# tirr-c/jxl-oxide

Measured on NVIDIA H100. Metric: Megapixels/s decoded (8K VarDCT d1.0), higher is better.
Workload: dtype f32

## Files before the change

### jxl_oxide_b200/csrc/cuda_backend.cu

```cuda
#include "cuda_backend.h"

#include <algorithm>
#include <chrono>
#include <cmath>
#include <cstdlib>
#include <cstring>
#include <atomic>
#include <thread>

namespace jxlb {

void upload_sec_large(const float* host224);

#define CUDA_CHECK(expr)                                                                              \
  do {                                                                                                \
    cudaError_t err__ = (expr);                                                                       \
    if (err__ != cudaSuccess)                                                                         \
      fail(kErrCuda, std::string("CUDA error: ") + cudaGetErrorString(err__) + " at " #expr);        \
  } while (0)

CudaBackend::CudaBackend(int device, bool own_stream) : device_(device), own_stream_(own_stream) {
  int count = 0;
  cudaError_t e = cudaGetDeviceCount(&count);
  if (e != cudaSuccess || count == 0)
    fail(kErrCuda, "no CUDA device available: the jxl_oxide_b200 hot path has no CPU fallback");
  CUDA_CHECK(cudaSetDevice(device_));
  if (own_stream_) CUDA_CHECK(cudaStreamCreateWithFlags(&stream_, cudaStreamNonBlocking));
  CUDA_CHECK(cudaEventCreateWithFlags(&sync_event_, cudaEventBlockingSync | cudaEventDisableTiming));
  stage_cap_ = size_t(2) << 20;
  CUDA_CHECK(cudaHostAlloc(reinterpret_cast<void**>(&h_stage_), stage_cap_, cudaHostAllocDefault));
  CUDA_CHECK(cudaMalloc(reinterpret_cast<void**>(&d_stage_), stage_cap_));
  result_cap_ = size_t(256) << 10;
  CUDA_CHECK(cudaHostAlloc(reinterpret_cast<void**>(&h_result_), result_cap_, cudaHostAllocMapped));
  {
    void* f = nullptr;
    CUDA_CHECK(cudaHostAlloc(&f, 128, cudaHostAllocMapped));
    h_flag_ = static_cast<volatile uint32_t*>(f);
    h_flag_[0] = 0;
    h_flag_[16] = 0;
  }
  ensure_static_tables();
  cudaMemPoolProps props;
  std::memset(&props, 0, sizeof(props));
  props.allocType = cudaMemAllocationTypePinned;
  props.handleTypes = cudaMemHandleTypeNone;
  props.location.type = cudaMemLocationTypeDevice;
  props.location.id = device_;
  CUDA_CHECK(cudaMemPoolCreate(&pool_, &props));
  uint64_t keep = UINT64_MAX;
  CUDA_CHECK(cudaMemPoolSetAttribute(pool_, cudaMemPoolAttrReleaseThreshold, &keep));
  CUDA_CHECK(cudaDeviceSetCacheConfig(cudaFuncCachePreferShared));
  if (const char* lanes = std::getenv("JXLB_HF_LANES")) {
    const int n = std::atoi(lanes);
    hf_streams_per_cta = n <= 0 ? 0 : (n <= 4 ? 4 : (n <= 8 ? 8 : (n <= 16 ? 16 : (n <= 32 ? 32 : (n <= 64 ? 64 : 128)))));
  }
}

CudaBackend::~CudaBackend() {
  cudaSetDevice(device_);
  if (stream_) cudaStreamSynchronize(stream_);
  for (auto& kv : planes_)
    if (!(arena_base_ && kv.second.ptr >= static_cast<void*>(arena_base_) && kv.second.ptr < static_cast<void*>(arena_base_ + arena_cap_)) &&
        !in_lf_arena(kv.second.ptr))
      cudaFree(kv.second.ptr);
  for (void* p : temps_)
    if (!in_lf_arena(p)) cudaFree(p);
  for (void* p : deferred_free_) cudaFree(p);
  if (d_codestream_ && !in_lf_arena(d_codestream_) && stream_) cudaFreeAsync(d_codestream_, stream_);
  if (d_natural_orders_) cudaFree(d_natural_orders_);
  if (d_dequant_) cudaFree(d_dequant_);
  if (d_dequant_default_) cudaFree(d_dequant_default_);
  if (sync_event_) cudaEventDestroy(sync_event_);
  if (h_stage_) cudaFreeHost(h_stage_);
  if (d_stage_) cudaFree(d_stage_);
  if (h_result_) cudaFreeHost(h_result_);
  if (h_input_) cudaFreeHost(h_input_);
  if (h_flag_) cudaFreeHost(const_cast<uint32_t*>(h_flag_));
  if (stream_ && own_stream_) cudaStreamDestroy(stream_);
  if (lf_arena_) cudaFree(lf_arena_);
  if (pool_) cudaMemPoolDestroy(pool_);
}

cudaStream_t CudaBackend::S() {
  if (!stream_) {
    JXLB_CHECK(bool(on_need_stream), kErrCuda, "decoder has no CUDA stream");
    if (!heavy_announced_ && (profile || host_phases)) ++profile_acc["host:slot_before_heavy"].first;
    on_need_stream();
    JXLB_CHECK(stream_ != nullptr, kErrCuda, "no CUDA stream was leased to the decoder");
    if (pending_cs_bytes_) {
      CUDA_CHECK(cudaMemcpyAsync(d_codestream_, h_input_, pending_cs_bytes_, cudaMemcpyHostToDevice, stream_));
      pending_cs_bytes_ = 0;
    }
    for (void* p : deferred_free_) CUDA_CHECK(cudaFreeAsync(p, stream_));
    deferred_free_.clear();
  }
  return stream_;
}

void CudaBackend::end_lease() {
  if (!stream_ || own_stream_) return;
  release_temps();
  if (d_dequant_) {
    dfree(d_dequant_);
    d_dequant_ = nullptr;
    cached_hfg_ = nullptr;
  }
  if (d_codestream_ && !in_lf_arena(d_codestream_)) {
    CUDA_CHECK(cudaFreeAsync(d_codestream_, stream_));
    d_codestream_ = nullptr;
    codestream_cap_ = 0;
  }
  stream_ = nullptr;
}

void* CudaBackend::lf_arena_alloc(size_t bytes) {
  if (!lf_arena_) {
    CUDA_CHECK(cudaSetDevice(device_));
    CUDA_CHECK(cudaMalloc(reinterpret_cast<void**>(&lf_arena_), kLfArenaBytes));
  }
  const size_t need = (bytes + 255) & ~size_t(255);
  if (lf_arena_off_ + need > kLfArenaBytes) return nullptr;
  void* p = lf_arena_ + lf_arena_off_;
  lf_arena_off_ += need;
  return p;
}

void CudaBackend::begin_heavy_stage(size_t bytes_hint) {
  if (heavy_announced_) return;
  heavy_announced_ = true;
  if (on_heavy_stage) on_heavy_stage(bytes_hint);
}

void CudaBackend::end_arena() {
  if (!arena_base_) return;
  auto inside = [&](const void* p) { return p >= static_cast<void*>(arena_base_) && p < static_cast<void*>(arena_base_ + arena_cap_); };
  std::vector<void*> keep;
  for (void* p : temps_)
    if (!inside(p)) keep.push_back(p);
  temps_.swap(keep);
  if (d_dequant_ && inside(d_dequant_)) {
    d_dequant_ = nullptr;
    cached_hfg_ = nullptr;
  }
  for (auto it = planes_.begin(); it != planes_.end();)
    it = inside(it->second.ptr) ? planes_.erase(it) : std::next(it);
  arena_base_ = nullptr;
  arena_cap_ = arena_off_ = 0;
}

void* CudaBackend::dmalloc(size_t bytes) {
  void* p = nullptr;
  if (mem_limit_ && mem_in_use_ + bytes > mem_limit_)
    fail(kErrOutOfMemory, "allocation budget exceeded: " + std::to_string(mem_in_use_ + bytes) + " > " + std::to_string(mem_limit_) + " bytes");
  if (arena_base_ && bytes >= (256u << 10)) {
    const size_t need = (bytes + 511) & ~size_t(511);
    if (arena_off_ + need <= arena_cap_) {
      p = arena_base_ + arena_off_;
      arena_off_ += need;
      arena_peak_ = std::max(arena_peak_, arena_off_);
      if (mem_limit_) mem_in_use_ += need;
      return p;
    }
    arena_spill_ += need;
  }
  if (!stream_ && lf_service) {
    if (void* q = lf_arena_alloc(std::max<size_t>(bytes, 16))) return q;
  }
  CUDA_CHECK(cudaSetDevice(device_));
  CUDA_CHECK(cudaMallocFromPoolAsync(&p, std::max<size_t>(bytes, 16), pool_, S()));
  if (mem_limit_) {
    mem_in_use_ += bytes;
    alloc_sizes_[p] = bytes;
  }
  return p;
}
void CudaBackend::dfree(void* p) {
  if (!p) return;
  if (in_lf_arena(p)) return;
  if (!stream_ && lf_service) {
    deferred_free_.push_back(p);
    return;
  }
  if (arena_base_ && p >= arena_base_ && p < arena_base_ + arena_cap_) return;
  if (mem_limit_) {
    auto it = alloc_sizes_.find(p);
    if (it != alloc_sizes_.end()) {
      mem_in_use_ -= std::min<uint64_t>(mem_in_use_, it->second);
      alloc_sizes_.erase(it);
    }
  }
  CUDA_CHECK(cudaFreeAsync(p, S()));
}
void* CudaBackend::upload_temp(const void* src, size_t bytes) {
  const size_t off = (stage_off_ + 15) & ~size_t(15);
  if (off + bytes <= stage_cap_) {
    if (bytes) std::memcpy(h_stage_ + off, src, bytes);
    stage_off_ = off + bytes;
    return d_stage_ + off;
  }
  void* p = dmalloc(bytes);
  temps_.push_back(p);
  if (bytes) CUDA_CHECK(cudaMemcpyAsync(p, src, bytes, cudaMemcpyHostToDevice, S()));
  return p;
}
void* CudaBackend::stage_scratch(size_t bytes) {
  if (stream_) flush_uploads();
  const size_t off = (stage_off_ + 15) & ~size_t(15);
  if (off + bytes <= stage_cap_) {
    stage_off_ = off + bytes;
    if (stream_) stage_flushed_ = stage_off_;
    return d_stage_ + off;
  }
  void* p = dmalloc(bytes);
  temps_.push_back(p);
  return p;
}
void CudaBackend::flush_uploads() {
  if (!stream_ && lf_service) return;
  if (stage_off_ > stage_flushed_)
    CUDA_CHECK(cudaMemcpyAsync(d_stage_ + stage_flushed_, h_stage_ + stage_flushed_, stage_off_ - stage_flushed_, cudaMemcpyHostToDevice, S()));
  stage_flushed_ = stage_off_;
}
void* CudaBackend::fetch_result(const void* dsrc, size_t bytes) {
  const size_t off = (result_off_ + 15) & ~size_t(15);
  JXLB_CHECK(off + bytes <= result_cap_, kErrUnsupported, "too many stream jobs in one launch for the result buffer");
  CUDA_CHECK(cudaMemcpyAsync(h_result_ + off, dsrc, bytes, cudaMemcpyDeviceToHost, S()));
  result_off_ = off + bytes;
  return h_result_ + off;
}
void CudaBackend::release_temps() {
  for (void* p : temps_) dfree(p);
  temps_.clear();
}
void CudaBackend::sync() {
  if (!stream_) return;
  flush_uploads();
  const uint32_t seq = ++sync_seq_;
  launch_signal_word(const_cast<uint32_t*>(h_flag_), seq, S());
  ++launches;
  uint32_t spins = 0;
  const auto t_begin = std::chrono::steady_clock::now();
  auto t0 = t_begin;
  while (*h_flag_ != seq) {
    if (++spins < 2000) {
#if defined(__x86_64__)
      __builtin_ia32_pause();
#endif
      continue;
    }
    const auto waited = std::chrono::steady_clock::now() - t_begin;
    const long nap_us = std::min<long>(200, std::max<long>(20, std::chrono::duration_cast<std::chrono::microseconds>(waited).count() / 8));
    std::this_thread::sleep_for(std::chrono::microseconds(nap_us));
    if ((spins & 255) == 0 && std::chrono::steady_clock::now() - t0 > std::chrono::milliseconds(200)) {
      cudaError_t e = cudaStreamQuery(S());
      if (e == cudaSuccess) break;
      if (e != cudaErrorNotReady) fail(kErrCuda, std::string("CUDA error: ") + cudaGetErrorString(e) + " while waiting for the stream");
      t0 = std::chrono::steady_clock::now();
    }
  }
  std::atomic_thread_fence(std::memory_order_acquire);
  stage_off_ = stage_flushed_ = 0;
  result_off_ = 0;
  resolve_profile();
}

namespace {
struct TimeOrigin {
  cudaEvent_t ev = nullptr;
  double host_ms = 0.0;
  unsigned long long dev_ns = 0;
};
double host_now_ms() {
  return std::chrono::duration<double, std::milli>(std::chrono::steady_clock::now().time_since_epoch()).count();
}
TimeOrigin& time_origin() {
  static TimeOrigin o = [] {
    TimeOrigin t;
    cudaEventCreate(&t.ev);
    cudaDeviceSynchronize();
    cudaEventRecord(t.ev, 0);
    cudaEventSynchronize(t.ev);
    unsigned long long* d = nullptr;
    cudaMalloc(&d, 8);
    launch_read_globaltimer(d, 0);
    cudaMemcpy(&t.dev_ns, d, 8, cudaMemcpyDeviceToHost);
    cudaFree(d);
    t.host_ms = std::chrono::duration<double, std::milli>(std::chrono::steady_clock::now().time_since_epoch()).count();
    return t;
  }();
  return o;
}
}

void CudaBackend::begin_k(const char* name) {
  S();
  flush_uploads();
  ++launches;
  if (!profile) return;
  time_origin();
  PendingTiming t;
  t.name = name;
  CUDA_CHECK(cudaEventCreate(&t.e0));
  CUDA_CHECK(cudaEventCreate(&t.e1));
  CUDA_CHECK(cudaEventRecord(t.e0, S()));
  pending_.push_back(t);
}

void CudaBackend::end_k() {
  if (!profile || pending_.empty()) return;
  CUDA_CHECK(cudaEventRecord(pending_.back().e1, S()));
}

void CudaBackend::resolve_profile() {
  for (PendingTiming& t : pending_) {
    float ms = 0.0f;
    if (cudaEventElapsedTime(&ms, t.e0, t.e1) == cudaSuccess) {
      auto& acc = profile_acc[t.name];
      acc.first += 1;
      acc.second += double(ms);
      float since = 0.0f;
      if (cudaEventElapsedTime(&since, time_origin().ev, t.e0) == cudaSuccess)
        timeline.push_back({t.name, double(since), double(since) + double(ms)});
    }
    cudaEventDestroy(t.e0);
    cudaEventDestroy(t.e1);
  }
  pending_.clear();
}

uint8_t* CudaBackend::upload_resident(const uint8_t* data, size_t size) {
  CUDA_CHECK(cudaSetDevice(device_));
  size_t need = ((size + 7) & ~size_t(7)) + 64;
  uint8_t* p = nullptr;
  CUDA_CHECK(cudaMalloc(&p, need));
  CUDA_CHECK(cudaMemset(p, 0, need));
  CUDA_CHECK(cudaMemcpy(p, data, size, cudaMemcpyHostToDevice));
  return p;
}

void CudaBackend::set_codestream(const uint8_t* data, size_t size) {
  CUDA_CHECK(cudaSetDevice(device_));
  stages.clear();
  stage_dims.clear();
  if (!stream_) {
    lf_arena_off_ = 0;
    if (in_lf_arena(d_codestream_)) d_codestream_ = nullptr, codestream_cap_ = 0;
    pending_cs_bytes_ = 0;
  }
  if (resident_next_) {
    active_cs_ = resident_next_;
    resident_next_ = nullptr;
    ensure_static_tables();
    return;
  }
  size_t need = ((size + 7) & ~size_t(7)) + 64;
  if (need > input_cap_) {
    if (h_input_) CUDA_CHECK(cudaFreeHost(h_input_));
    h_input_ = nullptr;
    input_cap_ = std::max<size_t>(need + need / 2, size_t(1) << 20);
    CUDA_CHECK(cudaHostAlloc(reinterpret_cast<void**>(&h_input_), input_cap_, cudaHostAllocDefault));
  }
  std::memcpy(h_input_, data, size);
  std::memset(h_input_ + size, 0, need - size);
  if (!stream_ && lf_service) {
    if (void* q = lf_arena_alloc(need)) {
      d_codestream_ = static_cast<uint8_t*>(q);
      codestream_cap_ = need;
      pending_cs_bytes_ = need;
      active_cs_ = d_codestream_;
      ensure_static_tables();
      return;
    }
  }
  if (need > codestream_cap_ || in_lf_arena(d_codestream_)) {
    if (d_codestream_ && !in_lf_arena(d_codestream_)) CUDA_CHECK(cudaFreeAsync(d_codestream_, S()));
    d_codestream_ = nullptr;
    codestream_cap_ = std::max<size_t>(need + need / 2, size_t(1) << 20);
    CUDA_CHECK(cudaMallocFromPoolAsync(reinterpret_cast<void**>(&d_codestream_), codestream_cap_, pool_, S()));
  }
  CUDA_CHECK(cudaMemcpyAsync(d_codestream_, h_input_, need, cudaMemcpyHostToDevice, S()));
  active_cs_ = d_codestream_;
  ensure_static_tables();
}

void CudaBackend::new_frame() {
  heavy_announced_ = false;
  cached_hfg_ = nullptr;
  if (d_dequant_) {
    dfree(d_dequant_);
    d_dequant_ = nullptr;
  }
}

void CudaBackend::ensure_static_tables() {
  if (!d_natural_orders_) {
    const std::vector<uint32_t> all = natural_order_table(natural_order_offset_);
    CUDA_CHECK(cudaMalloc(&d_natural_orders_, all.size() * 4));
    CUDA_CHECK(cudaMemcpy(d_natural_orders_, all.data(), all.size() * 4, cudaMemcpyHostToDevice));
  }
  if (!sec_uploaded_) {
    float tab[224];
    size_t off = 0;
    for (int i = 0; i < 3; ++i) {
      size_t n = size_t(64) << i;
      for (size_t k = 0; k < n / 2; ++k) {
        float theta = float(2 * k + 1) / float(2 * n) * 3.14159265358979323846f;
        tab[off + k] = (1.0f / cosf(theta)) / 2.0f;
      }
      off += n / 2;
    }
    upload_sec_large(tab);
    sec_uploaded_ = true;
  }
}

int CudaBackend::alloc_plane(uint32_t w, uint32_t h, bool zero) {
  PlaneRec r;
  r.w = w;
  r.h = h;
  size_t bytes = size_t(w) * h * 4;
  r.ptr = dmalloc(bytes);
  if (zero) CUDA_CHECK(cudaMemsetAsync(r.ptr, 0, bytes, S()));
  int id = next_id_++;
  planes_[id] = r;
  return id;
}

void CudaBackend::free_plane(int id) {
  auto it = planes_.find(id);
  if (it == planes_.end()) return;
  dfree(it->second.ptr);
  planes_.erase(it);
}

DevView CudaBackend::dev_view(const View& v) const {
  DevView d;
  d.ptr = nullptr;
  d.stride = 0;
  d.w = v.w;
  d.h = v.h;
  if (v.plane >= 0) {
    const PlaneRec& p = planes_.at(v.plane);
    d.ptr = static_cast<uint32_t*>(p.ptr) + size_t(v.y0) * p.w + v.x0;
    d.stride = p.w;
  }
  return d;
}

void CudaBackend::download_rect(const View& v, void* dst) {
  if (!v.w || !v.h) return;
  DevView d = dev_view(v);
  if (d.stride == v.w)
    CUDA_CHECK(cudaMemcpyAsync(dst, d.ptr, size_t(v.w) * v.h * 4, cudaMemcpyDeviceToHost, S()));
  else
    CUDA_CHECK(cudaMemcpy2DAsync(dst, size_t(v.w) * 4, d.ptr, size_t(d.stride) * 4, size_t(v.w) * 4, v.h,
                                 cudaMemcpyDeviceToHost, S()));
  sync();
}

void CudaBackend::copy_rect(const View& src, const View& dst) {
  begin_k("copy_rect");
  launch_copy_rect(dev_view(src), dev_view(dst), S());
  end_k();
}

void CudaBackend::phase_mark(const char* name) {
  if (!profile && !host_phases) return;
  const double now = std::chrono::duration<double, std::milli>(std::chrono::steady_clock::now().time_since_epoch()).count();
  if (name && phase_t0_ >= 0.0) {
    auto& acc = profile_acc[std::string("host:") + name];
    acc.first += 1;
    acc.second += now - phase_t0_;
    if (profile) timeline.push_back({std::string("host:") + name, phase_t0_ - time_origin().host_ms, now - time_origin().host_ms});
  }
  phase_t0_ = now;
}

void CudaBackend::stage_marker(const char* name, const View* views, int n) {
  if (!stop_stage.empty() && stop_stage == name) {
    stop_dims.clear();
    for (int i = 0; i < n; ++i) {
      stop_dims.push_back({views[i].w, views[i].h});
      if (size_t(i) < stop_dst.size() && stop_dst[size_t(i)] && views[i].w && views[i].h) {
        JXLB_CHECK(stop_stride >= views[i].w, kErrInvalidArg, "destination stride smaller than the stage's planes");
        const DevView d = dev_view(views[i]);
        CUDA_CHECK(cudaMemcpy2DAsync(stop_dst[size_t(i)], size_t(stop_stride) * 4, d.ptr, size_t(d.stride) * 4, size_t(views[i].w) * 4,
                                     views[i].h, cudaMemcpyDeviceToDevice, S()));
      }
    }
    sync();
    throw StopDecode();
  }
  if (!capture) return;
  auto& out = stages[name];
  auto& dims = stage_dims[name];
  out.clear();
  dims.clear();
  for (int i = 0; i < n; ++i) {
    std::vector<uint32_t> buf(size_t(views[i].w) * views[i].h);
    download_rect(views[i], buf.data());
    out.push_back(std::move(buf));
    dims.push_back({views[i].w, views[i].h});
  }
}

namespace {
const char* dev_status_message(int s) {
  switch (s) {
    case kDevBadStream: return "invalid entropy-coded stream (ANS final state / LZ77)";
    case kDevOverrun: return "entropy-coded stream reads past the end of its section";
    case kDevInvalid: return "semantic validation of a decoded stream failed";
    case kDevUnsupported: return "chroma subsampling with varblocks larger than 8x8 is not supported";
    case kDevBadLayout: return "invalid HfMetadata block layout";
    default: return "unknown device decode error";
  }
}
}

void CudaBackend::decode_modular(std::vector<ModularStreamJob>& jobs) {
  if (jobs.empty()) return;
  ModularLaunch L = build_modular_launch(jobs, [this](const View& v) { return dev_view(v); }, *this);
  for (size_t i = 0; i < jobs.size(); ++i) {
    const ModularLaunch::JobNeeds& n = L.needs[i];
    if (n.wp_scratch_bytes) temps_.push_back(L.jobs[i].wp_scratch = static_cast<int32_t*>(dmalloc(n.wp_scratch_bytes)));
    if (n.lz_window_bytes) temps_.push_back(L.jobs[i].lz_window = static_cast<uint32_t*>(dmalloc(n.lz_window_bytes)));
  }
  const DevModularJob* d_jobs = static_cast<const DevModularJob*>(upload_temp(L.jobs.data(), L.jobs.size() * sizeof(DevModularJob)));
  const DevChannel* d_chans = static_cast<const DevChannel*>(upload_temp(L.channels.data(), L.channels.size() * sizeof(DevChannel)));
  uint64_t* d_end = static_cast<uint64_t*>(stage_scratch(jobs.size() * 8));
  int* d_status = static_cast<int*>(stage_scratch(jobs.size() * 4));
  const DevChannelPlan* d_plans = static_cast<const DevChannelPlan*>(upload_temp(L.plans.data(), L.plans.size() * sizeof(DevChannelPlan)));
  unsigned long long* d_trace = nullptr;
  double host_launch = 0.0;
  if (trace_device) {
    time_origin();
    d_trace = static_cast<unsigned long long*>(dmalloc(jobs.size() * 16));
    temps_.push_back(d_trace);
    host_launch = host_now_ms();
  }
  const uint64_t* end;
  const int* status;
  if (!stream_ && lf_service && !d_trace && jobs.size() <= 2048) {
    LfBatchItem item;
    if (pending_cs_bytes_) {
      item.up[item.num_up++] = {d_codestream_, h_input_, pending_cs_bytes_};
      pending_cs_bytes_ = 0;
    }
    item.up[item.num_up++] = {d_stage_, h_stage_, stage_off_};
    item.ref.cs = active_cs_;
    item.ref.jobs = d_jobs;
    item.ref.channels = d_chans;
    item.ref.plans = d_plans;
    item.ref.end_bits = d_end;
    item.ref.status = d_status;
    item.num_jobs = int(jobs.size());
    item.smem_bytes = L.smem_bytes;
    item.all_staged = L.all_staged;
    uint8_t* h_end = h_result_;
    uint8_t* h_status = h_result_ + ((jobs.size() * 8 + 15) & ~size_t(15));
    JXLB_CHECK(size_t(h_status - h_result_) + jobs.size() * 4 <= result_cap_, kErrUnsupported, "too many stream jobs in one launch for the result buffer");
    if (profile || ((stage_off_ + 15) & ~size_t(15)) + 4 > stage_cap_) {
      item.down[item.num_down++] = {h_end, d_end, jobs.size() * 8};
      item.down[item.num_down++] = {h_status, d_status, jobs.size() * 4};
    } else {
      const uint32_t zero = 0;
      item.ref.counter = static_cast<uint32_t*>(upload_temp(&zero, 4));
      item.up[item.num_up - 1].bytes = stage_off_;
      item.ref.end_bits = reinterpret_cast<uint64_t*>(h_end);
      item.ref.status = reinterpret_cast<int*>(h_status);
      item.ref.num_jobs = uint32_t(jobs.size());
      item.ref.done_flag = const_cast<uint32_t*>(h_flag_ + 16);
      item.ref.done_seq = ++item_seq_;
      item.done_flag = h_flag_ + 16;
    }
    item.want_timing = profile;
    lf_service->run(item);
    ++launches;
    if (profile) {
      auto& acc = profile_acc["modular_decode"];
      acc.first += 1;
      acc.second += double(item.elapsed_ms);
    }
    stage_off_ = stage_flushed_ = 0;
    result_off_ = 0;
    end = reinterpret_cast<const uint64_t*>(h_end);
    status = reinterpret_cast<const int*>(h_status);
  } else {
    begin_k("modular_decode");
    launch_modular_decode(active_cs_, d_jobs, d_chans, d_plans, d_end, d_status, int(jobs.size()), L.smem_bytes, L.all_staged, S(), d_trace);
    end_k();
    end = static_cast<const uint64_t*>(fetch_result(d_end, jobs.size() * 8));
    status = static_cast<const int*>(fetch_result(d_status, jobs.size() * 4));
    const unsigned long long* trace = d_trace ? static_cast<const unsigned long long*>(fetch_result(d_trace, jobs.size() * 16)) : nullptr;
    sync();
    if (d_trace) {
      const TimeOrigin& o = time_origin();
      unsigned long long first = ~0ull, last = 0;
      for (size_t i = 0; i < jobs.size(); ++i) {
        first = std::min<unsigned long long>(first, trace[2 * i]);
        last = std::max<unsigned long long>(last, trace[2 * i + 1]);
      }
      timeline.push_back({"host:launch_to_return modular", host_launch - o.host_ms, host_now_ms() - o.host_ms});
      timeline.push_back({"dev:modular_decode", (double(first) - double(o.dev_ns)) * 1e-6, (double(last) - double(o.dev_ns)) * 1e-6});
    }
    CUDA_CHECK(cudaGetLastError());
  }
  release_temps();
  for (size_t i = 0; i < jobs.size(); ++i) {
    if (status[i] != kDevOk && status[i] != kDevBadLayout)
      fail(status[i] == kDevOverrun ? kErrEof : kErrDeviceDecode,
           std::string("modular stream ") + std::to_string(jobs[i].stream_index) + ": " + dev_status_message(status[i]));
    jobs[i].end_bit = size_t(end[i]);
    jobs[i].placed = jobs[i].placement.group.nb_blocks != 0;
    jobs[i].layout_ok = status[i] == kDevOk;
  }
}

int CudaBackend::squeeze_inverse(const View& avg, const View& res, bool horizontal) {
  uint32_t ow = horizontal ? avg.w + res.w : avg.w;
  uint32_t oh = horizontal ? avg.h : avg.h + res.h;
  JXLB_CHECK(horizontal ? (res.h == avg.h || res.w == 0) : (res.w == avg.w || res.h == 0), kErrBitstream,
             "squeeze residual size mismatch");
  int id = alloc_plane(std::max(ow, 1u), std::max(oh, 1u), false);
  if (!ow || !oh) return id;
  View ov{id, 0, 0, ow, oh};
  begin_k("squeeze_inverse");
  launch_squeeze_inverse(dev_view(avg), dev_view(res), dev_view(ov), horizontal, S());
  end_k();
  return id;
}

std::vector<int> CudaBackend::squeeze_inverse_many(const std::vector<std::pair<View, View>>& avg_res, bool horizontal) {
  std::vector<int> ids;
  std::vector<DevView> a, r, o;
  for (const auto& p : avg_res) {
    const View& avg = p.first;
    const View& res = p.second;
    const uint32_t ow = horizontal ? avg.w + res.w : avg.w, oh = horizontal ? avg.h : avg.h + res.h;
    JXLB_CHECK(horizontal ? (res.h == avg.h || res.w == 0) : (res.w == avg.w || res.h == 0), kErrBitstream,
               "squeeze residual size mismatch");
    const int id = alloc_plane(std::max(ow, 1u), std::max(oh, 1u), false);
    ids.push_back(id);
    if (!ow || !oh) continue;
    a.push_back(dev_view(avg));
    r.push_back(dev_view(res));
    o.push_back(dev_view(View{id, 0, 0, ow, oh}));
  }
  if (!o.empty()) {
    begin_k("squeeze_inverse");
    launch_squeeze_inverse_batch(a.data(), r.data(), o.data(), int(o.size()), horizontal, S());
    end_k();
  }
  return ids;
}

void CudaBackend::rct_inverse(const View v[3], uint32_t rct_type) {
  begin_k("rct_inverse");
  launch_rct_inverse(dev_view(v[0]), dev_view(v[1]), dev_view(v[2]), rct_type, S());
  end_k();
}

void CudaBackend::palette_inverse(const View& palette, const std::vector<View>& targets, const Transform& t,
                                  const WpHeader& wph, uint32_t bit_depth) {
  JXLB_CHECK(targets.size() <= size_t(kMaxPaletteChannels), kErrUnsupported, "palettes with more than 16 channels are not implemented on the device");
  DevView tv[kMaxPaletteChannels];
  for (size_t i = 0; i < targets.size(); ++i) tv[i] = dev_view(targets[i]);
  const uint32_t w = targets[0].w, h = targets[0].h;
  int* d_status = static_cast<int*>(dmalloc(4));
  uint8_t* d_mask = static_cast<uint8_t*>(dmalloc(size_t(w) * h));
  CUDA_CHECK(cudaMemsetAsync(d_status, 0, 4, S()));
  DevView pal{};
  if (palette.plane >= 0) pal = dev_view(palette);
  begin_k("palette_inverse");
  launch_palette_inverse(pal, tv, int(targets.size()), int(t.nb_colours), int(bit_depth), int(t.nb_deltas), d_mask, d_status, S());
  end_k();
  const int* num_delta_p = static_cast<const int*>(fetch_result(d_status, 4));
  sync();
  const int num_delta = *num_delta_p;
  if (num_delta > 0) {
    JXLB_CHECK(t.d_pred <= 13, kErrBitstream, "invalid delta-palette predictor");
    DevPaletteDeltaParams p;
    std::memset(&p, 0, sizeof(p));
    for (size_t i = 0; i < targets.size(); ++i) p.target[i] = tv[i];
    p.mask = d_mask;
    p.d_pred = t.d_pred;
    pack_wp(wph, p.wp);
    int32_t* rows = nullptr;
    if (t.d_pred == 6) rows = static_cast<int32_t*>(dmalloc(targets.size() * ((5 * size_t(w) + 3) & ~size_t(3)) * 4));
    p.wp_rows = rows;
    begin_k("palette_delta");
    launch_palette_delta(p, int(targets.size()), S());
    end_k();
    sync();
    if (rows) dfree(rows);
  }
  dfree(d_status);
  dfree(d_mask);
}

void CudaBackend::int_to_float(const View& v, const BitDepth& d) {
  begin_k("int_to_float");
  launch_int_to_float(dev_view(v), d.bits_per_sample, d.exp_bits, d.float_sample, S());
  end_k();
}

void CudaBackend::modular_xyb_to_float(const View yxb[3], const float m[3]) {
  begin_k("modular_xyb");
  launch_modular_xyb(dev_view(yxb[0]), dev_view(yxb[1]), dev_view(yxb[2]), m[0], m[1], m[2], S());
  end_k();
}

void CudaBackend::build_block_info(VarDctState& st, const std::vector<BlockInfoJob>& jobs) {
  if (jobs.empty()) return;
  std::vector<DevPlacement> dp;
  for (const BlockInfoJob& j : jobs) dp.push_back(make_dev_placement(varblock_placement(st, j), [this](const View& v) { return dev_view(v); }));
  const DevPlacement* d_jobs = static_cast<const DevPlacement*>(upload_temp(dp.data(), dp.size() * sizeof(DevPlacement)));
  int* d_status = static_cast<int*>(stage_scratch(jobs.size() * 4));
  begin_k("place_varblocks");
  launch_place_varblocks(d_jobs, int(jobs.size()), d_status, S());
  end_k();
  const int* status = static_cast<const int*>(fetch_result(d_status, jobs.size() * 4));
  sync();
  CUDA_CHECK(cudaGetLastError());
  release_temps();
  for (size_t i = 0; i < jobs.size(); ++i) JXLB_CHECK(status[i] == kDevOk, kErrBitstream, "invalid HfMetadata block layout");
}

void CudaBackend::decode_hf(VarDctState& st, std::vector<HfGroupJob>& jobs) {
  if (jobs.empty()) return;
  const uint32_t pass = jobs[0].pass_idx;
  const HfPassSyntax& hp = st.hfg->passes[pass];
  const bool hf_lz77 = hp.code.lz77_enabled;
  const DevHfParams p = build_hf_params(st, pass, *this, d_natural_orders_, natural_order_offset_);
  const HfSchedule sched = hf_schedule(p, hf_streams_per_cta);
  const std::vector<uint32_t> perm = hf_launch_order(jobs, sched.lanes);
  std::vector<DevHfJob> dj;
  for (uint32_t i : perm) dj.push_back({jobs[i].bit_pos, jobs[i].bit_limit, jobs[i].group_idx});
  const DevHfJob* d_jobs = static_cast<const DevHfJob*>(upload_temp(dj.data(), dj.size() * sizeof(DevHfJob)));
  uint64_t* d_end = static_cast<uint64_t*>(stage_scratch(jobs.size() * 8));
  int* d_status = static_cast<int*>(stage_scratch(jobs.size() * 4));
  uint2* d_list = nullptr;
  uint32_t* d_counts = nullptr;
  if (sched.lanes) {
    const size_t groups = hf_block_list_count(dev_frame(st), p);
    const size_t records = groups * p.group_dim_blocks * p.group_dim_blocks;
    d_list = static_cast<uint2*>(dmalloc(records * sizeof(uint2) + groups * 4));
    temps_.push_back(d_list);
    d_counts = reinterpret_cast<uint32_t*>(d_list + records);
    begin_k("hf_block_ctx");
    launch_hf_block_list(dev_frame(st), p, d_list, d_counts, S());
    end_k();
  }
  begin_k("decode_hf");
  if (sched.lanes)
    launch_decode_hf_lanes(active_cs_, dev_frame(st), p, d_list, d_counts, d_jobs, d_end, d_status, int(jobs.size()),
                           pass == 0 ? 1 : 0, sched.per_cta, S());
  else
    launch_decode_hf(active_cs_, dev_frame(st), p, d_jobs, d_end, d_status, int(jobs.size()), pass == 0 ? 1 : 0,
                     sched.per_cta, S());
  end_k();
  const uint64_t* end = static_cast<const uint64_t*>(fetch_result(d_end, jobs.size() * 8));
  const int* status = static_cast<const int*>(fetch_result(d_status, jobs.size() * 4));
  sync();
  CUDA_CHECK(cudaGetLastError());
  release_temps();
  for (size_t i = 0; i < jobs.size(); ++i) {
    HfGroupJob& job = jobs[perm[i]];
    if (status[i] != kDevOk)
      fail(status[i] == kDevOverrun ? kErrEof : (status[i] == kDevUnsupported ? kErrUnsupported : kErrDeviceDecode),
           std::string("HF group ") + std::to_string(job.group_idx) + ": " + dev_status_message(status[i]));
    job.end_bit = size_t(end[i]);
  }
  JXLB_CHECK(!hf_lz77, kErrUnsupported, "LZ77 in the HF coefficient streams is not supported on the device");
}

void CudaBackend::lf_dequant(VarDctState& st, const std::vector<LfDequantJob>& jobs) {
  std::vector<DevLfDequantJob> dj;
  for (const LfDequantJob& j : jobs)
    dj.push_back({{j.rect.bx0, j.rect.by0, j.rect.bw, j.rect.bh}, {j.scale[0], j.scale[1], j.scale[2]}});
  const DevLfDequantJob* d = static_cast<const DevLfDequantJob*>(upload_temp(dj.data(), dj.size() * sizeof(DevLfDequantJob)));
  begin_k("lf_dequant");
  launch_lf_dequant(dev_frame(st), d, int(dj.size()), S());
  end_k();
}

void CudaBackend::lf_chroma_from_luma(VarDctState& st) {
  const LfGlobalSyntax& g = *st.lfg;
  int32_t x_factor = int32_t(g.x_factor_lf) - 128, b_factor = int32_t(g.b_factor_lf) - 128;
  float kx = g.base_correlation_x + (float(x_factor) / float(g.colour_factor));
  float kb = g.base_correlation_b + (float(b_factor) / float(g.colour_factor));
  begin_k("lf_cfl");
  launch_lf_cfl(dev_frame(st), kx, kb, S());
  end_k();
}

void CudaBackend::lf_adaptive_smoothing(VarDctState& st) {
  const LfGlobalSyntax& g = *st.lfg;
  uint64_t scale_inv = uint64_t(g.global_scale) * g.quant_lf;
  float lf_x = float(512.0 * double(g.m_x_lf) / double(scale_inv));
  float lf_y = float(512.0 * double(g.m_y_lf) / double(scale_inv));
  float lf_b = float(512.0 * double(g.m_b_lf) / double(scale_inv));
  float* tmp[3];
  for (int c = 0; c < 3; ++c) tmp[c] = static_cast<float*>(dmalloc(size_t(st.bw) * st.bh * 4));
  begin_k("lf_smooth");
  launch_lf_smooth(dev_frame(st), tmp, lf_x, lf_y, lf_b, S());
  end_k();
  for (int c = 0; c < 3; ++c) {
    PlaneRec& r = planes_.at(st.lf[c]);
    dfree(r.ptr);
    r.ptr = tmp[c];
  }
}

void CudaBackend::hf_dequant_cfl(VarDctState& st) {
  const bool use_default = st.hfg->dequant_all_default;
  if (use_default ? d_dequant_default_ == nullptr : cached_hfg_ != st.hfg) {
    std::vector<float> all;
    DevDequantParams& dp = use_default ? dequant_default_params_ : dequant_params_;
    std::memset(&dp, 0, sizeof(dp));
    for (int set = 0; set < 17; ++set)
      for (int c = 0; c < 3; ++c)
        for (int tr = 0; tr < 2; ++tr) {
          const std::vector<float>& m = tr ? st.hfg->dequant->matrices_tr[set][c] : st.hfg->dequant->matrices[set][c];
          dp.matrix_offset[(set * 3 + c) * 2 + tr] = uint32_t(all.size());
          all.insert(all.end(), m.begin(), m.end());
        }
    if (use_default) {
      CUDA_CHECK(cudaMalloc(&d_dequant_default_, all.size() * 4));
      CUDA_CHECK(cudaMemcpyAsync(d_dequant_default_, all.data(), all.size() * 4, cudaMemcpyHostToDevice, S()));
      CUDA_CHECK(cudaStreamSynchronize(S()));
    } else {
      if (d_dequant_) dfree(d_dequant_);
      d_dequant_ = static_cast<float*>(dmalloc(all.size() * 4));
      CUDA_CHECK(cudaMemcpyAsync(d_dequant_, all.data(), all.size() * 4, cudaMemcpyHostToDevice, S()));
      cached_hfg_ = st.hfg;
    }
  }
  DevDequantParams p = use_default ? dequant_default_params_ : dequant_params_;
  p.matrices = use_default ? d_dequant_default_ : d_dequant_;
  const OpsinInverseMatrix& oim = st.ih->opsin_inverse_matrix;
  for (int c = 0; c < 3; ++c) p.quant_bias[c] = oim.quant_bias[c];
  p.quant_bias_numerator = oim.quant_bias_numerator;
  p.qm_scale[0] = powi_f32(0.8f, int32_t(st.fh->x_qm_scale) - 2);
  p.qm_scale[1] = 1.0f;
  p.qm_scale[2] = powi_f32(0.8f, int32_t(st.fh->b_qm_scale) - 2);
  p.global_scale = float(st.lfg->global_scale);
  p.base_correlation_x = st.lfg->base_correlation_x;
  p.base_correlation_b = st.lfg->base_correlation_b;
  p.colour_factor = float(st.lfg->colour_factor);
  if (!capture && !st.subsampled && fuse_dequant) {
    pending_dequant_ = p;
    have_pending_dequant_ = true;
    return;
  }
  begin_k("hf_dequant_cfl");
  launch_hf_dequant_cfl(dev_frame(st), p, S());
  end_k();
}

void CudaBackend::hf_transform(VarDctState& st) {
  void* scratch = dmalloc(hf_transform_scratch_bytes(st.bw, st.bh));
  begin_k("hf_transform");
  launch_hf_transform(dev_frame(st), scratch, have_pending_dequant_ ? &pending_dequant_ : nullptr, S());
  end_k();
  have_pending_dequant_ = false;
  dfree(scratch);
}

void CudaBackend::gaborish(const View v[3], const float weights[3][2]) {
  for (int c = 0; c < 3; ++c) {
    PlaneRec& r = planes_.at(v[c].plane);
    JXLB_CHECK(v[c].x0 == 0 && v[c].y0 == 0, kErrInvalidArg, "gaborish expects a top-left anchored view");
    void* out = dmalloc(size_t(r.w) * r.h * 4);
    DevView in = dev_view(v[c]);
    DevView ov = in;
    ov.ptr = out;
    begin_k("gaborish");
    launch_gaborish(in, ov, weights[c][0], weights[c][1], S());
    end_k();
    dfree(r.ptr);
    r.ptr = out;
  }
}

void CudaBackend::epf(const View v[3], const View& sigma, const EpfParams& p, bool sigma_is_constant) {
  DevView cur[3], alt[3];
  void* alt_ptr[3];
  for (int c = 0; c < 3; ++c) {
    PlaneRec& r = planes_.at(v[c].plane);
    JXLB_CHECK(v[c].x0 == 0 && v[c].y0 == 0, kErrInvalidArg, "epf expects a top-left anchored view");
    alt_ptr[c] = dmalloc(size_t(r.w) * r.h * 4);
    cur[c] = dev_view(v[c]);
    alt[c] = cur[c];
    alt[c].ptr = alt_ptr[c];
  }
  const float* d_sigma = nullptr;
  uint32_t sigma_stride = 0;
  if (!sigma_is_constant) {
    const PlaneRec& s = planes_.at(sigma.plane);
    d_sigma = static_cast<const float*>(s.ptr);
    sigma_stride = s.w;
  }
  DevEpfParams dp;
  for (int c = 0; c < 3; ++c) dp.channel_scale[c] = p.channel_scale[c];
  dp.pass0_sigma_scale = p.pass0_sigma_scale;
  dp.pass2_sigma_scale = p.pass2_sigma_scale;
  dp.border_sad_mul = p.border_sad_mul;
  dp.sigma_for_modular = p.sigma_for_modular;
  bool in_alt = false;
  auto run = [&](int step) {
    begin_k("epf_step");
    launch_epf_step(in_alt ? alt : cur, in_alt ? cur : alt, d_sigma, sigma_stride, dp, step, S());
    end_k();
    in_alt = !in_alt;
  };
  if (p.iters == 3) run(0);
  run(1);
  if (p.iters >= 2) run(2);
  for (int c = 0; c < 3; ++c) {
    PlaneRec& r = planes_.at(v[c].plane);
    if (in_alt) {
      dfree(r.ptr);
      r.ptr = alt_ptr[c];
    } else {
      dfree(alt_ptr[c]);
    }
  }
}

bool CudaBackend::filters_colour_fused(const View v[3], const RestorationFilter& rf, const View& sigma,
                                       bool sigma_is_constant, const ColorParams* colour) {
  if (!fuse_filters || !fused_filters_supported(v[0].w, v[0].h)) return false;
  DevView in[3], out[3];
  void* out_ptr[3];
  for (int c = 0; c < 3; ++c) {
    PlaneRec& r = planes_.at(v[c].plane);
    JXLB_CHECK(v[c].x0 == 0 && v[c].y0 == 0, kErrInvalidArg, "filters expect top-left anchored views");
    out_ptr[c] = dmalloc(size_t(r.w) * r.h * 4);
    in[c] = dev_view(v[c]);
    out[c] = in[c];
    out[c].ptr = out_ptr[c];
  }
  const float* d_sigma = nullptr;
  uint32_t sigma_stride = 0;
  if (!sigma_is_constant && rf.epf.iters > 0) {
    const PlaneRec& s = planes_.at(sigma.plane);
    d_sigma = static_cast<const float*>(s.ptr);
    sigma_stride = s.w;
  }
  JXLB_CHECK(!colour || (!colour->second_stage && colour->gamma == 0.0f), kErrInvalidArg,
             "the fused filter kernel converts to sRGB-gamut targets only");
  const DevFusedFilterParams p = fused_filter_params(rf, d_sigma, sigma_stride, colour);
  begin_k("filters_fused");
  launch_filters_fused(in, out, p, S());
  end_k();
  for (int c = 0; c < 3; ++c) {
    PlaneRec& r = planes_.at(v[c].plane);
    dfree(r.ptr);
    r.ptr = out_ptr[c];
  }
  return true;
}

void CudaBackend::blend_patches(const std::vector<PatchJob>& jobs) {
  std::vector<DevPatchJob> batch;
  std::vector<const PatchJob*> members;
  auto flush = [&] {
    if (batch.empty()) return;
    const DevPatchJob* d = static_cast<const DevPatchJob*>(upload_temp(batch.data(), batch.size() * sizeof(DevPatchJob)));
    begin_k("blend_patches");
    launch_blend_patches(d, int(batch.size()), S());
    end_k();
    batch.clear();
    members.clear();
  };
  auto overlaps = [](const View& a, const View& b) {
    return a.plane == b.plane && a.x0 < b.x0 + b.w && b.x0 < a.x0 + a.w && a.y0 < b.y0 + b.h && b.y0 < a.y0 + a.h;
  };
  for (const PatchJob& j : jobs) {
    if (!j.dst.w || !j.dst.h) continue;
    bool clash = false;
    for (const PatchJob* m : members)
      if (overlaps(m->dst, j.dst) || (j.base_alpha.plane >= 0 && overlaps(m->dst, j.base_alpha)) ||
          (j.new_alpha.plane >= 0 && overlaps(m->dst, j.new_alpha)) ||
          (m->base_alpha.plane >= 0 && overlaps(j.dst, m->base_alpha)) ||
          (m->new_alpha.plane >= 0 && overlaps(j.dst, m->new_alpha))) {
        clash = true;
        break;
      }
    if (clash || batch.size() >= 4096) flush();
    DevView s = dev_view(j.src), d = dev_view(j.dst), ba = dev_view(j.base_alpha), na = dev_view(j.new_alpha);
    batch.push_back({static_cast<const float*>(s.ptr), static_cast<float*>(d.ptr), static_cast<const float*>(ba.ptr),
                     static_cast<const float*>(na.ptr), s.stride, d.stride, ba.stride, na.stride, j.dst.w, j.dst.h, j.mode,
                     j.clamp ? 1u : 0u, j.premultiplied ? 1u : 0u, j.swapped ? 1u : 0u});
    members.push_back(&j);
  }
  flush();
}

void CudaBackend::blend_raw(const DevPatchJob& job) {
  const DevPatchJob* d = static_cast<const DevPatchJob*>(upload_temp(&job, sizeof(job)));
  begin_k("blend_patches");
  launch_blend_patches(d, 1, S());
  end_k();
  sync();
  release_temps();
}

void CudaBackend::splat_splines(const View v[3], const std::vector<SplineArc>& arcs) {
  if (arcs.empty()) return;
  static_assert(sizeof(SplineArc) == sizeof(DevSplineArc), "arc layouts must agree");
  DevView dv[3] = {dev_view(v[0]), dev_view(v[1]), dev_view(v[2])};
  const DevSplineArc* d = static_cast<const DevSplineArc*>(upload_temp(arcs.data(), arcs.size() * sizeof(SplineArc)));
  begin_k("splat_splines");
  launch_splat_splines(dv, d, int(arcs.size()), S());
  end_k();
}

void CudaBackend::add_noise(const View v[3], const float lut[8], uint32_t group_dim, uint64_t seed0, float corr_x,
                            float corr_b) {
  JXLB_CHECK(v[0].w >= 2 && v[0].h >= 2, kErrUnsupported, "noise on frames narrower than 2 samples is not supported");
  DevView dv[3];
  float* field[3];
  for (int c = 0; c < 3; ++c) {
    JXLB_CHECK(v[c].w == v[0].w && v[c].h == v[0].h, kErrInvalidArg, "noise needs three equally sized planes");
    dv[c] = dev_view(v[c]);
    field[c] = static_cast<float*>(dmalloc(size_t(v[0].w) * v[0].h * 4));
  }
  DevNoiseParams p;
  for (int i = 0; i < 8; ++i) p.lut[i] = lut[i];
  p.lut[8] = lut[7];
  p.corr_x = corr_x;
  p.corr_b = corr_b;
  p.group_dim = group_dim;
  p.seed0 = seed0;
  begin_k("add_noise");
  launch_add_noise(dv, field, p, S());
  end_k();
  for (int c = 0; c < 3; ++c) dfree(field[c]);
}

void CudaBackend::pack_to_host(const DevPackParams& p, void* dst, size_t bytes) {
  void* d = dmalloc(bytes);
  begin_k("pack_interleaved");
  launch_pack_interleaved(p, d, S());
  end_k();
  CUDA_CHECK(cudaMemcpyAsync(dst, d, bytes, cudaMemcpyDeviceToHost, S()));
  sync();
  dfree(d);
}

void CudaBackend::pack_to_device(const DevPackParams& p, void* d_dst) {
  cudaPointerAttributes attr;
  if (cudaPointerGetAttributes(&attr, d_dst) != cudaSuccess || attr.type != cudaMemoryTypeDevice || attr.device != device_) {
    cudaGetLastError();
    fail(kErrInvalidArg, "destination is not device memory of this decoder's GPU");
  }
  begin_k("pack_interleaved");
  launch_pack_interleaved(p, d_dst, S());
  end_k();
  sync();
}

int CudaBackend::upsample(const View& v, uint32_t factor_log2, const ImageHeader& ih) {
  DevView cur = dev_view(v);
  void* cur_owned = nullptr;
  uint32_t w = v.w, h = v.h;
  auto pass = [&](uint32_t k, const std::vector<float>& weights) {
// ... 181 lines not shown
```

### jxl_oxide_b200/csrc/cuda_backend.h

```cpp
#pragma once
#include <cuda_runtime.h>

#include <functional>
#include <map>
#include <string>
#include <vector>

#include "host/backend.h"
#include "host/jbrd.h"
#include "kernels/kernels.h"
#include "launch_tables.h"

namespace jxlb {

struct LfBatchItem {
  struct Copy {
    void* dst;
    const void* src;
    size_t bytes;
  };
  Copy up[2];
  int num_up = 0;
  DevModularBatchRef ref{};
  int num_jobs = 0;
  size_t smem_bytes = 0;
  bool all_staged = false;
  Copy down[2];
  int num_down = 0;
  volatile uint32_t* done_flag = nullptr;
  bool want_timing = false;
  float elapsed_ms = 0.0f;
};
class LfBatchService {
 public:
  virtual ~LfBatchService() {}
  virtual void run(LfBatchItem& item) = 0;
};

struct StopDecode {};

class CudaBackend : public Backend, private TableSink {
 public:
  explicit CudaBackend(int device, bool own_stream = true);
  ~CudaBackend() override;

  void set_codestream(const uint8_t* data, size_t size) override;
  void new_frame() override;
  int alloc_plane(uint32_t w, uint32_t h, bool zero) override;
  void free_plane(int id) override;
  void download_rect(const View& v, void* dst) override;
  void copy_rect(const View& src, const View& dst) override;
  void decode_modular(std::vector<ModularStreamJob>& jobs) override;
  int squeeze_inverse(const View& avg, const View& residual, bool horizontal) override;
  std::vector<int> squeeze_inverse_many(const std::vector<std::pair<View, View>>& avg_res, bool horizontal) override;
  void rct_inverse(const View v[3], uint32_t rct_type) override;
  void palette_inverse(const View& palette, const std::vector<View>& targets, const Transform& t, const WpHeader& wp,
                       uint32_t bit_depth) override;
  void int_to_float(const View& v, const BitDepth& depth) override;
  void modular_xyb_to_float(const View yxb[3], const float m_lf_unscaled[3]) override;
  void build_block_info(VarDctState& st, const std::vector<BlockInfoJob>& jobs) override;
  void decode_hf(VarDctState& st, std::vector<HfGroupJob>& jobs) override;
  void lf_dequant(VarDctState& st, const std::vector<LfDequantJob>& jobs) override;
  void lf_chroma_from_luma(VarDctState& st) override;
  void lf_adaptive_smoothing(VarDctState& st) override;
  void hf_dequant_cfl(VarDctState& st) override;
  void hf_transform(VarDctState& st) override;
  void gaborish(const View v[3], const float weights[3][2]) override;
  void epf(const View v[3], const View& sigma, const EpfParams& p, bool sigma_is_constant) override;
  int upsample(const View& v, uint32_t factor_log2, const ImageHeader& ih) override;
  int upsample_jpeg(const View& v, bool horizontal, bool vertical, uint32_t out_w, uint32_t out_h) override;
  void blend_patches(const std::vector<PatchJob>& jobs) override;
  void blend_raw(const DevPatchJob& job);
  void splat_splines(const View v[3], const std::vector<SplineArc>& arcs) override;
  void add_noise(const View v[3], const float lut[8], uint32_t group_dim, uint64_t seed0, float corr_x, float corr_b) override;
  void xyb_to_rgb(const View v[3], const ColorParams& p) override;
  void ycbcr_to_rgb(const View v[3], const YcbcrParams& p) override;
  bool filters_colour_fused(const View v[3], const RestorationFilter& rf, const View& sigma, bool sigma_is_constant,
                            const ColorParams* colour) override;
  void stage_marker(const char* name, const View* views, int n) override;
  void phase_mark(const char* name) override;
  void vardct_coefficients(const VarDctState& st) override;
  JpegJob* jpeg_job = nullptr;

  void begin_heavy_stage(size_t bytes_hint) override;
  std::function<void(size_t)> on_heavy_stage;
  std::function<void()> on_need_stream;
  void set_arena(void* base, size_t bytes) {
    arena_base_ = static_cast<uint8_t*>(base);
    arena_cap_ = bytes;
    arena_off_ = 0;
  }
  void end_arena();
  void set_mem_limit(uint64_t bytes) { mem_limit_ = bytes; }
  uint64_t mem_in_use() const { return mem_in_use_; }
  size_t arena_peak() const { return arena_peak_; }
  size_t arena_spill() const { return arena_spill_; }

  cudaStream_t stream() { return S(); }
  void set_stream(cudaStream_t s) { stream_ = s; }
  bool has_stream() const { return stream_ != nullptr; }
  void end_lease();
  LfBatchService* lf_service = nullptr;
  uint8_t* upload_resident(const uint8_t* data, size_t size);
  void use_resident_once(const uint8_t* dptr) { resident_next_ = dptr; }
  void sync();
  void* plane_ptr(int id) const { return id < 0 ? nullptr : planes_.at(id).ptr; }
  DevView dev_view(const View& v) const;

  std::string stop_stage;
  std::vector<void*> stop_dst;
  uint32_t stop_stride = 0;
  std::vector<std::pair<uint32_t, uint32_t>> stop_dims;
  bool capture = false;
  std::map<std::string, std::vector<std::vector<uint32_t>>> stages;
  std::map<std::string, std::vector<std::pair<uint32_t, uint32_t>>> stage_dims;
  uint64_t launches = 0;
  void pack_to_host(const DevPackParams& p, void* dst, size_t bytes);
  void pack_to_device(const DevPackParams& p, void* d_dst);
  bool fuse_dequant = true;
  bool fuse_filters = true;
  int hf_streams_per_cta = 0;
  bool profile = false;
  bool host_phases = false;
  bool trace_device = false;
  double phase_t0_ = -1.0;
  std::map<std::string, std::pair<uint64_t, double>> profile_acc;
  void resolve_profile();

 private:
  struct PlaneRec {
    void* ptr;
    uint32_t w, h;
  };
  void* dmalloc(size_t bytes);
  void dfree(void* p);
  void* upload_temp(const void* src, size_t bytes);
  const void* put(const void* src, size_t bytes) override { return upload_temp(src, bytes); }
  void* stage_scratch(size_t bytes);
  void flush_uploads();
  void release_temps();
  void* fetch_result(const void* dsrc, size_t bytes);
  DevFrame dev_frame(const VarDctState& st) const {
    return make_dev_frame(st, [this](int id) { return plane_ptr(id); });
  }
  void ensure_static_tables();
  uint64_t encode_jpeg_scan(const VarDctState& st, const JpegScanPlan& plan, std::vector<uint8_t>* out);
  void begin_k(const char* name);
  void end_k();
  struct PendingTiming {
    const char* name;
    cudaEvent_t e0, e1;
  };
  std::vector<PendingTiming> pending_;

 public:
  struct TimelineEntry {
    std::string name;
    double t0_ms, t1_ms;
  };
  std::vector<TimelineEntry> timeline;

 private:

  cudaStream_t S();
  void* lf_arena_alloc(size_t bytes);
  bool in_lf_arena(const void* p) const {
    return lf_arena_ && p >= static_cast<const void*>(lf_arena_) && p < static_cast<const void*>(lf_arena_ + kLfArenaBytes);
  }
  int device_;
  bool own_stream_ = true;
  static constexpr size_t kLfArenaBytes = size_t(64) << 20;
  uint8_t* lf_arena_ = nullptr;
  size_t lf_arena_off_ = 0;
  size_t pending_cs_bytes_ = 0;
  std::vector<void*> deferred_free_;
  uint8_t* h_stage_ = nullptr;
  uint8_t* d_stage_ = nullptr;
  size_t stage_cap_ = 0, stage_off_ = 0, stage_flushed_ = 0;
  uint8_t* h_result_ = nullptr;
  size_t result_cap_ = 0, result_off_ = 0;
  uint8_t* h_input_ = nullptr;
  size_t input_cap_ = 0;
  volatile uint32_t* h_flag_ = nullptr;
  uint32_t sync_seq_ = 0, item_seq_ = 0;
  uint8_t* arena_base_ = nullptr;
  size_t arena_cap_ = 0, arena_off_ = 0, arena_peak_ = 0, arena_spill_ = 0;
  bool heavy_announced_ = false;
  uint64_t mem_limit_ = 0, mem_in_use_ = 0;
  std::map<void*, size_t> alloc_sizes_;
  cudaStream_t stream_ = nullptr;
  cudaEvent_t sync_event_ = nullptr;
  cudaMemPool_t pool_ = nullptr;
  uint8_t* d_codestream_ = nullptr;
  const uint8_t* active_cs_ = nullptr;
  const uint8_t* resident_next_ = nullptr;
  size_t codestream_cap_ = 0;
  std::map<int, PlaneRec> planes_;
  int next_id_ = 0;
  std::vector<void*> temps_;
  uint32_t* d_natural_orders_ = nullptr;
  uint32_t natural_order_offset_[13];
  bool sec_uploaded_ = false;
  const HfGlobalSyntax* cached_hfg_ = nullptr;
  float* d_dequant_ = nullptr;
  float* d_dequant_default_ = nullptr;
  DevDequantParams dequant_default_params_;
  DevDequantParams dequant_params_;
  DevDequantParams pending_dequant_;
  bool have_pending_dequant_ = false;
};

}
```

### jxl_oxide_b200/csrc/host/backend.h

```cpp
#pragma once
#include <cstddef>
#include <cstdint>
#include <utility>
#include <vector>

#include "frame_syntax.h"
#include "headers.h"
#include "modular_syntax.h"

namespace jxlb {

struct View {
  int plane = -1;
  uint32_t x0 = 0, y0 = 0, w = 0, h = 0;
};

struct ModularChannelTarget {
  View view;
  int32_t hshift = 0, vshift = 0;
};

struct LfGroupRect {
  uint32_t bx0 = 0, by0 = 0, bw = 0, bh = 0;
};

struct BlockInfoJob {
  LfGroupRect rect;
  int raw_plane = -1;
  uint32_t nb_blocks = 0;
};

struct VarblockPlacement {
  BlockInfoJob group;
  int blk_type = -1, blk_mul = -1, epf_sigma = -1, sharpness = -1;
  float quant_mul_base = 0.0f;
  float sharp_lut[8] = {};
  bool has_epf = false;
};

struct ModularStreamJob {
  size_t bit_pos = 0;
  size_t bit_limit = 0;
  const MaTree* tree = nullptr;
  WpHeader wp;
  uint32_t stream_index = 0;
  std::vector<ModularChannelTarget> channels;
  size_t end_bit = 0;
  VarblockPlacement placement;
  bool placed = false;
  bool layout_ok = true;
};

struct HfGroupJob {
  size_t bit_pos = 0, bit_limit = 0;
  uint32_t group_idx = 0, pass_idx = 0;
  size_t end_bit = 0;
};

struct VarDctState {
  uint32_t width = 0, height = 0;
  uint32_t bw = 0, bh = 0;
  uint32_t group_dim = 256, groups_per_row = 0, num_groups = 0;
  const LfGlobalSyntax* lfg = nullptr;
  const HfGlobalSyntax* hfg = nullptr;
  const FrameHeader* fh = nullptr;
  const ImageHeader* ih = nullptr;
  bool use_lf_frame = false;
  uint32_t hshift[3] = {0, 0, 0}, vshift[3] = {0, 0, 0};
  bool subsampled = false;
  int lf_quant[3] = {-1, -1, -1};
  int x_from_y = -1, b_from_y = -1;
  int sharpness = -1;
  int blk_type = -1;
  int blk_mul = -1;
  int epf_sigma = -1;
  int lf[3] = {-1, -1, -1};
  int coeff[3] = {-1, -1, -1};
};

inline VarblockPlacement varblock_placement(const VarDctState& st, const BlockInfoJob& group) {
  const EpfParams& epf = st.fh->restoration_filter.epf;
  VarblockPlacement p;
  p.group = group;
  p.blk_type = st.blk_type;
  p.blk_mul = st.blk_mul;
  p.epf_sigma = st.epf_sigma;
  p.sharpness = st.sharpness;
  p.quant_mul_base = epf.quant_mul * 65536.0f / float(st.lfg->global_scale);
  for (int i = 0; i < 8; ++i) p.sharp_lut[i] = epf.sharp_lut[i];
  p.has_epf = epf.iters > 0;
  return p;
}

inline LfGroupRect shifted_rect(const LfGroupRect& r, uint32_t hshift, uint32_t vshift) {
  return LfGroupRect{r.bx0 >> hshift, r.by0 >> vshift, (r.bw + (1u << hshift) - 1) >> hshift, (r.bh + (1u << vshift) - 1) >> vshift};
}

struct LfDequantJob {
  LfGroupRect rect;
  float scale[3];
};

struct ColorParams {
  float opsin_bias[3], cbrt_opsin_bias[3];
  float itscale;
  float matrix[9];
  bool apply_srgb_tf;
  bool apply_bt709_tf = false;
  bool second_stage = false;
  float luminances[3] = {0, 0, 0};
  float matrix2[9] = {1, 0, 0, 0, 1, 0, 0, 0, 1};
  bool to_luma = false;
  float gamma = 0.0f;
  float pq_intensity_target = 0.0f;
};

class Backend {
 public:
  virtual ~Backend() {}
  virtual void set_codestream(const uint8_t* data, size_t size) = 0;
  virtual void new_frame() {}
  virtual void begin_heavy_stage(size_t ) {}
  virtual int alloc_plane(uint32_t w, uint32_t h, bool zero) = 0;
  virtual void free_plane(int id) = 0;
  virtual void download_rect(const View& v, void* dst) = 0;
  virtual void copy_rect(const View& src, const View& dst) = 0;
  virtual void decode_modular(std::vector<ModularStreamJob>& jobs) = 0;
  virtual int squeeze_inverse(const View& avg, const View& residual, bool horizontal) = 0;
  virtual std::vector<int> squeeze_inverse_many(const std::vector<std::pair<View, View>>& avg_res, bool horizontal) {
    std::vector<int> ids;
    for (const auto& p : avg_res) ids.push_back(squeeze_inverse(p.first, p.second, horizontal));
    return ids;
  }
  virtual void rct_inverse(const View v[3], uint32_t rct_type) = 0;
  virtual void palette_inverse(const View& palette, const std::vector<View>& targets, const Transform& t,
                               const WpHeader& wp, uint32_t bit_depth) = 0;
  virtual void int_to_float(const View& v, const BitDepth& depth) = 0;
  virtual void modular_xyb_to_float(const View yxb[3], const float m_lf_unscaled[3]) = 0;
  virtual void build_block_info(VarDctState& st, const std::vector<BlockInfoJob>& jobs) = 0;
  virtual void decode_hf(VarDctState& st, std::vector<HfGroupJob>& jobs) = 0;
  virtual void lf_dequant(VarDctState& st, const std::vector<LfDequantJob>& jobs) = 0;
  virtual void lf_chroma_from_luma(VarDctState& st) = 0;
  virtual void lf_adaptive_smoothing(VarDctState& st) = 0;
  virtual void hf_dequant_cfl(VarDctState& st) = 0;
  virtual void hf_transform(VarDctState& st) = 0;
  virtual void gaborish(const View v[3], const float weights[3][2]) = 0;
  virtual void epf(const View v[3], const View& sigma, const EpfParams& p, bool sigma_is_constant) = 0;
  virtual int upsample(const View& v, uint32_t factor_log2, const ImageHeader& ih) = 0;
  virtual int upsample_jpeg(const View& v, bool horizontal, bool vertical, uint32_t out_w, uint32_t out_h) = 0;
  struct PatchJob {
    View src, dst;
    uint32_t mode;
    bool clamp;
    bool premultiplied = false;
    bool swapped = false;
    View base_alpha, new_alpha;
  };
  virtual void blend_patches(const std::vector<PatchJob>& jobs) = 0;
  struct SplineArc {
    float x, y, sigma, inv_sigma, value[3];
    int32_t xbegin, xend, ybegin, yend;
  };
  virtual void splat_splines(const View v[3], const std::vector<SplineArc>& arcs) = 0;
  virtual void add_noise(const View v[3], const float lut[8], uint32_t group_dim, uint64_t seed0, float corr_x,
                         float corr_b) = 0;
  virtual void xyb_to_rgb(const View v[3], const ColorParams& p) = 0;
  struct YcbcrParams {
    float y_offset, cr_to_r, cb_to_g, cr_to_g, cb_to_b;
    YcbcrParams() {
      y_offset = 128.0f / 255.0f;
      cr_to_r = 1.402f;
      cb_to_g = -0.114f * 1.772f / 0.587f;
      cr_to_g = -0.299f * 1.402f / 0.587f;
      cb_to_b = 1.772f;
    }
  };
  virtual void ycbcr_to_rgb(const View v[3], const YcbcrParams& p) = 0;
  virtual bool filters_colour_fused(const View [3], const RestorationFilter& , const View& ,
                                    bool , const ColorParams* ) {
    return false;
  }
  virtual void vardct_coefficients(const VarDctState& ) {}
  virtual void stage_marker(const char* , const View* , int ) {}
  virtual void phase_mark(const char* ) {}
};

}
```

### jxl_oxide_b200/csrc/host/planner.cc

```cpp
#include "planner.h"

#include "icc.h"

#include <algorithm>
#include <array>
#include <cmath>
#include <cstring>
#include <deque>
#include <map>
#include <memory>

namespace jxlb {

std::vector<uint8_t> extract_codestream(const uint8_t* data, size_t size) {
  static const uint8_t kSig[12] = {0, 0, 0, 0x0c, 'J', 'X', 'L', ' ', 0x0d, 0x0a, 0x87, 0x0a};
  if (size < 12 || std::memcmp(data, kSig, 12) != 0) return std::vector<uint8_t>(data, data + size);
  std::vector<uint8_t> out;
  size_t pos = 0;
  while (pos + 8 <= size) {
    uint64_t box_size = (uint64_t(data[pos]) << 24) | (uint64_t(data[pos + 1]) << 16) | (uint64_t(data[pos + 2]) << 8) | data[pos + 3];
    const uint8_t* ty = data + pos + 4;
    size_t header = 8;
    if (box_size == 1) {
      JXLB_CHECK(pos + 16 <= size, kErrEof, "truncated container box");
// ... 345 lines not shown
    JXLB_CHECK(src.w == dst.w && src.h == dst.h, kErrBitstream, "modular transform size mismatch");
    if (src.w && src.h) be_.copy_rect(src, dst);
    if (ps.coded[i].owned && src.plane >= 0) drop_plane(src.plane);
  }
}

void FramePlanner::setup_gmodular() {
  const ModularStreamSyntax& s = lfg_.gmodular;
  const uint32_t gd = fh_.group_dim();
  const uint32_t gshift = ceil_log2_nonzero(gd);
  for (const ChannelInfo& c : s.channels) {
    View v;
    v.w = c.width;
    v.h = c.height;
    v.plane = (c.width && c.height) ? new_plane(c.width, c.height) : -1;
    gm_coded_.push_back({v, true});
  }
  size_t i = 0;
  for (; i < s.channels.size(); ++i) {
    const ChannelInfo& c = s.channels[i];
    if (!(i < s.nb_meta_channels || (c.width <= gd && c.height <= gd))) break;
  }
  gm_global_count_ = i;
  std::map<uint32_t, std::pair<int32_t, int32_t>> pass_shifts;
  int32_t maxshift = 3;
  for (size_t k = 0; k < fh_.passes.downsample.size() && k < fh_.passes.last_pass.size(); ++k) {
    int32_t minshift = int32_t(ceil_log2_nonzero(fh_.passes.downsample[k]));
    pass_shifts[fh_.passes.last_pass[k]] = {minshift, maxshift};
    maxshift = minshift;
  }
  pass_shifts[fh_.passes.num_passes - 1] = {0, maxshift};
  const uint32_t num_passes = fh_.passes.num_passes;
  const uint32_t cw = fh_.color_sample_width(), chh = fh_.color_sample_height();
  gm_lf_groups_.assign(fh_.num_lf_groups(), {});
  gm_pass_groups_.assign(num_passes, std::vector<std::vector<GroupChannel>>(fh_.num_groups()));
  for (; i < s.channels.size(); ++i) {
    const ChannelInfo& c = s.channels[i];
    JXLB_CHECK(c.hshift >= 0 && c.vshift >= 0, kErrBitstream, "unshiftable channel outside the global stream");
    uint32_t ow = cw, oh = chh;
    if (c.hshift < 3 || c.vshift < 3) {
      int32_t shift = std::min(c.hshift, c.vshift);
      int pass = -1;
      for (auto& kv : pass_shifts)
        if (shift >= kv.second.first && shift < kv.second.second) {
          pass = int(kv.first);
          break;
        }
      JXLB_CHECK(pass >= 0 && uint32_t(pass) < num_passes, kErrBitstream, "no pass for modular channel shift");
      uint32_t gw = gd >> c.hshift, gh = gd >> c.vshift;
      JXLB_CHECK(gw && gh, kErrBitstream, "channel shift too large after transform");
      uint32_t nx = (ow + gd - 1) >> gshift, ny = (oh + gd - 1) >> gshift;
      JXLB_CHECK(nx * ny == fh_.num_groups(), kErrBitstream, "modular group count mismatch");
      for (uint32_t gy = 0; gy < ny; ++gy)
        for (uint32_t gx = 0; gx < nx; ++gx) {
          uint32_t x0 = gx * gw, y0 = gy * gh;
          if (x0 >= c.width || y0 >= c.height) continue;
          View v{gm_coded_[i].view.plane, x0, y0, std::min(gw, c.width - x0), std::min(gh, c.height - y0)};
          gm_pass_groups_[pass][gy * nx + gx].push_back({v, c.hshift, c.vshift});
        }
    } else {
      uint32_t gw = gd >> (c.hshift - 3), gh = gd >> (c.vshift - 3);
      JXLB_CHECK(gw && gh, kErrBitstream, "channel shift too large after transform");
      uint32_t nx = (ow + (gd << 3) - 1) >> (gshift + 3), ny = (oh + (gd << 3) - 1) >> (gshift + 3);
      JXLB_CHECK(nx * ny == fh_.num_lf_groups(), kErrBitstream, "modular LF group count mismatch");
      for (uint32_t gy = 0; gy < ny; ++gy)
        for (uint32_t gx = 0; gx < nx; ++gx) {
          uint32_t x0 = gx * gw, y0 = gy * gh;
          if (x0 >= c.width || y0 >= c.height) continue;
          View v{gm_coded_[i].view.plane, x0, y0, std::min(gw, c.width - x0), std::min(gh, c.height - y0)};
          gm_lf_groups_[gy * nx + gx].push_back({v, c.hshift, c.vshift});
        }
    }
  }
}

DecodedFrame FramePlanner::decode_frame(size_t frame_begin_byte, size_t* frame_end_byte) {
  BitReader br(cs_, size_, frame_begin_byte * 8);
  be_.phase_mark(nullptr);
  be_.new_frame();
  fh_ = parse_frame_header(br, ih_);
  toc_ = parse_toc(br, fh_);
  *frame_end_byte = toc_.data_begin + toc_.total_size;
  JXLB_CHECK(*frame_end_byte <= size_, kErrEof, "frame data beyond end of codestream");

  const bool vardct = fh_.encoding == Encoding::kVarDct;
  const bool is_lf_frame = fh_.frame_type == FrameType::kLfFrame;
  const bool is_ref_frame = fh_.frame_type == FrameType::kReferenceOnly;
  if (is_ref_frame) {
    JXLB_CHECK(fh_.save_before_ct, kErrUnsupported, "reference frames saved after the colour transform are not supported");
    JXLB_CHECK(fh_.upsampling == 1, kErrUnsupported, "upsampled reference frames are not supported");
  } else if (!is_lf_frame) {
    JXLB_CHECK(!fh_.save_before_ct || fh_.is_last, kErrUnsupported, "regular frames saved before the colour transform are not supported");
  } else {
    JXLB_CHECK(fh_.lf_level >= 1 && fh_.lf_level <= 4 && fh_.upsampling == 1, kErrBitstream, "invalid LF frame header");
  }
  if (fh_.use_lf_frame()) {
    JXLB_CHECK(vardct, kErrBitstream, "use_lf_frame on a Modular frame");
    JXLB_CHECK(fh_.lf_level < 4 && (*lf_store_)[fh_.lf_level].valid, kErrBitstream, "frame refers to an LF frame that was not decoded");
  }
  bool h_subsampling = false, v_subsampling = false;
  uint32_t chan_hshift[3] = {0, 0, 0}, chan_vshift[3] = {0, 0, 0};
  for (uint32_t j : fh_.jpeg_upsampling) {
    h_subsampling |= j == 1 || j == 2;
    v_subsampling |= j == 1 || j == 3;
  }
  for (int c = 0; c < 3; ++c) {
    const uint32_t j = fh_.jpeg_upsampling[c];
    chan_hshift[c] = (j == 0 || j == 3) && h_subsampling;
    chan_vshift[c] = (j == 0 || j == 2) && v_subsampling;
  }
  const bool chroma_subsampled = h_subsampling || v_subsampling;
  JXLB_CHECK(!chroma_subsampled || vardct, kErrUnsupported, "chroma-subsampled Modular frames are not implemented");
  JXLB_CHECK(!chroma_subsampled || fh_.skip_adaptive_lf_smoothing(), kErrUnsupported, "adaptive LF smoothing of a chroma-subsampled frame");
  auto blocks_w = [&](uint32_t px) { return h_subsampling ? ((px + 7) / 8 + 1) / 2 * 2 : (px + 7) / 8; };
  auto blocks_h = [&](uint32_t px) { return v_subsampling ? ((px + 7) / 8 + 1) / 2 * 2 : (px + 7) / 8; };
  for (uint32_t u : fh_.ec_upsampling) JXLB_CHECK(u == fh_.upsampling, kErrUnsupported, "extra-channel upsampling differs from colour");
  for (const auto& ec : ih_.ec_info) JXLB_CHECK(ec.dim_shift == 0, kErrUnsupported, "dim_shift extra channels not supported");

  const uint32_t num_lf_groups = fh_.num_lf_groups(), num_groups = fh_.num_groups();
  const uint32_t num_passes = fh_.passes.num_passes;
  const bool single = toc_.single_entry();
  const uint32_t cw = fh_.color_sample_width(), chh = fh_.color_sample_height();

  size_t pos, limit;
  section(0, &pos, &limit);
  {
    BitReader r = reader_at(pos, limit);
    lfg_ = parse_lf_global(r, ih_, fh_);
    pos = r.pos();
  }
  if (lfg_.has_gmodular) {
    if (!vardct) be_.begin_heavy_stage(size_t(cw) * chh * 4 * 2 * (lfg_.gmodular.channels.size() + 2) + (size_t(64) << 20));
    setup_gmodular();
    std::vector<ModularStreamJob> jobs(1);
    ModularStreamJob& job = jobs[0];
    job.bit_pos = pos;
    job.bit_limit = limit * 8;
    job.tree = tree_for(lfg_.gmodular);
    job.wp = lfg_.gmodular.header.wp;
    job.stream_index = 0;
    for (size_t i = 0; i < gm_global_count_; ++i) {
      const ChannelInfo& c = lfg_.gmodular.channels[i];
      job.channels.push_back({gm_coded_[i].view, c.hshift, c.vshift});
    }
    be_.decode_modular(jobs);
    pos = jobs[0].end_bit;
  } else {
    gm_lf_groups_.assign(num_lf_groups, {});
    gm_pass_groups_.assign(num_passes, std::vector<std::vector<GroupChannel>>(num_groups));
  }

  be_.phase_mark("lf_global");
  if (vardct) {
    st_ = VarDctState();
    st_.width = cw;
    st_.height = chh;
    st_.bw = blocks_w(cw);
    st_.bh = blocks_h(chh);
    st_.subsampled = chroma_subsampled;
    for (int c = 0; c < 3; ++c) st_.hshift[c] = chan_hshift[c], st_.vshift[c] = chan_vshift[c];
    st_.group_dim = fh_.group_dim();
    st_.groups_per_row = fh_.groups_per_row();
    st_.num_groups = num_groups;
    st_.lfg = &lfg_;
    st_.hfg = &hfg_;
    st_.fh = &fh_;
    st_.ih = &ih_;
    st_.use_lf_frame = fh_.use_lf_frame();
    if (st_.use_lf_frame) {
      const LfFrameStore& lf = (*lf_store_)[fh_.lf_level];
      JXLB_CHECK(lf.planes[0].w == st_.bw && lf.planes[0].h == st_.bh, kErrBitstream, "LF frame size does not match the frame");
    }
    for (int c = 0; c < 3; ++c) {
      st_.lf_quant[c] = new_plane(st_.bw, st_.bh);
      st_.lf[c] = new_plane(st_.bw, st_.bh);
    }
    st_.x_from_y = new_plane((cw + 63) / 64, (chh + 63) / 64);
    st_.b_from_y = new_plane((cw + 63) / 64, (chh + 63) / 64);
    st_.sharpness = new_plane(st_.bw, st_.bh);
    st_.blk_type = new_plane(st_.bw, st_.bh);
    st_.blk_mul = new_plane(st_.bw, st_.bh);
    st_.epf_sigma = new_plane(st_.bw, st_.bh);
  }

  be_.phase_mark("alloc");
  std::vector<size_t> lf_pos(num_lf_groups), lf_limit(num_lf_groups);
  std::vector<LfGroupRect> lf_rect(num_lf_groups);
  for (uint32_t g = 0; g < num_lf_groups; ++g) {
    if (single) {
      lf_pos[g] = pos;
      lf_limit[g] = limit;
    } else {
      section(1 + g, &lf_pos[g], &lf_limit[g]);
    }
    uint32_t gx = g % fh_.lf_groups_per_row(), gy = g / fh_.lf_groups_per_row();
    uint32_t lfd = fh_.lf_group_dim();
    uint32_t lw = std::min(lfd, cw - gx * lfd), lh = std::min(lfd, chh - gy * lfd);
    lf_rect[g] = {gx * (lfd / 8), gy * (lfd / 8), blocks_w(lw), blocks_h(lh)};
  }
  lf_rect_ = lf_rect;
  extra_precision_.assign(num_lf_groups, 0);
  if (vardct && !fh_.use_lf_frame()) {
    std::vector<ModularStreamJob> jobs;
    std::vector<PendingStream> pend;
    for (uint32_t g = 0; g < num_lf_groups; ++g) {
      BitReader r = reader_at(lf_pos[g], lf_limit[g]);
      extra_precision_[g] = r.read(2);
      const LfGroupRect& rc = lf_rect[g];
      std::vector<GroupChannel> chans;
      for (int mc : {1, 0, 2}) {
        const LfGroupRect sr = shifted_rect(rc, st_.hshift[mc], st_.vshift[mc]);
        chans.push_back({View{st_.lf_quant[mc], sr.bx0, sr.by0, sr.bw, sr.bh}, int32_t(st_.hshift[mc]), int32_t(st_.vshift[mc])});
      }
      pend.push_back(prepare_stream(r, lf_limit[g], chans, 1 + g, &jobs));
    }
    be_.decode_modular(jobs);
    for (uint32_t g = 0; g < num_lf_groups; ++g) {
      finish_stream(pend[g]);
      lf_pos[g] = jobs[pend[g].job_index].end_bit;
    }
  }
  be_.phase_mark("lf_coeff");
  {
    std::vector<ModularStreamJob> jobs;
    std::vector<PendingStream> pend;
    std::vector<uint32_t> owner;
    for (uint32_t g = 0; g < num_lf_groups; ++g) {
      if (gm_lf_groups_[g].empty()) continue;
      BitReader r = reader_at(lf_pos[g], lf_limit[g]);
      pend.push_back(prepare_stream(r, lf_limit[g], gm_lf_groups_[g], 1 + num_lf_groups + g, &jobs));
      owner.push_back(g);
    }
    if (!jobs.empty()) be_.decode_modular(jobs);
    for (size_t k = 0; k < pend.size(); ++k) {
      finish_stream(pend[k]);
      lf_pos[owner[k]] = jobs[pend[k].job_index].end_bit;
    }
  }
  be_.phase_mark("mlf");
  if (vardct) {
    std::vector<ModularStreamJob> jobs;
    std::vector<PendingStream> pend;
    std::vector<BlockInfoJob> bjobs;
    for (uint32_t g = 0; g < num_lf_groups; ++g) {
      BitReader r = reader_at(lf_pos[g], lf_limit[g]);
      const LfGroupRect& rc = lf_rect[g];
      uint32_t nb_blocks = 1 + r.read(ceil_log2_nonzero(rc.bw * rc.bh));
      uint32_t w64 = (rc.bw + 7) / 8, h64 = (rc.bh + 7) / 8;
      int raw = new_plane(nb_blocks, 2);
      std::vector<GroupChannel> chans;
      chans.push_back({View{st_.x_from_y, rc.bx0 / 8, rc.by0 / 8, w64, h64}, 0, 0});
      chans.push_back({View{st_.b_from_y, rc.bx0 / 8, rc.by0 / 8, w64, h64}, 0, 0});
      chans.push_back({View{raw, 0, 0, nb_blocks, 2}, 0, 0});
      chans.push_back({View{st_.sharpness, rc.bx0, rc.by0, rc.bw, rc.bh}, 0, 0});
      pend.push_back(prepare_stream(r, lf_limit[g], chans, 1 + 2 * num_lf_groups + g, &jobs));
      bjobs.push_back({rc, raw, nb_blocks});
      if (pend.back().direct) jobs[pend.back().job_index].placement = varblock_placement(st_, bjobs.back());
    }
    be_.decode_modular(jobs);
    for (uint32_t g = 0; g < num_lf_groups; ++g) {
      finish_stream(pend[g]);
      lf_pos[g] = jobs[pend[g].job_index].end_bit;
    }
    std::vector<BlockInfoJob> rest;
    for (uint32_t g = 0; g < num_lf_groups; ++g) {
      const ModularStreamJob& j = jobs[pend[g].job_index];
      if (j.placed) JXLB_CHECK(j.layout_ok, kErrBitstream, "invalid HfMetadata block layout");
      else rest.push_back(bjobs[g]);
    }
    if (!rest.empty()) be_.build_block_info(st_, rest);
    for (auto& b : bjobs) drop_plane(b.raw_plane);
  }
  be_.phase_mark("hf_metadata");
  if (single) pos = lf_pos[0];

  if (vardct) {
    size_t hpos = pos, hlimit = limit;
    if (!single) section(1 + num_lf_groups, &hpos, &hlimit);
    BitReader r = reader_at(hpos, hlimit);
    RawTableDecoder raw_decoder = [&](BitReader& br, uint32_t w, uint32_t h, uint32_t stream_index, std::vector<int32_t> out[3]) {
      std::vector<GroupChannel> chans;
      std::vector<int> planes;
      for (int c = 0; c < 3; ++c) {
        planes.push_back(new_plane(w, h));
        chans.push_back({View{planes[c], 0, 0, w, h}, 0, 0});
      }
      std::vector<ModularStreamJob> jobs;
      PendingStream ps = prepare_stream(br, hlimit, chans, stream_index, &jobs);
      be_.decode_modular(jobs);
      finish_stream(ps);
      for (int c = 0; c < 3; ++c) {
        out[c].resize(size_t(w) * h);
        be_.download_rect(chans[c].view, out[c].data());
        drop_plane(planes[c]);
      }
      br = BitReader(cs_, hlimit, jobs[ps.job_index].end_bit);
    };
    hfg_ = parse_hf_global(r, ih_, fh_, lfg_, raw_decoder);
    if (single) pos = r.pos();
  }

  be_.phase_mark("hf_global");
  if (vardct) {
    be_.begin_heavy_stage(size_t(st_.bw) * st_.bh * 64 * 4 * 6 + (size_t(64) << 20));
    be_.phase_mark("heavy_wait");
    for (int c = 0; c < 3; ++c) st_.coeff[c] = new_plane(st_.bw * 8, st_.bh * 8, true);
  }
  for (uint32_t p = 0; p < num_passes; ++p) {
    std::vector<size_t> gpos(num_groups), glimit(num_groups);
    for (uint32_t g = 0; g < num_groups; ++g) {
      if (single) {
        gpos[g] = pos;
        glimit[g] = limit;
      } else {
        section(2 + num_lf_groups + p * num_groups + g, &gpos[g], &glimit[g]);
      }
    }
    if (vardct) {
      std::vector<HfGroupJob> jobs(num_groups);
      for (uint32_t g = 0; g < num_groups; ++g) jobs[g] = {gpos[g], glimit[g] * 8, g, p, 0};
      be_.decode_hf(st_, jobs);
      for (uint32_t g = 0; g < num_groups; ++g) gpos[g] = jobs[g].end_bit;
    }
    std::vector<ModularStreamJob> jobs;
    std::vector<PendingStream> pend;
    for (uint32_t g = 0; g < num_groups; ++g) {
      if (gm_pass_groups_[p][g].empty()) continue;
      BitReader r = reader_at(gpos[g], glimit[g]);
      pend.push_back(prepare_stream(r, glimit[g], gm_pass_groups_[p][g],
                                    1 + 3 * num_lf_groups + 17 + p * num_groups + g, &jobs));
    }
    if (!jobs.empty()) be_.decode_modular(jobs);
    for (auto& ps : pend) finish_stream(ps);
  }

  be_.phase_mark("pass_groups");
  {
    std::vector<View> coded;
    if (lfg_.has_gmodular)
      for (const ChanBuf& c : gm_coded_) coded.push_back(c.view);
    be_.stage_marker("modular_coded", coded.data(), int(coded.size()));
  }
  std::vector<ChanBuf> gm_image = gm_coded_;
  if (lfg_.has_gmodular) run_inverse_transforms(lfg_.gmodular, gm_image);

  be_.phase_mark("inverse_transforms");
  DecodedFrame out;
  out.header = fh_;
  out.width = cw;
  out.height = chh;
  std::vector<View> colour;
  size_t ec_from = 0;
  if (vardct) {
    render_vardct(&out);
    for (int c = 0; c < 3; ++c) {
      if (st_.hshift[c] || st_.vshift[c]) {
        const View sub{st_.coeff[c], 0, 0, (cw + st_.hshift[c]) >> st_.hshift[c], (chh + st_.vshift[c]) >> st_.vshift[c]};
        const int id = be_.upsample_jpeg(sub, st_.hshift[c] != 0, st_.vshift[c] != 0, cw, chh);
        frame_planes_.push_back(id);
        colour.push_back(View{id, 0, 0, cw, chh});
      } else {
        colour.push_back(View{st_.coeff[c], 0, 0, cw, chh});
      }
    }
    if (st_.subsampled) be_.stage_marker("jpeg_upsampled", colour.data(), 3);
  } else {
    ec_from = fh_.encoded_color_channels;
    JXLB_CHECK(gm_image.size() >= ec_from, kErrBitstream, "missing modular colour channels");
    for (size_t c = 0; c < ec_from; ++c) colour.push_back(gm_image[c].view);
    if (ih_.xyb_encoded) {
      JXLB_CHECK(colour.size() == 3, kErrBitstream, "XYB modular frame needs three channels");
      View yxb[3] = {colour[0], colour[1], colour[2]};
      const float m[3] = {lfg_.m_x_lf / 128.0f, lfg_.m_y_lf / 128.0f, lfg_.m_b_lf / 128.0f};
      be_.modular_xyb_to_float(yxb, m);
    } else {
      for (View& v : colour) be_.int_to_float(v, ih_.bit_depth);
    }
  }
  be_.phase_mark("render_vardct");
  be_.stage_marker("pre_filter", colour.data(), int(colour.size()));

  const RestorationFilter& rf = fh_.restoration_filter;
  const bool upsampled = fh_.upsampling > 1;
  bool colour_done = is_lf_frame || is_ref_frame;
  if (rf.gab_enabled || rf.epf.iters > 0) {
    JXLB_CHECK(colour.size() == 3 || colour.size() == 1, kErrUnsupported, "restoration filters need one or three colour channels");
    View v[3];
    for (int c = 0; c < 3; ++c) {
      if (size_t(c) < colour.size()) {
        v[c] = colour[c];
      } else {
        int id = new_plane(colour[0].w, colour[0].h);
        v[c] = View{id, 0, 0, colour[0].w, colour[0].h};
        be_.copy_rect(colour[0], v[c]);
      }
    }
    View sigma_view;
    if (vardct) sigma_view = View{st_.epf_sigma, 0, 0, st_.bw, st_.bh};
    ColorParams cp;
    const bool want_colour = !upsampled && !colour_done && !lfg_.has_noise && !lfg_.has_patches && !lfg_.has_splines &&
                             colour_params(ih_.xyb_encoded, colour.size(), &cp) && !cp.second_stage && cp.gamma == 0.0f &&
                             cp.pq_intensity_target == 0.0f;
    if (be_.filters_colour_fused(v, rf, sigma_view, !vardct, want_colour ? &cp : nullptr)) {
      colour_done = want_colour;
      if (want_colour) be_.stage_marker("rgb", v, 3);
    } else {
      if (rf.gab_enabled) {
        be_.gaborish(v, rf.gab_weights);
        be_.stage_marker("gaborish", v, 3);
      }
      if (rf.epf.iters > 0) {
        be_.epf(v, sigma_view, rf.epf, !vardct);
        be_.stage_marker("epf", v, 3);
      }
    }
  }

  be_.phase_mark("filters");
  auto upsample_view = [&](View& v) {
    const uint32_t factor_log2 = ceil_log2_nonzero(fh_.upsampling);
    int id = be_.upsample(v, factor_log2, ih_);
    frame_planes_.push_back(id);
    v = View{id, 0, 0, std::min(v.w << factor_log2, fh_.width), std::min(v.h << factor_log2, fh_.height)};
  };
  if (upsampled) {
    for (View& v : colour) upsample_view(v);
    out.width = fh_.width;
    out.height = fh_.height;
    be_.stage_marker("upsampled", colour.data(), int(colour.size()));
  }
  std::vector<View> extra;
  for (size_t c = ec_from; c < gm_image.size() && (c - ec_from) < ih_.ec_info.size(); ++c) {
    View v = gm_image[c].view;
    be_.int_to_float(v, ih_.ec_info[c - ec_from].bit_depth);
    if (upsampled) upsample_view(v);
    extra.push_back(v);
  }
  if (lfg_.has_patches) {
    std::vector<View> all = colour;
    all.insert(all.end(), extra.begin(), extra.end());
    std::vector<Backend::PatchJob> jobs;
    for (const PatchRef& pr : lfg_.patches) {
      const RefFrameStore& ref = (*ref_store_)[pr.ref_idx];
      JXLB_CHECK(ref.valid, kErrBitstream, "patch refers to a reference frame that was not decoded");
      JXLB_CHECK(ref.channels.size() == all.size(), kErrBitstream, "patch reference has a different channel count");
      for (const PatchTarget& t : pr.targets)
        for (size_t idx = 0; idx < all.size(); ++idx) {
          const PatchBlending& b = idx < colour.size() ? t.blending[0] : t.blending[1 + idx - colour.size()];
          if (b.mode == 0) continue;
          uint32_t job_mode = b.mode;
          bool with_alpha = false, swapped = false;
          const size_t alpha_view = colour.size() + b.alpha_channel;
          if (b.mode >= 4) {
            JXLB_CHECK(alpha_view < all.size(), kErrBitstream, "patch blending refers to a missing alpha channel");
            swapped = b.mode == 5 || b.mode == 7;
            const bool is_alpha = idx == alpha_view;
            if (b.mode <= 5) {
              job_mode = is_alpha ? 6 : 4;
            } else {
              if (is_alpha && !swapped) continue;
              job_mode = is_alpha ? 1 : 5;
            }
            with_alpha = !is_alpha;
          }
          const int64_t fw = all[idx].w, fhh = all[idx].h;
          const int64_t tl = std::max<int64_t>(t.x, 0), tt = std::max<int64_t>(t.y, 0);
          const int64_t tr = std::min<int64_t>(int64_t(t.x) + pr.width, fw), tb = std::min<int64_t>(int64_t(t.y) + pr.height, fhh);
          if (tr <= tl || tb <= tt) continue;
          const int64_t left = tl - t.x, top = tt - t.y;
          const int64_t rl = int64_t(pr.x0) + left, rt = int64_t(pr.y0) + top;
          const int64_t rr = std::min<int64_t>(rl + (tr - tl), ref.width), rb = std::min<int64_t>(rt + (tb - tt), ref.height);
          if (rr <= rl || rb <= rt) continue;
          const View& rv = ref.channels[idx];
          const View& dv = all[idx];
          Backend::PatchJob j;
          j.src = View{rv.plane, rv.x0 + uint32_t(rl), rv.y0 + uint32_t(rt), uint32_t(rr - rl), uint32_t(rb - rt)};
          j.dst = View{dv.plane, dv.x0 + uint32_t(tl), dv.y0 + uint32_t(tt), uint32_t(rr - rl), uint32_t(rb - rt)};
          j.mode = job_mode;
          j.clamp = b.clamp;
          j.swapped = swapped && job_mode != 1;
          if (with_alpha) {
            const View& fa = all[alpha_view];
            const View& ra = ref.channels[alpha_view];
            j.base_alpha = View{fa.plane, fa.x0 + uint32_t(tl), fa.y0 + uint32_t(tt), j.dst.w, j.dst.h};
            j.new_alpha = View{ra.plane, ra.x0 + uint32_t(rl), ra.y0 + uint32_t(rt), j.dst.w, j.dst.h};
            j.premultiplied = ih_.ec_info[b.alpha_channel].alpha_associated;
          }
          jobs.push_back(j);
        }
    }
    be_.blend_patches(jobs);
    be_.stage_marker("patches", colour.data(), int(colour.size()));
  }
  if (lfg_.has_splines) {
    JXLB_CHECK(colour.size() == 3, kErrUnsupported, "splines need three colour channels");
    JXLB_CHECK(!upsampled, kErrUnsupported, "splines together with upsampling are not implemented");
    const std::vector<Backend::SplineArc> arcs =
        build_spline_arcs(lfg_, vardct, vardct ? lfg_.base_correlation_x : 0.0f, vardct ? lfg_.base_correlation_b : 1.0f, fh_.width, fh_.height);
    View v[3] = {colour[0], colour[1], colour[2]};
    be_.splat_splines(v, arcs);
    be_.stage_marker("splines", v, 3);
  }
  if (lfg_.has_noise) {
    JXLB_CHECK(colour.size() == 3 && ih_.xyb_encoded, kErrUnsupported, "noise synthesis is implemented for XYB colour frames");
    JXLB_CHECK(!upsampled, kErrUnsupported, "noise synthesis together with upsampling is not implemented");
    View v[3] = {colour[0], colour[1], colour[2]};
    const float corr_x = vardct ? lfg_.base_correlation_x : 0.0f, corr_b = vardct ? lfg_.base_correlation_b : 1.0f;
    const bool shown = !is_lf_frame && !is_ref_frame;
    const uint64_t seed0 = shown ? ((visible_before_ + 1) << 32) : (visible_before_ << 32) + invisible_before_ + 1;
    be_.add_noise(v, lfg_.noise_lut, fh_.group_dim(), seed0, corr_x, corr_b);
    be_.stage_marker("noise", v, 3);
  }
  if (fh_.do_ycbcr && !colour_done) {
    JXLB_CHECK(colour.size() == 3, kErrBitstream, "YCbCr needs three channels");
    View v[3] = {colour[0], colour[1], colour[2]};
    be_.ycbcr_to_rgb(v, Backend::YcbcrParams());
    be_.stage_marker("rgb", v, 3);
    if (ih_.colour_encoding.colour_space == ColourSpace::kGrey) colour.resize(1);
  }
  finish_colour(colour, ih_.xyb_encoded, colour_done, &out);
  out.channels.insert(out.channels.end(), extra.begin(), extra.end());
  if (is_lf_frame) {
    JXLB_CHECK(colour.size() == 3, kErrUnsupported, "grayscale LF frames are not supported");
    LfFrameStore& slot = (*lf_store_)[fh_.lf_level - 1];
    if (slot.valid)
      for (const View& v : slot.planes) be_.free_plane(v.plane);
    for (int c = 0; c < 3; ++c) slot.planes[c] = colour[c];
    slot.valid = true;
    out.internal = true;
  }
  const bool normal_frame = !is_lf_frame && !is_ref_frame;
  const bool can_reference = !fh_.is_last && (fh_.duration == 0 || fh_.save_as_reference != 0) && !is_lf_frame;
  if (normal_frame && !(fh_.resets_canvas && out.width == ih_.width && out.height == ih_.height)) {
    const size_t ncol = colour.size();
    const bool has_extra = !fh_.ec_blending_info.empty();
    std::vector<View> frame_ch = out.channels;
    std::vector<View> canvas(frame_ch.size());
    std::vector<Backend::PatchJob> colour_jobs, extra_jobs;
    const int64_t fx0 = std::max<int64_t>(fh_.x0, 0), fy0 = std::max<int64_t>(fh_.y0, 0);
    const int64_t fx1 = std::min<int64_t>(int64_t(fh_.x0) + out.width, ih_.width), fy1 = std::min<int64_t>(int64_t(fh_.y0) + out.height, ih_.height);
    for (size_t idx = 0; idx < frame_ch.size(); ++idx) {
      const BlendingInfo& bi = idx < ncol ? fh_.blending_info : fh_.ec_blending_info[idx - ncol];
      const RefFrameStore& base = (*ref_store_)[bi.source];
      int id = new_plane(ih_.width, ih_.height, true);
      canvas[idx] = View{id, 0, 0, ih_.width, ih_.height};
      const bool have_base = base.valid && idx < base.channels.size();
      if (have_base) {
        JXLB_CHECK(base.ct_done || !ih_.xyb_encoded, kErrUnsupported, "blending onto a frame saved before the colour transform");
        const View& bv = base.channels[idx];
        const uint32_t cw = std::min(bv.w, ih_.width), chh = std::min(bv.h, ih_.height);
        be_.copy_rect(View{bv.plane, bv.x0, bv.y0, cw, chh}, View{id, 0, 0, cw, chh});
      }
      if (fx1 <= fx0 || fy1 <= fy0) continue;
      Backend::PatchJob j;
      const uint32_t rw = uint32_t(fx1 - fx0), rh = uint32_t(fy1 - fy0);
      const uint32_t sx = uint32_t(fx0 - fh_.x0), sy = uint32_t(fy0 - fh_.y0);
      j.src = View{frame_ch[idx].plane, frame_ch[idx].x0 + sx, frame_ch[idx].y0 + sy, rw, rh};
      j.dst = View{id, uint32_t(fx0), uint32_t(fy0), rw, rh};
      j.clamp = bi.clamp;
      const bool uses_alpha = (bi.mode == BlendMode::kBlend || bi.mode == BlendMode::kMulAdd) && has_extra;
      const size_t alpha_ch = ncol + bi.alpha_channel;
      if (uses_alpha) {
        JXLB_CHECK(alpha_ch < frame_ch.size(), kErrBitstream, "blend alpha channel out of range");
        j.new_alpha = View{frame_ch[alpha_ch].plane, frame_ch[alpha_ch].x0 + sx, frame_ch[alpha_ch].y0 + sy, rw, rh};
        if (base.valid && alpha_ch < base.channels.size()) {
          const View& av = base.channels[alpha_ch];
          if (uint32_t(fx1) <= av.w && uint32_t(fy1) <= av.h) j.base_alpha = View{av.plane, av.x0 + uint32_t(fx0), av.y0 + uint32_t(fy0), rw, rh};
          else JXLB_CHECK(false, kErrUnsupported, "blend base smaller than the frame rectangle");
        }
        j.premultiplied = ih_.ec_info[bi.alpha_channel].alpha_associated;
      }
      switch (bi.mode) {
        case BlendMode::kReplace: j.mode = 1; break;
        case BlendMode::kAdd: j.mode = 2; break;
        case BlendMode::kMul: j.mode = 3; break;
        case BlendMode::kBlend: j.mode = !uses_alpha ? 1 : (idx == alpha_ch ? 6 : 4); break;
        default: j.mode = !uses_alpha ? 2 : (idx == alpha_ch ? 0 : 5); break;
      }
      if (j.mode == 6) j.new_alpha = j.base_alpha = View();
      if (j.mode == 0) continue;
      (idx < ncol ? colour_jobs : extra_jobs).push_back(j);
    }
    be_.blend_patches(colour_jobs);
    be_.blend_patches(extra_jobs);
    out.channels = canvas;
    out.width = ih_.width;
    out.height = ih_.height;
  }
  if (is_ref_frame || (normal_frame && can_reference)) {
    RefFrameStore& slot = (*ref_store_)[fh_.save_as_reference];
    if (slot.valid)
      for (const View& v : slot.channels) be_.free_plane(v.plane);
    slot.channels.clear();
    if (is_ref_frame) {
      slot.channels = out.channels;
    } else {
      for (const View& v : out.channels) {
        int id = be_.alloc_plane(std::max(v.w, 1u), std::max(v.h, 1u), false);
        if (v.w && v.h) be_.copy_rect(v, View{id, 0, 0, v.w, v.h});
        slot.channels.push_back(View{id, 0, 0, v.w, v.h});
      }
    }
    slot.width = out.width;
    slot.height = out.height;
    slot.ct_done = !is_ref_frame;
    slot.valid = true;
  }
  if (is_ref_frame || (normal_frame && !fh_.is_keyframe())) out.internal = true;
  for (int id : frame_planes_) {
    bool exported = false;
    for (const View& v : out.channels) exported |= (v.plane == id);
    if (!exported) be_.free_plane(id);
  }
  frame_planes_.clear();
  gm_coded_.clear();
  be_.phase_mark("filters_colour");
  return out;
}

void FramePlanner::render_vardct(DecodedFrame*) {
  be_.vardct_coefficients(st_);
  std::vector<LfDequantJob> jobs;
  const uint32_t lfd = fh_.lf_group_dim();
  for (uint32_t g = 0; g < fh_.num_lf_groups(); ++g) {
    LfDequantJob j;
    j.rect = lf_rect_[g];
    const float m[3] = {lfg_.m_x_lf, lfg_.m_y_lf, lfg_.m_b_lf};
    int32_t precision_scale = 1 << (9 - extra_precision_[g]);
    uint64_t scale_inv = uint64_t(lfg_.global_scale) * lfg_.quant_lf;
    for (int c = 0; c < 3; ++c) j.scale[c] = float(double(m[c]) * double(precision_scale) / double(scale_inv));
    jobs.push_back(j);
  }
  if (st_.use_lf_frame) {
    const LfFrameStore& lf = (*lf_store_)[fh_.lf_level];
    for (int c = 0; c < 3; ++c) be_.copy_rect(lf.planes[c], View{st_.lf[c], 0, 0, st_.bw, st_.bh});
  } else {
    be_.lf_dequant(st_, jobs);
    if (!st_.subsampled) be_.lf_chroma_from_luma(st_);
    if (!fh_.skip_adaptive_lf_smoothing()) be_.lf_adaptive_smoothing(st_);
// ... 237 lines not shown
```

### jxl_oxide_b200/csrc/kernels/entropy.cu

```cuda
#include "kernels.h"

#include "stream_common.cuh"
#include "hf_lanes.cuh"

namespace jxlb {

namespace {


struct HfSmem {
  uint32_t ctxlut, configs, bctx, cmap, cmap_stride, ans, total;
};
__host__ __device__ inline HfSmem hf_layout(const DevHfParams& p) {
  HfSmem L;
  uint32_t off = 0;
  auto take = [&](uint32_t bytes) {
    uint32_t o = off;
    off += (bytes + 15) & ~15u;
    return o;
  };
  L.ctxlut = take(128);
  L.configs = take(p.code.num_clusters * 4);
  L.bctx = take(p.block_ctx_map_size);
  L.cmap_stride = 495 * p.num_block_clusters;
  L.cmap = take(L.cmap_stride * p.num_hf_presets);
  uint32_t ab = p.code.use_prefix ? 0 : (p.code.num_clusters << p.code.log_alphabet_size) * 8;
  L.ans = (!p.code.use_prefix && ab <= kHfAnsSmemBytes) ? take(ab) : 0xffffffffu;
  L.total = off;
  return L;
}

template <bool SUB, int W, bool ANS_SMEM>
__global__ void __launch_bounds__(W * 32) decode_hf_warp_kernel(const uint8_t* __restrict__ cs, DevFrame f, DevHfParams p,
                                                                const DevHfJob* __restrict__ jobs,
                                                                uint64_t* __restrict__ end_bits, int* __restrict__ status,
                                                                int num_jobs, int first_pass) {
  extern __shared__ __align__(16) uint8_t smem[];
  __shared__ uint32_t s_nz[W][3][32];
  const HfSmem L = hf_layout(p);
  const uint32_t tid = threadIdx.x, nthreads = blockDim.x, lane = tid & 31, warp = tid >> 5;
  uint8_t* s_ctx = smem + L.ctxlut;
  for (uint32_t i = tid; i < 63; i += nthreads) {
    s_ctx[i] = hftab::kCoeffFreqContext[i];
    s_ctx[64 + i] = hftab::kCoeffNumNonzeroContext[i];
  }
  uint32_t* s_cfg = reinterpret_cast<uint32_t*>(smem + L.configs);
  for (uint32_t i = tid; i < p.code.num_clusters; i += nthreads) s_cfg[i] = __ldg(p.code.configs + i);
  uint8_t* s_bctx = smem + L.bctx;
  for (uint32_t i = tid; i < p.block_ctx_map_size; i += nthreads) s_bctx[i] = __ldg(p.block_ctx_map + i);
  {
    uint8_t* dst = smem + L.cmap;
    const uint32_t n = L.cmap_stride * p.num_hf_presets;
    for (uint32_t i = tid; i < n; i += nthreads) dst[i] = __ldg(p.code.cluster_map + i);
  }
  if (ANS_SMEM) {
    uint4* s_ans = reinterpret_cast<uint4*>(smem + L.ans);
    const uint32_t quads = (p.code.num_clusters << p.code.log_alphabet_size) / 2;
    const uint4* src = reinterpret_cast<const uint4*>(p.code.ans);
    for (uint32_t i = tid; i < quads; i += nthreads) s_ans[i] = __ldg(src + i);
  }
  __syncthreads();
  const int job_idx = blockIdx.x * W + int(warp);
  if (job_idx >= num_jobs || lane != 0) return;

  HfTables<HfLds> T;
  T.cfg = HfLds::addr(s_cfg);
  T.ans = ANS_SMEM ? HfLds::addr(smem + L.ans) : 0;
  T.ans_g = p.code.ans;
  T.prefix = p.code.prefix;
  T.prefix_meta = p.code.prefix_meta;
  T.log_alphabet_size = p.code.log_alphabet_size;
  T.log_bucket = 12 - p.code.log_alphabet_size;
  T.use_prefix = p.code.use_prefix;
  const uint32_t a_ctx = HfLds::addr(s_ctx), a_bctx = HfLds::addr(s_bctx);

  const DevHfJob job = jobs[job_idx];
  HfBits br;
  br.init(cs, job.bit_pos, job.bit_limit);
  int err = kDevOk;
  uint32_t hfp_bits = 0;
  while ((1u << hfp_bits) < p.num_hf_presets) ++hfp_bits;
  uint32_t hfp = br.take(hfp_bits);
  if (hfp >= p.num_hf_presets) {
    err = kDevInvalid;
    hfp = 0;
  }
  const uint32_t nbc = p.num_block_clusters;
  const uint32_t a_cmap = HfLds::addr(smem + L.cmap) + hfp * L.cmap_stride;
  const uint32_t lf_idx_mul = (p.num_lf_thr[0] + 1) * (p.num_lf_thr[1] + 1) * (p.num_lf_thr[2] + 1);
  const uint32_t hf_idx_mul = p.num_qf_thr + 1;
  br.top_up();
  uint32_t ans_state = p.code.use_prefix ? 0x130000u : br.take(32);

  const uint32_t gx = job.group_idx % p.groups_per_row, gy = job.group_idx / p.groups_per_row;
  const uint32_t gb = p.group_dim_blocks;
  const uint32_t bx0 = gx * gb, by0 = gy * gb;
  const uint32_t width = min(gb, f.bw - bx0), height = min(gb, f.bh - by0);
  uint32_t(*nz_row)[32] = s_nz[warp];
  for (int c = 0; c < 3; ++c)
    for (int i = 0; i < 32; ++i) nz_row[c][i] = 0;
  const int32_t* thr_base[3] = {p.lf_thresholds, p.lf_thresholds + p.num_lf_thr[0],
                                p.lf_thresholds + p.num_lf_thr[0] + p.num_lf_thr[1]};

  for (uint32_t y = 0; y < height && err == kDevOk; ++y)
    for (uint32_t x = 0; x < width && err == kDevOk; ++x) {
      const size_t gi = size_t(by0 + y) * f.bw + bx0 + x;
      const int32_t t = f.blk_type[gi];
      if (t < 0) continue;
      const int32_t qf = f.blk_mul[gi];
      const uint32_t w8 = kTInfo[t][0], h8 = kTInfo[t][1];
      const uint32_t order_id = kTInfo[t][3];
      const bool transpose = kTInfo[t][4] != 0;
      const uint32_t num_blocks = w8 * h8;
      const uint32_t num_blocks_log = 31u - uint32_t(__clz(int(num_blocks)));
      uint32_t lf_idx = 0;
      if (p.has_lf_quant) {
        const int cs3[3] = {0, 2, 1};
#pragma unroll
        for (int k = 0; k < 3; ++k) {
          const int c = cs3[k];
          lf_idx *= p.num_lf_thr[c] + 1;
          if (p.num_lf_thr[c]) {
            const int32_t q = SUB ? f.lf_quant[c][size_t((by0 + y) >> f.vshift[c]) * f.bw + ((bx0 + x) >> f.hshift[c])] : f.lf_quant[c][gi];
            for (uint32_t i = 0; i < p.num_lf_thr[c]; ++i)
              if (q > thr_base[c][i]) ++lf_idx;
          }
        }
      }
      uint32_t hf_idx = 0;
      for (uint32_t i = 0; i < p.num_qf_thr; ++i)
        if (qf > int32_t(p.qf_thresholds[i])) ++hf_idx;
#pragma unroll 1
      for (int ci = 0; ci < 3 && err == kDevOk; ++ci) {
        const uint32_t ch_idx = uint32_t(ci) * 13 + order_id;
        const int c = (ci == 0) ? 1 : (ci == 1 ? 0 : 2);
        uint32_t sx = x, sy = y, sbx0 = bx0, sby0 = by0;
        if (SUB) {
          const uint32_t hs = f.hshift[c], vs = f.vshift[c];
          sx = x >> hs, sy = y >> vs, sbx0 = bx0 >> hs, sby0 = by0 >> vs;
          if (hs | vs) {
            if ((sx << hs) != x || (sy << vs) != y) continue;
            if (f.blk_type[size_t(by0 + sy) * f.bw + bx0 + sx] < 0) continue;
            if (num_blocks != 1) {
              err = kDevUnsupported;
              break;
            }
          }
        }
        const uint32_t idx = (ch_idx * hf_idx_mul + hf_idx) * lf_idx_mul + lf_idx;
        const uint32_t block_ctx = HfLds::u8(a_bctx + idx);
        uint32_t predicted;
        const uint32_t nz_here = nz_row[c][sx];
        const uint32_t nz_left = sx ? nz_row[c][sx - 1] : 0;
        if (sy == 0) predicted = sx == 0 ? 32 : nz_left;
        else if (sx == 0) predicted = nz_here;
        else predicted = (nz_here + nz_left + 1) >> 1;
        const uint32_t pidx = predicted >= 8 ? 4 + predicted / 2 : predicted;
        br.top_up();
        uint32_t non_zeros = hf_read_value<HfLds, ANS_SMEM>(T, br, ans_state, HfLds::u8(a_cmap + block_ctx + pidx * nbc));
        if (non_zeros > (63u << num_blocks_log)) {
          err = kDevInvalid;
          break;
        }
        const uint32_t nz_val = (non_zeros + num_blocks - 1) >> num_blocks_log;
        for (uint32_t dx = 0; dx < w8; ++dx) nz_row[c][sx + dx] = nz_val;
        if (non_zeros == 0) continue;
        uint32_t prev_nonzero = (non_zeros <= num_blocks * 4) ? 1 : 0;
        const uint32_t* order = p.orders + p.order_offset[order_id * 3 + c];
        const uint32_t size = num_blocks * 64;
        const uint32_t a_blk = a_cmap + block_ctx * 458 + 37 * nbc;
        uint32_t* plane = f.coeff[c];
        const size_t base = (size_t(sby0 + sy) * 8) * f.cw + size_t(sbx0 + sx) * 8;
        uint32_t nzc2 = HfLds::u8(a_ctx + 64 + ((non_zeros - 1) >> num_blocks_log)) * 2;
        for (uint32_t k = num_blocks, i = 0; k < size; ++k, ++i) {
          const uint32_t cctx = nzc2 + HfLds::u8(a_ctx + (i >> num_blocks_log)) * 2 + prev_nonzero;
          if (cctx >= 458) {
            err = kDevInvalid;
            break;
          }
          br.top_up();
          const uint32_t ucoeff = hf_read_value<HfLds, ANS_SMEM>(T, br, ans_state, HfLds::u8(a_blk + cctx));
          if (ucoeff == 0) {
            prev_nonzero = 0;
            continue;
          }
          const uint32_t o = __ldg(order + k);
          const uint32_t cvv = uint32_t(dev_unpack_signed(ucoeff)) << p.coeff_shift;
          uint32_t dx = o & 0xffff, dy = o >> 16;
          if (transpose) {
            const uint32_t tmp = dx;
            dx = dy;
            dy = tmp;
          }
          uint32_t* dst = plane + base + size_t(dy) * f.cw + dx;
          if (first_pass) *dst = cvv;
          else *dst += cvv;
          prev_nonzero = 1;
          if (--non_zeros == 0) break;
          nzc2 = HfLds::u8(a_ctx + 64 + ((non_zeros - 1) >> num_blocks_log)) * 2;
        }
        if (br.pos() > job.bit_limit) err = kDevOverrun;
      }
    }
  if (err == kDevOk && !p.code.use_prefix && ans_state != 0x130000u) err = kDevBadStream;
  if (err == kDevOk && br.pos() > job.bit_limit) err = kDevOverrun;
  end_bits[job_idx] = br.pos();
  status[job_idx] = err;
}


template <bool SUB>
__global__ void __launch_bounds__(256) hf_block_list_kernel(DevFrame f, DevHfParams p, uint2* __restrict__ list,
                                                            uint32_t* __restrict__ counts) {
  __shared__ uint32_t s_warp[8];
  const uint32_t g = blockIdx.x, tid = threadIdx.x, lane = tid & 31, warp = tid >> 5;
  const HfGroupRect r = hf_group_rect(f, p, g);
  const uint32_t n = r.width * r.height;
  uint2* out = list + size_t(g) * p.group_dim_blocks * p.group_dim_blocks;
  uint32_t base = 0;
  for (uint32_t i0 = 0; i0 < n; i0 += 256) {
    uint2 rec;
    const bool has = i0 + tid < n && hf_block_record<SUB>(f, p, r, i0 + tid, rec);
    const uint32_t ballot = __ballot_sync(0xffffffffu, has);
    if (lane == 0) s_warp[warp] = __popc(ballot);
    __syncthreads();
    uint32_t before = base, total = 0;
    for (uint32_t w = 0; w < 8; ++w) {
      before += w < warp ? s_warp[w] : 0;
      total += s_warp[w];
    }
    if (has) out[before + __popc(ballot & ((1u << lane) - 1))] = rec;
    base += total;
    __syncthreads();
  }
  if (tid == 0) counts[g] = base;
}

template <bool SUB, bool STAGED>
__global__ void __launch_bounds__(128) decode_hf_lanes_kernel(const uint8_t* __restrict__ cs, DevFrame f, DevHfParams p,
                                                              const uint2* __restrict__ list,
                                                              const uint32_t* __restrict__ counts,
                                                              const DevHfJob* __restrict__ jobs,
                                                              uint64_t* __restrict__ end_bits, int* __restrict__ status,
                                                              int num_jobs, int first_pass) {
  extern __shared__ __align__(16) uint8_t smem[];
  const uint32_t tid = threadIdx.x, nthreads = blockDim.x;
  const HfLaneSmem L = hf_lane_layout(p, nthreads);
  uint8_t* s_ctx = smem + L.ctxlut;
  for (uint32_t i = tid; i < 63; i += nthreads) {
    s_ctx[i] = hftab::kCoeffFreqContext[i];
    s_ctx[64 + i] = hftab::kCoeffNumNonzeroContext[i];
  }
  uint32_t* s_cfg = reinterpret_cast<uint32_t*>(smem + L.configs);
  for (uint32_t i = tid; i < p.code.num_clusters; i += nthreads) s_cfg[i] = __ldg(p.code.configs + i);
  uint8_t* s_bctx = smem + L.bctx;
  for (uint32_t i = tid; i < p.block_ctx_map_size; i += nthreads) s_bctx[i] = __ldg(p.block_ctx_map + i);
  uint32_t* s_small = reinterpret_cast<uint32_t*>(smem + L.small);
  for (uint32_t i = tid; i < 27; i += nthreads) s_small[i] = hf_pack_tinfo(i);
  for (uint32_t i = tid; i < 39; i += nthreads) s_small[27 + i] = p.order_offset[i];
  HfLaneView<HfLds> T;
  T.tinfo = HfLds::addr(s_small);
  T.order_offset = HfLds::addr(s_small + 27);
  T.ctx = HfLds::addr(s_ctx);
  T.bctx = HfLds::addr(s_bctx);
  T.nz = HfLds::addr(smem + L.nz + tid);
  T.nz_stride = nthreads;
  T.cmap_stride = L.cmap_stride;
  T.cmap = 0;
  T.cmap_ptr = p.code.cluster_map;
  if (L.cmap != 0xffffffffu) {
    uint8_t* s_cmap = smem + L.cmap;
    const uint32_t n = L.cmap_stride * p.num_hf_presets;
    for (uint32_t i = tid; i < n; i += nthreads) s_cmap[i] = __ldg(p.code.cluster_map + i);
    T.cmap = HfLds::addr(s_cmap);
    T.cmap_ptr = s_cmap;
  }
  T.code.cfg = HfLds::addr(s_cfg);
  T.code.ans = 0;
  T.code.ans_g = p.code.ans;
  T.code.prefix = p.code.prefix;
  T.code.prefix_meta = p.code.prefix_meta;
  T.code.log_alphabet_size = p.code.log_alphabet_size;
  T.code.log_bucket = 12 - p.code.log_alphabet_size;
  T.code.use_prefix = p.code.use_prefix;
  T.cv.log_alphabet_size = p.code.log_alphabet_size;
  T.cv.use_prefix = p.code.use_prefix;
  T.cv.configs = s_cfg;
  T.cv.ans = p.code.ans;
  T.cv.prefix = p.code.prefix;
  T.cv.prefix_meta = p.code.prefix_meta;
  if (L.ans != 0xffffffffu) {
    uint4* s_ans = reinterpret_cast<uint4*>(smem + L.ans);
    const uint32_t quads = (p.code.num_clusters << p.code.log_alphabet_size) / 2;
    const uint4* src = reinterpret_cast<const uint4*>(p.code.ans);
    for (uint32_t i = tid; i < quads; i += nthreads) s_ans[i] = __ldg(src + i);
    T.code.ans = HfLds::addr(s_ans);
    T.cv.ans = reinterpret_cast<const uint64_t*>(s_ans);
  }
  __syncthreads();
  const int job_idx = blockIdx.x * int(nthreads) + int(tid);
  if (job_idx >= num_jobs) return;
  const DevHfJob job = jobs[job_idx];
  const uint32_t gb = p.group_dim_blocks;
  hf_lane_stream<SUB, STAGED>(cs, f, p, T, list + size_t(job.group_idx) * gb * gb, __ldg(counts + job.group_idx), job,
                              first_pass, end_bits + job_idx, status + job_idx);
}

}

size_t hf_block_list_count(DevFrame f, DevHfParams p) {
  const uint32_t gb = p.group_dim_blocks;
  return size_t((f.bh + gb - 1) / gb) * p.groups_per_row;
}

void launch_hf_block_list(DevFrame f, DevHfParams p, uint2* list, uint32_t* counts, cudaStream_t stream) {
  const uint32_t groups = uint32_t(hf_block_list_count(f, p));
  if (f.subsampled) hf_block_list_kernel<true><<<groups, 256, 0, stream>>>(f, p, list, counts);
  else hf_block_list_kernel<false><<<groups, 256, 0, stream>>>(f, p, list, counts);
}

void launch_decode_hf_lanes(const uint8_t* cs, DevFrame f, DevHfParams p, const uint2* list, const uint32_t* counts,
                            const DevHfJob* jobs, uint64_t* end_bits, int* status, int num_jobs, int first_pass,
                            int streams_per_cta, cudaStream_t stream) {
  if (num_jobs <= 0) return;
  static const bool attr_set = [] {
    cudaFuncSetAttribute(decode_hf_lanes_kernel<false, false>, cudaFuncAttributeMaxDynamicSharedMemorySize, 200 * 1024);
    cudaFuncSetAttribute(decode_hf_lanes_kernel<true, false>, cudaFuncAttributeMaxDynamicSharedMemorySize, 200 * 1024);
    cudaFuncSetAttribute(decode_hf_lanes_kernel<false, true>, cudaFuncAttributeMaxDynamicSharedMemorySize, 200 * 1024);
    cudaFuncSetAttribute(decode_hf_lanes_kernel<true, true>, cudaFuncAttributeMaxDynamicSharedMemorySize, 200 * 1024);
    return true;
  }();
  (void)attr_set;
  const int nthreads = streams_per_cta <= 64 ? 64 : 128;
  const HfLaneSmem L = hf_lane_layout(p, uint32_t(nthreads));
  const int ctas = (num_jobs + nthreads - 1) / nthreads;
#define JXLB_HF_LANES(SUB_, STAGED_)                                                                                 \
  decode_hf_lanes_kernel<SUB_, STAGED_><<<ctas, nthreads, L.total, stream>>>(cs, f, p, list, counts, jobs, end_bits, \
                                                                             status, num_jobs, first_pass)
  if (hf_lane_staged(p, L)) {
    if (f.subsampled) JXLB_HF_LANES(true, true);
    else JXLB_HF_LANES(false, true);
  } else {
    if (f.subsampled) JXLB_HF_LANES(true, false);
    else JXLB_HF_LANES(false, false);
  }
#undef JXLB_HF_LANES
}

namespace {
template <int W, bool ANS_SMEM>
void launch_hf_warp(const uint8_t* cs, DevFrame f, DevHfParams p, const DevHfJob* jobs, uint64_t* end_bits, int* status,
                    int num_jobs, int first_pass, cudaStream_t stream) {
  static const bool attr_set = [] {
    cudaFuncSetAttribute(decode_hf_warp_kernel<false, W, ANS_SMEM>, cudaFuncAttributeMaxDynamicSharedMemorySize, 200 * 1024);
    cudaFuncSetAttribute(decode_hf_warp_kernel<true, W, ANS_SMEM>, cudaFuncAttributeMaxDynamicSharedMemorySize, 200 * 1024);
    return true;
  }();
  (void)attr_set;
  const HfSmem L = hf_layout(p);
  const int ctas = (num_jobs + W - 1) / W;
  if (f.subsampled)
    decode_hf_warp_kernel<true, W, ANS_SMEM><<<ctas, W * 32, L.total, stream>>>(cs, f, p, jobs, end_bits, status, num_jobs, first_pass);
  else
    decode_hf_warp_kernel<false, W, ANS_SMEM><<<ctas, W * 32, L.total, stream>>>(cs, f, p, jobs, end_bits, status, num_jobs, first_pass);
}
}

void launch_decode_hf(const uint8_t* cs, DevFrame f, DevHfParams p, const DevHfJob* jobs, uint64_t* end_bits, int* status,
                      int num_jobs, int first_pass, int warps_per_cta, cudaStream_t stream) {
  if (num_jobs <= 0) return;
  const bool ans_smem = hf_layout(p).ans != 0xffffffffu;
#define JXLB_HF(W_)                                                                                          \
  do {                                                                                                       \
    if (ans_smem) launch_hf_warp<W_, true>(cs, f, p, jobs, end_bits, status, num_jobs, first_pass, stream);  \
    else launch_hf_warp<W_, false>(cs, f, p, jobs, end_bits, status, num_jobs, first_pass, stream);          \
  } while (0)
  if (warps_per_cta == 32) JXLB_HF(32);
  else if (warps_per_cta == 16) JXLB_HF(16);
  else JXLB_HF(8);
#undef JXLB_HF
}

}
```

### jxl_oxide_b200/csrc/kernels/kernels.h

```cpp
#pragma once
#include <cstdint>
#include <cuda_runtime.h>

#include "../host/frame_syntax.h"
#include "../host/headers.h"
#include "../host/modular_syntax.h"
#include "common.cuh"
#include "jpeg_blocks.cuh"

namespace jxlb {

struct DevChannel {
  int32_t* ptr;
  uint32_t stride, w, h;
  int32_t hshift, vshift;
};

struct DevChannelPlan {
  uint32_t root;
  int32_t lut_prop;
  int32_t lut_base;
  uint32_t lut_len, lut_offset;
};

struct DevPlacement {
  const int32_t* raw;
  uint32_t raw_stride, nb_blocks;
  uint32_t bw, bh;
  uint32_t grid_stride;
  int32_t* blk_type;
  int32_t* blk_mul;
  float* epf_sigma;
  const int32_t* sharpness;
  float quant_mul_base;
  float sharp_lut[8];
  uint32_t has_epf;
};
constexpr size_t kPlaceSharedBytes = 2112;

struct DevModularJob {
  uint64_t bit_pos, bit_limit;
  const MaNode* tree;
  uint32_t num_tree_nodes;
  const uint16_t* luts;
  uint32_t lut_total;
  DevEntropyCode code;
  uint32_t wp[11];
  uint32_t stream_index;
  uint32_t first_channel, num_channels;
  uint32_t dist_multiplier;
  uint32_t use_wp;
  int32_t* wp_scratch;
  uint32_t* lz_window;
  DevPlacement place;
};

struct DevView {
  void* ptr;
  uint32_t stride, w, h;
};

struct DevChannel;
struct DevChannelPlan;
struct DevModularBatchRef {
  const uint8_t* cs;
  const DevModularJob* jobs;
  const DevChannel* channels;
  const DevChannelPlan* plans;
  uint64_t* end_bits;
  int* status;
  uint32_t job;
  uint32_t num_jobs;
  uint32_t* counter;
  uint32_t* done_flag;
  uint32_t done_seq, pad;
};

void launch_modular_decode(const uint8_t* codestream, const DevModularJob* jobs, const DevChannel* channels,
                           const DevChannelPlan* plans, uint64_t* end_bits, int* status, int num_jobs,
                           size_t smem_bytes, bool all_tables_staged, cudaStream_t stream,
                           unsigned long long* trace = nullptr);
void launch_signal_word(uint32_t* host_mapped_word, uint32_t value, cudaStream_t stream);
void launch_modular_decode_batch(const DevModularBatchRef* refs, int total, size_t smem_bytes, bool all_tables_staged,
                                 cudaStream_t stream);
void launch_read_globaltimer(unsigned long long* out, cudaStream_t stream);
void launch_squeeze_inverse(DevView avg, DevView res, DevView out, bool horizontal, cudaStream_t stream);
void launch_squeeze_inverse_batch(const DevView* avg, const DevView* res, const DevView* out, int n, bool horizontal,
                                  cudaStream_t stream);
void launch_rct_inverse(DevView a, DevView b, DevView c, uint32_t rct_type, cudaStream_t stream);
constexpr int kMaxPaletteChannels = 16;
struct DevPaletteDeltaParams {
  DevView target[kMaxPaletteChannels];
  const uint8_t* mask;
  uint32_t d_pred;
  uint32_t wp[11];
  int32_t* wp_rows;
};
void launch_palette_delta(DevPaletteDeltaParams p, int num_c, cudaStream_t stream);
void launch_palette_inverse(DevView palette, const DevView* targets, int num_c, int nb_colours, int bit_depth, int nb_deltas,
                            uint8_t* mask, int* status, cudaStream_t stream);
void launch_int_to_float(DevView v, uint32_t bits_per_sample, uint32_t exp_bits, bool float_sample, cudaStream_t stream);
void launch_modular_xyb(DevView y, DevView x, DevView b, float mx, float my, float mb, cudaStream_t stream);
void launch_fill_u32(uint32_t* p, size_t n, uint32_t value, cudaStream_t stream);

struct DevLfGroupRect {
  uint32_t bx0, by0, bw, bh;
};
struct DevFrame {
  uint32_t width, height, bw, bh;
  uint32_t cw, ch;
  uint32_t w64;
  int32_t* lf_quant[3];
  int32_t* x_from_y;
  int32_t* b_from_y;
  int32_t* sharpness;
  int32_t* blk_type;
  int32_t* blk_mul;
  float* epf_sigma;
  float* lf[3];
  uint32_t* coeff[3];
  uint32_t group_blocks;
  uint8_t hshift[3], vshift[3], subsampled;
};
void launch_place_varblocks(const DevPlacement* jobs, int num_jobs, int* status, cudaStream_t stream);

struct DevHfParams {
  DevEntropyCode code;
  const uint32_t* orders;
  uint32_t order_offset[13 * 3];
  const uint8_t* block_ctx_map;
  uint32_t block_ctx_map_size;
  const int32_t* lf_thresholds;
  uint32_t num_lf_thr[3];
  uint32_t has_lf_quant;
  const uint32_t* qf_thresholds;
  uint32_t num_qf_thr;
  uint32_t num_block_clusters, num_hf_presets, coeff_shift;
  uint32_t group_dim_blocks, groups_per_row;
};
struct DevHfJob {
  uint64_t bit_pos, bit_limit;
  uint32_t group_idx;
};
constexpr uint32_t kHfAnsSmemBytes = 128 * 1024;
constexpr uint32_t kLaneCmapSmemBytes = 32 * 1024;
void launch_decode_hf(const uint8_t* codestream, DevFrame f, DevHfParams p, const DevHfJob* jobs, uint64_t* end_bits,
                      int* status, int num_jobs, int first_pass, int warps_per_cta, cudaStream_t stream);
size_t hf_block_list_count(DevFrame f, DevHfParams p);
void launch_hf_block_list(DevFrame f, DevHfParams p, uint2* list, uint32_t* counts, cudaStream_t stream);
void launch_decode_hf_lanes(const uint8_t* codestream, DevFrame f, DevHfParams p, const uint2* list, const uint32_t* counts,
                            const DevHfJob* jobs, uint64_t* end_bits, int* status, int num_jobs, int first_pass,
                            int streams_per_cta, cudaStream_t stream);

struct DevLfDequantJob {
  DevLfGroupRect rect;
  float scale[3];
};
void launch_lf_dequant(DevFrame f, const DevLfDequantJob* jobs, int num_jobs, cudaStream_t stream);
void launch_lf_cfl(DevFrame f, float kx, float kb, cudaStream_t stream);
void launch_lf_smooth(DevFrame f, float* tmp[3], float lf_x, float lf_y, float lf_b, cudaStream_t stream);

struct DevDequantParams {
  const float* matrices;
  uint32_t matrix_offset[17 * 3 * 2];
  float quant_bias[3], quant_bias_numerator;
  float qm_scale[3];
  float global_scale;
  float base_correlation_x, base_correlation_b, colour_factor;
};
void launch_hf_dequant_cfl(DevFrame f, DevDequantParams p, cudaStream_t stream);
void launch_upsample_jpeg(DevView in, DevView out, int horizontal, int vertical, cudaStream_t stream);
void launch_hf_transform(DevFrame f, void* scratch, const DevDequantParams* fused_dequant, cudaStream_t stream);
size_t hf_transform_scratch_bytes(uint32_t bw, uint32_t bh);

void launch_gaborish(DevView in, DevView out, float w0, float w1, cudaStream_t stream);
struct DevEpfParams {
  float channel_scale[3];
  float pass0_sigma_scale, pass2_sigma_scale, border_sad_mul, sigma_for_modular;
};
void launch_epf_step(const DevView in[3], const DevView out[3], const float* sigma, uint32_t sigma_stride,
                     DevEpfParams p, int step, cudaStream_t stream);
struct DevColorParams {
  float opsin_bias[3], cbrt_opsin_bias[3], itscale, matrix[9];
  int apply_srgb_tf;
  int apply_bt709_tf;
  int second_stage, to_luma;
  float luminances[3], matrix2[9], gamma;
  float pq_intensity_target;
};
void launch_xyb_to_rgb(DevView x, DevView y, DevView b, DevColorParams p, cudaStream_t stream);
struct DevYcbcrParams {
  float y_offset, cr_to_r, cb_to_g, cr_to_g, cb_to_b;
};
void launch_ycbcr_to_rgb(DevView cb, DevView y, DevView cr, DevYcbcrParams p, cudaStream_t stream);
void launch_copy_rect(DevView src, DevView dst, cudaStream_t stream);
void launch_upsample(DevView in, DevView out, int k, const float* quarter, cudaStream_t stream);
struct DevPackParams {
  const float* planes[8];
  uint32_t strides[8];
  uint32_t num_channels;
  uint32_t width, height;
  uint32_t orientation;
  uint32_t sample_type;
  uint32_t num_spots;
  const float* spot_planes[8];
  uint32_t spot_strides[8];
  float spot_rgb[8][3];
  float spot_solidity[8];
};
void launch_pack_interleaved(DevPackParams p, void* out, cudaStream_t stream);
struct DevPatchJob {
  const float* src;
  float* dst;
  const float* base_alpha;
  const float* new_alpha;
  uint32_t src_stride, dst_stride, base_alpha_stride, new_alpha_stride, w, h, mode, clamp, premultiplied;
  uint32_t swapped;
};
void launch_blend_patches(const DevPatchJob* jobs, int num_jobs, cudaStream_t stream);
struct DevSplineArc {
  float x, y, sigma, inv_sigma, value[3];
  int32_t xbegin, xend, ybegin, yend;
};
void launch_splat_splines(const DevView v[3], const DevSplineArc* arcs, int num_arcs, cudaStream_t stream);
struct DevNoiseParams {
  float lut[9];
  float corr_x, corr_b;
  uint32_t group_dim;
  unsigned long long seed0;
};
void launch_add_noise(const DevView v[3], float* const field[3], DevNoiseParams p, cudaStream_t stream);
struct DevFusedFilterParams {
  int gab_enabled;
  float gab_w[3][2];
  int epf_iters;
  DevEpfParams epf;
  const float* sigma;
  uint32_t sigma_stride;
  int colour;
  DevColorParams col;
};
void launch_filters_fused(const DevView in[3], const DevView out[3], DevFusedFilterParams p, cudaStream_t stream);
bool fused_filters_supported(uint32_t width, uint32_t height);

size_t jpeg_scan_temp_bytes(uint32_t max_items);
void launch_jpeg_lengths(const DevJpegScan& p, const uint32_t* huff, const uint32_t* ezr_block, const uint32_t* ezr_count,
                         uint64_t* lens, uint32_t* err, cudaStream_t s);
void launch_jpeg_scan_u64(const uint64_t* in, uint64_t* out, uint32_t n, void* temp, size_t temp_bytes, cudaStream_t s);
void launch_jpeg_scan_u32(const uint32_t* in, uint32_t* out, uint32_t n, void* temp, size_t temp_bytes, cudaStream_t s);
void launch_jpeg_intervals(const DevJpegScan& p, const uint64_t* boff, uint64_t* ibytes, uint64_t* ipad, cudaStream_t s);
void launch_jpeg_emit(const DevJpegScan& p, const uint32_t* huff, const uint32_t* ezr_block, const uint32_t* ezr_count,
                      const uint64_t* boff, const uint64_t* ibx, const uint64_t* ipx, const uint8_t* pad, uint32_t* words,
                      uint32_t* err, cudaStream_t s);
void launch_jpeg_ff_count(const uint32_t* words, uint64_t total_bytes, uint32_t nw, uint32_t* cnt, cudaStream_t s);
void launch_jpeg_stuff(const uint32_t* words, uint64_t total_bytes, uint32_t nw, const uint32_t* ffoff, const uint64_t* ibx,
                       uint32_t nint, uint8_t* out, cudaStream_t s);

}
```

### jxl_oxide_b200/csrc/pipeline.cu

```cuda
#include <chrono>
#include <condition_variable>
#include <cstdio>
#include <cstdlib>
#include <cstring>
#include <deque>
#include <fstream>
#include <mutex>
#include <sstream>
#include <thread>

#include <pthread.h>
#include <sched.h>

#include "capi_internal.h"

using namespace jxlb;

namespace {

struct Job {
  const uint8_t* data = nullptr;
  size_t size = 0;
  int32_t slot = -1;
  int32_t out_mode = 0;
  void* dst = nullptr;
  size_t dst_bytes = 0;
  uint64_t tag = 0;
};

struct Done {
  uint64_t tag;
  int32_t status;
  std::string error;
  void* out = nullptr;
  size_t out_bytes = 0;
};

struct HostBuf {
  void* p = nullptr;
  size_t bytes = 0;
  bool busy = false;
};

struct Resident {
  std::vector<uint8_t> codestream;
  uint8_t* dptr = nullptr;
};

struct Slab {
  void* base = nullptr;
  size_t bytes = 0;
  bool busy = false;
  cudaStream_t stream = nullptr;
};

class BatchService : public LfBatchService {
 public:
  BatchService(int device, int num_streams) : device_(device) {
    cudaSetDevice(device_);
    for (int i = 0; i < num_streams; ++i) {
      Batch b;
      cudaStreamCreateWithFlags(&b.stream, cudaStreamNonBlocking);
      cudaHostAlloc(reinterpret_cast<void**>(&b.h_refs), kMaxRefs * sizeof(DevModularBatchRef), cudaHostAllocDefault);
      cudaMalloc(reinterpret_cast<void**>(&b.d_refs), kMaxRefs * sizeof(DevModularBatchRef));
      void* f = nullptr;
      cudaHostAlloc(&f, 64, cudaHostAllocMapped);
      b.flag = static_cast<volatile uint32_t*>(f);
      *b.flag = 0;
      cudaEventCreate(&b.e0);
      cudaEventCreate(&b.e1);
      batches_.push_back(b);
    }
    thread_ = std::thread([this] { loop(); });
  }
  ~BatchService() override {
    {
      std::lock_guard<std::mutex> lk(mu_);
      stop_ = true;
    }
    cv_pending_.notify_all();
    thread_.join();
    cudaSetDevice(device_);
    for (Batch& b : batches_) {
      cudaStreamSynchronize(b.stream);
      cudaStreamDestroy(b.stream);
      cudaFreeHost(b.h_refs);
      cudaFree(b.d_refs);
      cudaFreeHost(const_cast<uint32_t*>(b.flag));
      cudaEventDestroy(b.e0);
      cudaEventDestroy(b.e1);
    }
  }
  void run(LfBatchItem& item) override {
    Waiter w;
    w.item = &item;
    {
      std::lock_guard<std::mutex> lk(mu_);
      pending_.push_back(&w);
    }
    cv_pending_.notify_one();
    std::unique_lock<std::mutex> lk(mu_);
    w.cv.wait(lk, [&] { return w.done; });
    if (w.error != cudaSuccess) fail(kErrCuda, std::string("CUDA error in the LF batch: ") + cudaGetErrorString(w.error));
  }
  uint64_t launches() const { return launches_; }
  uint64_t items() const { return items_; }

 private:
  static constexpr int kMaxRefs = 4096;
  struct Waiter {
    LfBatchItem* item = nullptr;
    bool done = false;
    cudaError_t error = cudaSuccess;
    std::condition_variable cv;
  };
  struct Batch {
    cudaStream_t stream = nullptr;
    DevModularBatchRef* h_refs = nullptr;
    DevModularBatchRef* d_refs = nullptr;
    volatile uint32_t* flag = nullptr;
    uint32_t seq = 0;
    bool busy = false;
    bool timed = false;
    cudaEvent_t e0 = nullptr, e1 = nullptr;
    std::vector<Waiter*> riders;
    std::chrono::steady_clock::time_point t0, t_launch;
  };

  void finish(Batch& b, cudaError_t err) {
    float ms = 0.0f;
    if (b.timed && err == cudaSuccess) cudaEventElapsedTime(&ms, b.e0, b.e1);
    {
      std::lock_guard<std::mutex> lk(mu_);
      for (Waiter* w : b.riders) {
        w->item->elapsed_ms = ms;
        w->error = err;
        w->done = true;
        w->cv.notify_one();
      }
    }
    b.riders.clear();
    b.busy = false;
  }
  void wake_finished(Batch& b) {
    size_t keep = 0;
    for (size_t i = 0; i < b.riders.size(); ++i) {
      Waiter* w = b.riders[i];
      const LfBatchItem& it = *w->item;
      if (it.done_flag && *it.done_flag == it.ref.done_seq) {
        std::atomic_thread_fence(std::memory_order_acquire);
        std::lock_guard<std::mutex> lk(mu_);
        w->done = true;
        w->cv.notify_one();
      } else {
        b.riders[keep++] = w;
      }
    }
    b.riders.resize(keep);
  }

  void launch(Batch& b, std::vector<Waiter*>& take) {
    cudaError_t err = cudaSuccess;
    auto chk = [&](cudaError_t e) {
      if (err == cudaSuccess && e != cudaSuccess) err = e;
    };
    int total = 0;
    size_t smem = 0;
    bool all_staged = true, timed = false;
    for (Waiter* w : take) {
      LfBatchItem& it = *w->item;
      for (int i = 0; i < it.num_up; ++i)
        if (it.up[i].bytes) chk(cudaMemcpyAsync(it.up[i].dst, it.up[i].src, it.up[i].bytes, cudaMemcpyHostToDevice, b.stream));
      for (int j = 0; j < it.num_jobs; ++j) {
        DevModularBatchRef r = it.ref;
        r.job = uint32_t(j);
        b.h_refs[total++] = r;
      }
      smem = std::max(smem, it.smem_bytes);
      all_staged = all_staged && it.all_staged;
      timed = timed || it.want_timing;
    }
    chk(cudaMemcpyAsync(b.d_refs, b.h_refs, size_t(total) * sizeof(DevModularBatchRef), cudaMemcpyHostToDevice, b.stream));
    if (timed) chk(cudaEventRecord(b.e0, b.stream));
    launch_modular_decode_batch(b.d_refs, total, smem, all_staged, b.stream);
    chk(cudaGetLastError());
    if (timed) chk(cudaEventRecord(b.e1, b.stream));
    for (Waiter* w : take) {
      LfBatchItem& it = *w->item;
      for (int i = 0; i < it.num_down; ++i)
        if (it.down[i].bytes) chk(cudaMemcpyAsync(it.down[i].dst, it.down[i].src, it.down[i].bytes, cudaMemcpyDeviceToHost, b.stream));
    }
    b.seq += 1;
    launch_signal_word(const_cast<uint32_t*>(b.flag), b.seq, b.stream);
    chk(cudaGetLastError());
    b.riders = take;
    b.busy = true;
    b.timed = timed;
    b.t0 = b.t_launch = std::chrono::steady_clock::now();
    ++launches_;
    items_ += take.size();
    if (err != cudaSuccess) {
      cudaStreamSynchronize(b.stream);
      finish(b, err);
    }
  }

  void loop() {
    cudaSetDevice(device_);
    for (;;) {
      bool any_busy = false;
      for (Batch& b : batches_) {
        if (!b.busy) continue;
        wake_finished(b);
        if (*b.flag == b.seq) {
          std::atomic_thread_fence(std::memory_order_acquire);
          const double ms = std::chrono::duration<double, std::milli>(std::chrono::steady_clock::now() - b.t_launch).count();
          ema_batch_ms_ = ema_batch_ms_ == 0.0 ? ms : 0.8 * ema_batch_ms_ + 0.2 * ms;
          finish(b, cudaSuccess);
        } else if (std::chrono::steady_clock::now() - b.t0 > std::chrono::milliseconds(500)) {
          cudaError_t e = cudaStreamQuery(b.stream);
          if (e != cudaErrorNotReady && e != cudaSuccess) finish(b, e);
          else if (e == cudaSuccess && *b.flag == b.seq) finish(b, cudaSuccess);
          else b.t0 = std::chrono::steady_clock::now();
        }
        any_busy = any_busy || b.busy;
      }
      std::vector<Waiter*> take;
      Batch* free_batch = nullptr;
      for (Batch& b : batches_)
        if (!b.busy) {
          free_batch = &b;
          break;
        }
      const auto now = std::chrono::steady_clock::now();
      const double since_ms = std::chrono::duration<double, std::milli>(now - last_launch_).count();
      const double gap_ms = std::min(30.0, std::max(0.5, ema_batch_ms_ / double(batches_.size())));
      if (any_busy && since_ms < gap_ms) free_batch = nullptr;
      {
        std::unique_lock<std::mutex> lk(mu_);
        if (stop_ && pending_.empty() && !any_busy) return;
        if (free_batch && !pending_.empty()) {
          int refs = 0;
          while (!pending_.empty() && refs + pending_.front()->item->num_jobs <= kMaxRefs) {
            refs += pending_.front()->item->num_jobs;
            take.push_back(pending_.front());
            pending_.pop_front();
          }
        } else if (!any_busy) {
          cv_pending_.wait(lk, [&] { return stop_ || !pending_.empty(); });
          continue;
        }
      }
      if (!take.empty()) {
        launch(*free_batch, take);
        last_launch_ = std::chrono::steady_clock::now();
        continue;
      }
      std::this_thread::sleep_for(std::chrono::microseconds(60));
    }
  }

  int device_;
  std::vector<Batch> batches_;
  std::thread thread_;
  std::mutex mu_;
  std::condition_variable cv_pending_;
  std::deque<Waiter*> pending_;
  bool stop_ = false;
  uint64_t launches_ = 0, items_ = 0;
  std::chrono::steady_clock::time_point last_launch_{};
  double ema_batch_ms_ = 0.0;
};

std::vector<int> device_local_cpus(int device) {
  std::vector<int> cpus;
  char busid[32] = {0};
  if (cudaDeviceGetPCIBusId(busid, sizeof(busid), device) != cudaSuccess) return cpus;
  for (char* c = busid; *c; ++c) *c = char(tolower(*c));
  std::ifstream f(std::string("/sys/bus/pci/devices/") + busid + "/local_cpulist");
  std::string list;
  if (!f || !std::getline(f, list)) return cpus;
  std::stringstream ss(list);
  std::string part;
  while (std::getline(ss, part, ',')) {
    int a = 0, b = 0;
    if (std::sscanf(part.c_str(), "%d-%d", &a, &b) == 2) {
      for (int i = a; i <= b; ++i) cpus.push_back(i);
    } else if (std::sscanf(part.c_str(), "%d", &a) == 1) {
      cpus.push_back(a);
    }
  }
  return cpus;
}

}

struct jxlb_pipeline {
  int device = 0;
  int heavy_frames = 0;
  std::vector<jxlb_decoder*> decoders;
  std::vector<std::thread> threads;
  std::mutex mu;
  std::condition_variable cv_job, cv_done, cv_slab;
  std::deque<Job> queue;
  std::deque<Done> done;
  uint64_t submitted = 0, reported = 0;
  bool stopping = false;
  std::map<int32_t, Resident> resident;
  std::vector<Slab> slabs;
  std::unique_ptr<BatchService> batcher;
  std::vector<HostBuf> hostbufs;
  size_t host_bytes = 0;
  std::condition_variable cv_host;
  std::mutex copy_mu;
  std::string error;
  std::vector<int> cpus;

  size_t max_hint = 0;
  int acquire_slab(size_t bytes_hint) {
    std::unique_lock<std::mutex> lk(mu);
    max_hint = std::max(max_hint, bytes_hint);
    bytes_hint = max_hint;
    int idx = -1;
    cv_slab.wait(lk, [&] {
      for (size_t i = 0; i < slabs.size(); ++i)
        if (!slabs[i].busy) {
          idx = int(i);
          return true;
        }
      return false;
    });
    Slab& s = slabs[size_t(idx)];
    s.busy = true;
    if (s.bytes < bytes_hint) {
      lk.unlock();
      cudaSetDevice(device);
      if (s.base) cudaFree(s.base);
      s.base = nullptr;
      s.bytes = 0;
      void* p = nullptr;
      if (cudaMalloc(&p, bytes_hint) == cudaSuccess) {
        s.base = p;
        s.bytes = bytes_hint;
      } else {
        cudaGetLastError();
      }
    }
    return idx;
  }
  void* acquire_host(size_t bytes) {
    std::unique_lock<std::mutex> lk(mu);
    if (bytes > host_bytes) {
      cv_host.wait(lk, [&] {
        for (const HostBuf& b : hostbufs)
          if (b.busy) return false;
        return true;
      });
      if (bytes > host_bytes) {
        for (HostBuf& b : hostbufs) {
          if (b.p) cudaFreeHost(b.p);
          b.p = nullptr;
          b.bytes = 0;
          void* q = nullptr;
          if (cudaHostAlloc(&q, bytes, cudaHostAllocDefault) == cudaSuccess) {
            std::memset(q, 0, bytes);
            b.p = q;
            b.bytes = bytes;
          } else {
            cudaGetLastError();
          }
        }
        host_bytes = bytes;
      }
    }
    int idx = -1;
    cv_host.wait(lk, [&] {
      for (size_t i = 0; i < hostbufs.size(); ++i)
        if (!hostbufs[i].busy && hostbufs[i].p) {
          idx = int(i);
          return true;
        }
      for (const HostBuf& b : hostbufs)
        if (b.p) return false;
      idx = -2;
      return true;
    });
    if (idx < 0) return nullptr;
    hostbufs[size_t(idx)].busy = true;
    return hostbufs[size_t(idx)].p;
  }
  bool release_host(void* ptr) {
    bool found = false;
    {
      std::lock_guard<std::mutex> lk(mu);
      for (HostBuf& b : hostbufs)
        if (b.p == ptr && b.busy) {
          b.busy = false;
          found = true;
        }
    }
    if (found) cv_host.notify_all();
    return found;
  }
  void release_slab(int idx) {
    {
      std::lock_guard<std::mutex> lk(mu);
      slabs[size_t(idx)].busy = false;
    }
    cv_slab.notify_one();
  }

  void worker(size_t wi) {
    cudaSetDevice(device);
    if (!cpus.empty()) {
      cpu_set_t set;
      CPU_ZERO(&set);
      for (int c : cpus) CPU_SET(c, &set);
      pthread_setaffinity_np(pthread_self(), sizeof(set), &set);
    }
    jxlb_decoder* dec = decoders[wi];
    int held = -1;
    std::chrono::steady_clock::time_point granted;
    auto profiled = [&] { return dec->be->profile || dec->be->host_phases; };
    auto add_ms = [&](const char* name, std::chrono::steady_clock::time_point since, std::chrono::steady_clock::time_point now) {
      auto& acc = dec->be->profile_acc[name];
      acc.first += 1;
      acc.second += std::chrono::duration<double, std::milli>(now - since).count();
    };
    auto take_slot = [&](size_t hint) {
      const auto t0 = std::chrono::steady_clock::now();
      held = acquire_slab(hint);
      granted = std::chrono::steady_clock::now();
      if (profiled()) add_ms("host:slot_wait", t0, granted);
      dec->be->set_arena(slabs[size_t(held)].base, slabs[size_t(held)].bytes);
    };
    dec->be->on_heavy_stage = [&](size_t hint) {
      if (held >= 0) return;
      take_slot(hint);
    };
    dec->be->on_need_stream = [&] {
      if (held < 0) take_slot(0);
      dec->be->set_stream(slabs[size_t(held)].stream);
    };
    dec->be->lf_service = batcher.get();
    for (;;) {
      Job job;
      {
        std::unique_lock<std::mutex> lk(mu);
        cv_job.wait(lk, [&] { return stopping || !queue.empty(); });
        if (queue.empty()) return;
        job = queue.front();
        queue.pop_front();
      }
      Done d{job.tag, JXLB_OK, std::string()};
      int32_t rc;
      if (job.data) {
        rc = jxlb_decode(dec, job.data, job.size, nullptr);
      } else {
        const Resident* r = nullptr;
        {
          std::lock_guard<std::mutex> lk(mu);
          auto it = resident.find(job.slot);
          if (it != resident.end()) r = &it->second;
        }
        if (!r) {
          rc = JXLB_ERR_INVALID_ARG;
          dec->error = "unknown preload slot";
        } else {
          rc = decode_resident(dec, r->codestream.data(), r->codestream.size(), r->dptr, nullptr);
        }
      }
      if (rc == JXLB_OK && (job.out_mode == 4 || job.out_mode == 5)) {
        rc = jxlb_frame_write_to_device(dec, 0, job.out_mode - 4, 0, job.dst, job.dst_bytes);
        d.out = job.dst;
        d.out_bytes = job.dst_bytes;
      } else if (rc == JXLB_OK && job.out_mode != 0) {
        void* dst = job.dst;
        size_t dst_bytes = job.dst_bytes;
        if (!dst) {
          jxlb_frame_info fi;
          jxlb_frame_get_info(dec, 0, &fi);
          if (job.out_mode == 1) {
            dst_bytes = 0;
            for (const View& v : dec->res.frames[0].channels) dst_bytes += size_t(v.w) * v.h * 4;
          } else {
            dst_bytes = size_t(fi.width) * fi.height * size_t(jxlb_frame_stream_channels(dec, 0)) * (job.out_mode == 2 ? 1 : 2);
          }
          dst = acquire_host(dst_bytes);
          if (!dst) {
            rc = JXLB_ERR_CUDA;
            dec->error = "cannot allocate pinned host memory for the frame output";
          }
        }
        if (rc == JXLB_OK) {
          rc = jxlb_sync(dec);
          std::lock_guard<std::mutex> copy_lock(copy_mu);
          if (rc != JXLB_OK) {
          } else if (job.out_mode == 1) rc = frame_planar_to_host(dec, 0, static_cast<float*>(dst), dst_bytes);
          else rc = jxlb_frame_write_to_buffer(dec, 0, job.out_mode - 2, 0, dst, dst_bytes);
          d.out = dst;
          d.out_bytes = dst_bytes;
          if (rc != JXLB_OK && !job.dst) {
            release_host(dst);
            d.out = nullptr;
          }
        }
      } else if (rc == JXLB_OK) {
        rc = jxlb_sync(dec);
      }
      if (rc != JXLB_OK) {
        d.status = rc;
        d.error = dec->error;
        jxlb_sync(dec);
      }
      jxlb_release_frames(dec);
      if (held >= 0) {
        dec->be->end_arena();
        try {
          dec->be->end_lease();
        } catch (const Error&) {
        }
        release_slab(held);
        held = -1;
        if (profiled()) add_ms("host:slot_hold", granted, std::chrono::steady_clock::now());
      }
      {
        std::lock_guard<std::mutex> lk(mu);
        done.push_back(std::move(d));
      }
      cv_done.notify_all();
    }
  }
};

extern "C" {

int32_t jxlb_pipeline_create(int32_t device, const jxlb_pipeline_config* cfg, jxlb_pipeline** out) {
  if (!out) return JXLB_ERR_INVALID_ARG;
  *out = nullptr;
  const int workers = cfg && cfg->workers > 0 ? cfg->workers : 64;
  const int heavy = cfg && cfg->heavy_frames > 0 ? cfg->heavy_frames : 16;
  auto p = std::make_unique<jxlb_pipeline>();
  p->device = device;
  p->heavy_frames = heavy;
  p->slabs.resize(size_t(heavy));
  if (cudaSetDevice(device) != cudaSuccess) return JXLB_ERR_CUDA;
  cudaDeviceSetLimit(cudaLimitMaxL2FetchGranularity, 32);
  for (Slab& sl : p->slabs)
    if (cudaStreamCreateWithFlags(&sl.stream, cudaStreamNonBlocking) != cudaSuccess) return JXLB_ERR_CUDA;
  p->batcher.reset(new BatchService(device, cfg && cfg->batch_streams > 0 ? cfg->batch_streams : 6));
  p->hostbufs.resize(6);
  for (int i = 0; i < workers; ++i) {
    int32_t rc = JXLB_OK;
    jxlb_decoder* d = create_decoder_internal(device, 0, false, &rc);
    if (rc != JXLB_OK) {
      for (jxlb_decoder* q : p->decoders) jxlb_decoder_destroy(q);
      return rc;
    }
    jxlb_set_hf_streams_per_cta(d, cfg && cfg->hf_streams_per_cta > 0 ? cfg->hf_streams_per_cta : 128);
    p->decoders.push_back(d);
  }
  if (!(cfg && cfg->no_affinity)) p->cpus = device_local_cpus(device);
  for (int i = 0; i < workers; ++i) p->threads.emplace_back([q = p.get(), i] { q->worker(size_t(i)); });
  *out = p.release();
  return JXLB_OK;
}

void jxlb_pipeline_destroy(jxlb_pipeline* p) {
  if (!p) return;
  {
    std::lock_guard<std::mutex> lk(p->mu);
    p->stopping = true;
    p->queue.clear();
  }
  p->cv_job.notify_all();
  for (std::thread& t : p->threads) t.join();
  for (jxlb_decoder* d : p->decoders) jxlb_decoder_destroy(d);
  cudaSetDevice(p->device);
  p->batcher.reset();
  for (Slab& s : p->slabs) {
    if (s.base) cudaFree(s.base);
    if (s.stream) cudaStreamDestroy(s.stream);
  }
  for (auto& kv : p->resident)
    if (kv.second.dptr) cudaFree(kv.second.dptr);
  for (HostBuf& b : p->hostbufs)
    if (b.p) cudaFreeHost(b.p);
  delete p;
}

const char* jxlb_pipeline_last_error(const jxlb_pipeline* p) { return p ? p->error.c_str() : "null pipeline"; }

int32_t jxlb_pipeline_preload(jxlb_pipeline* p, int32_t slot, const uint8_t* data, size_t size) {
  if (!p || !data) return JXLB_ERR_INVALID_ARG;
  try {
    Resident r;
    r.codestream = extract_codestream(data, size);
    r.dptr = p->decoders[0]->be->upload_resident(r.codestream.data(), r.codestream.size());
    std::lock_guard<std::mutex> lk(p->mu);
    Resident& dst = p->resident[slot];
    if (dst.dptr) cudaFree(dst.dptr);
    dst = std::move(r);
    return JXLB_OK;
  } catch (const Error& e) {
    p->error = e.what();
    return e.code;
  }
}

int32_t jxlb_pipeline_submit(jxlb_pipeline* p, const uint8_t* data, size_t size, int32_t slot, int32_t out_mode, void* dst,
                             size_t dst_bytes, uint64_t tag) {
  if (!p || out_mode < 0 || out_mode > 5 || (!data && slot < 0) || (out_mode >= 4 && !dst)) return JXLB_ERR_INVALID_ARG;
  Job j;
  j.data = data;
  j.size = size;
  j.slot = slot;
  j.out_mode = out_mode;
  j.dst = dst;
  j.dst_bytes = dst_bytes;
  j.tag = tag;
  {
    std::lock_guard<std::mutex> lk(p->mu);
    if (p->stopping) return JXLB_ERR_INVALID_ARG;
    p->queue.push_back(j);
    ++p->submitted;
  }
  p->cv_job.notify_one();
  return JXLB_OK;
}

int32_t jxlb_pipeline_wait(jxlb_pipeline* p, uint64_t* tag, int32_t* status, void** out, size_t* out_bytes, char* err,
                           size_t err_cap) {
  if (!p || !tag || !status) return JXLB_ERR_INVALID_ARG;
  std::unique_lock<std::mutex> lk(p->mu);
  if (p->reported == p->submitted) return JXLB_ERR_INVALID_ARG;
  p->cv_done.wait(lk, [&] { return !p->done.empty(); });
  Done d = std::move(p->done.front());
  p->done.pop_front();
  ++p->reported;
  *tag = d.tag;
  *status = d.status;
  if (out) *out = d.out;
  if (out_bytes) *out_bytes = d.out_bytes;
  if (err && err_cap) std::snprintf(err, err_cap, "%s", d.error.c_str());
  return JXLB_OK;
}

int32_t jxlb_pipeline_release_output(jxlb_pipeline* p, void* out) {
  if (!p || !out) return JXLB_ERR_INVALID_ARG;
  return p->release_host(out) ? JXLB_OK : JXLB_ERR_INVALID_ARG;
}

uint64_t jxlb_pipeline_launch_count(const jxlb_pipeline* p) {
  uint64_t n = 0;
  if (p)
    for (const jxlb_decoder* d : p->decoders) n += d->be->launches;
  return n;
}

int32_t jxlb_pipeline_workers(const jxlb_pipeline* p) { return p ? int32_t(p->decoders.size()) : 0; }

jxlb_decoder* jxlb_pipeline_decoder(jxlb_pipeline* p, int32_t index) {
  return (p && index >= 0 && size_t(index) < p->decoders.size()) ? p->decoders[size_t(index)] : nullptr;
}

}
```

Before: 8377.

## Batch HF entropy decoding across frames via shared service with coefficient memory leases

Adds a separate coefficient-plane memory lease pool that is acquired before the heavy slab, so frames can decode HF groups without holding a stream slot. HF block-list and lane-decode kernels are refactored into CTA helpers and batched across frames by a generic batch service, with plane zeroing deferred into the batch item. The heavy slab is now requested after pass groups and sized smaller. The aim is to cut per-frame kernel launches and slot contention, at the cost of more device memory and extra coordination complexity.

```diff
diff --git a/jxl_oxide_b200/csrc/cuda_backend.cu b/jxl_oxide_b200/csrc/cuda_backend.cu
--- a/jxl_oxide_b200/csrc/cuda_backend.cu
+++ b/jxl_oxide_b200/csrc/cuda_backend.cu
@@ -61,10 +61,10 @@
   if (stream_) cudaStreamSynchronize(stream_);
   for (auto& kv : planes_)
     if (!(arena_base_ && kv.second.ptr >= static_cast<void*>(arena_base_) && kv.second.ptr < static_cast<void*>(arena_base_ + arena_cap_)) &&
-        !in_lf_arena(kv.second.ptr))
+        !in_lf_arena(kv.second.ptr) && !in_lease(kv.second.ptr))
       cudaFree(kv.second.ptr);
   for (void* p : temps_)
-    if (!in_lf_arena(p)) cudaFree(p);
+    if (!in_lf_arena(p) && !in_lease(p)) cudaFree(p);
   for (void* p : deferred_free_) cudaFree(p);
   if (d_codestream_ && !in_lf_arena(d_codestream_) && stream_) cudaFreeAsync(d_codestream_, stream_);
   if (d_natural_orders_) cudaFree(d_natural_orders_);
@@ -93,6 +93,8 @@
     }
     for (void* p : deferred_free_) CUDA_CHECK(cudaFreeAsync(p, stream_));
     deferred_free_.clear();
+    for (const BatchItem::Copy& z : pending_zero_) CUDA_CHECK(cudaMemsetAsync(z.dst, 0, z.bytes, stream_));
+    pending_zero_.clear();
   }
   return stream_;
 }
@@ -129,6 +131,26 @@
   if (heavy_announced_) return;
   heavy_announced_ = true;
   if (on_heavy_stage) on_heavy_stage(bytes_hint);
+}
+
+void CudaBackend::begin_coeff_stage(const VarDctState& st) {
+  if (!on_coeff_stage) return;
+  auto carve = [](size_t bytes) { return (bytes + 511) & ~size_t(511); };
+  const size_t gb = st.group_dim / 8, groups = size_t((st.bh + gb - 1) / gb) * st.groups_per_row;
+  on_coeff_stage(3 * carve(size_t(st.bw) * st.bh * 64 * 4) + carve(groups * gb * gb * sizeof(uint2) + groups * 4));
+}
+
+void CudaBackend::end_coeff_lease() {
+  if (!lease_base_) return;
+  std::vector<void*> keep;
+  for (void* p : temps_)
+    if (!in_lease(p)) keep.push_back(p);
+  temps_.swap(keep);
+  for (auto it = planes_.begin(); it != planes_.end();)
+    it = in_lease(it->second.ptr) ? planes_.erase(it) : std::next(it);
+  pending_zero_.clear();
+  lease_base_ = nullptr;
+  lease_cap_ = lease_off_ = 0;
 }
 
 void CudaBackend::end_arena() {
@@ -163,6 +185,15 @@
     }
     arena_spill_ += need;
   }
+  if (lease_base_ && !arena_base_ && bytes >= (256u << 10)) {
+    const size_t need = (bytes + 511) & ~size_t(511);
+    if (lease_off_ + need <= lease_cap_) {
+      p = lease_base_ + lease_off_;
+      lease_off_ += need;
+      if (mem_limit_) mem_in_use_ += need;
+      return p;
+    }
+  }
   if (!stream_ && lf_service) {
     if (void* q = lf_arena_alloc(std::max<size_t>(bytes, 16))) return q;
   }
@@ -176,7 +207,7 @@
 }
 void CudaBackend::dfree(void* p) {
   if (!p) return;
-  if (in_lf_arena(p)) return;
+  if (in_lf_arena(p) || in_lease(p)) return;
   if (!stream_ && lf_service) {
     deferred_free_.push_back(p);
     return;
@@ -420,7 +451,8 @@
   r.h = h;
   size_t bytes = size_t(w) * h * 4;
   r.ptr = dmalloc(bytes);
-  if (zero) CUDA_CHECK(cudaMemsetAsync(r.ptr, 0, bytes, S()));
+  if (zero && !stream_ && in_lease(r.ptr)) pending_zero_.push_back({r.ptr, nullptr, bytes});
+  else if (zero) CUDA_CHECK(cudaMemsetAsync(r.ptr, 0, bytes, S()));
   int id = next_id_++;
   planes_[id] = r;
   return id;
@@ -572,6 +604,7 @@
       item.ref.done_flag = const_cast<uint32_t*>(h_flag_ + 16);
       item.ref.done_seq = ++item_seq_;
       item.done_flag = h_flag_ + 16;
+      item.done_seq = item.ref.done_seq;
     }
     item.want_timing = profile;
     lf_service->run(item);
@@ -737,33 +770,104 @@
   std::vector<DevHfJob> dj;
   for (uint32_t i : perm) dj.push_back({jobs[i].bit_pos, jobs[i].bit_limit, jobs[i].group_idx});
   const DevHfJob* d_jobs = static_cast<const DevHfJob*>(upload_temp(dj.data(), dj.size() * sizeof(DevHfJob)));
-  uint64_t* d_end = static_cast<uint64_t*>(stage_scratch(jobs.size() * 8));
-  int* d_status = static_cast<int*>(stage_scratch(jobs.size() * 4));
+  const size_t lease_mark = lease_off_;
   uint2* d_list = nullptr;
   uint32_t* d_counts = nullptr;
+  size_t groups = 0;
   if (sched.lanes) {
-    const size_t groups = hf_block_list_count(dev_frame(st), p);
+    groups = hf_block_list_count(dev_frame(st), p);
     const size_t records = groups * p.group_dim_blocks * p.group_dim_blocks;
     d_list = static_cast<uint2*>(dmalloc(records * sizeof(uint2) + groups * 4));
     temps_.push_back(d_list);
     d_counts = reinterpret_cast<uint32_t*>(d_list + records);
-    begin_k("hf_block_ctx");
-    launch_hf_block_list(dev_frame(st), p, d_list, d_counts, S());
+  }
+  const uint64_t* end;
+  const int* status;
+  uint32_t* d_counter = nullptr;
+  const bool ride = !stream_ && hf_service && sched.lanes && jobs.size() <= 8192;
+  if (ride) {
+    const uint32_t zero = 0;
+    d_counter = static_cast<uint32_t*>(upload_temp(&zero, 4));
+  }
+  if (ride && !stream_) {
+    HfBatchItem item;
+    if (pending_cs_bytes_) {
+      item.up[item.num_up++] = {d_codestream_, h_input_, pending_cs_bytes_};
+      pending_cs_bytes_ = 0;
+    }
+    item.up[item.num_up++] = {d_stage_, h_stage_, stage_off_};
+    JXLB_CHECK(pending_zero_.size() <= sizeof(item.zero) / sizeof(item.zero[0]), kErrUnsupported,
+               "too many lease planes to zero in one HF batch item");
+    for (const BatchItem::Copy& z : pending_zero_) item.zero[item.num_zero++] = z;
+    pending_zero_.clear();
+    uint8_t* h_end = h_result_;
+    uint8_t* h_status = h_result_ + ((jobs.size() * 8 + 15) & ~size_t(15));
+    JXLB_CHECK(size_t(h_status - h_result_) + jobs.size() * 4 <= result_cap_, kErrUnsupported, "too many stream jobs in one launch for the result buffer");
+    DevHfBatchFrame& fr = item.frame;
+    fr.f = dev_frame(st);
+    fr.p = p;
+    fr.cs = active_cs_;
+    fr.list = d_list;
+    fr.counts = d_counts;
+    fr.jobs = d_jobs;
+    fr.end_bits = reinterpret_cast<uint64_t*>(h_end);
+    fr.status = reinterpret_cast<int*>(h_status);
+    fr.num_jobs = uint32_t(jobs.size());
+    fr.first_pass = pass == 0 ? 1 : 0;
+    fr.counter = d_counter;
+    fr.done_flag = const_cast<uint32_t*>(h_flag_ + 16);
+    fr.done_seq = ++item_seq_;
+    item.num_groups = uint32_t(groups);
+    item.sub = fr.f.subsampled != 0;
+    const HfLanesShape shape = hf_lanes_shape(p, sched.per_cta);
+    fr.num_ctas = uint32_t((jobs.size() + size_t(shape.nthreads) - 1) / size_t(shape.nthreads));
+    item.nthreads = shape.nthreads;
+    item.staged = shape.staged;
+    item.smem_bytes = shape.smem_bytes;
+    if (!profile) item.done_flag = h_flag_ + 16;
+    item.done_seq = fr.done_seq;
+    item.want_timing = profile;
+    hf_service->run(item);
+    launches += 2;
+    if (profile || host_phases) {
+      if (item.riders > 1) ++profile_acc["host:hf_batch_shared"].first;
+      if (item.sub) ++profile_acc["host:hf_batch_sub"].first;
+    }
+    if (profile) {
+      auto& acc_b = profile_acc["hf_block_ctx"];
+      acc_b.first += 1;
+      acc_b.second += double(item.block_list_ms);
+      auto& acc = profile_acc["decode_hf"];
+      acc.first += 1;
+      acc.second += double(item.elapsed_ms);
+    }
+    stage_off_ = stage_flushed_ = 0;
+    result_off_ = 0;
+    end = reinterpret_cast<const uint64_t*>(h_end);
+    status = reinterpret_cast<const int*>(h_status);
+  } else {
+    uint64_t* d_end = static_cast<uint64_t*>(stage_scratch(jobs.size() * 8));
+    int* d_status = static_cast<int*>(stage_scratch(jobs.size() * 4));
+    if (sched.lanes) {
+      begin_k("hf_block_ctx");
+      launch_hf_block_list(dev_frame(st), p, d_list, d_counts, S());
+      end_k();
+    }
+    begin_k("decode_hf");
+    if (sched.lanes)
+      launch_decode_hf_lanes(active_cs_, dev_frame(st), p, d_list, d_counts, d_jobs, d_end, d_status, int(jobs.size()),
+                             pass == 0 ? 1 : 0, sched.per_cta, S());
+    else
+      launch_decode_hf(active_cs_, dev_frame(st), p, d_jobs, d_end, d_status, int(jobs.size()), pass == 0 ? 1 : 0,
+                       sched.per_cta, S());
     end_k();
-  }
-  begin_k("decode_hf");
-  if (sched.lanes)
-    launch_decode_hf_lanes(active_cs_, dev_frame(st), p, d_list, d_counts, d_jobs, d_end, d_status, int(jobs.size()),
-                           pass == 0 ? 1 : 0, sched.per_cta, S());
-  else
-    launch_decode_hf(active_cs_, dev_frame(st), p, d_jobs, d_end, d_status, int(jobs.size()), pass == 0 ? 1 : 0,
-                     sched.per_cta, S());
-  end_k();
-  const uint64_t* end = static_cast<const uint64_t*>(fetch_result(d_end, jobs.size() * 8));
-  const int* status = static_cast<const int*>(fetch_result(d_status, jobs.size() * 4));
-  sync();
-  CUDA_CHECK(cudaGetLastError());
+    end = static_cast<const uint64_t*>(fetch_result(d_end, jobs.size() * 8));
+    status = static_cast<const int*>(fetch_result(d_status, jobs.size() * 4));
+    sync();
+    CUDA_CHECK(cudaGetLastError());
+  }
   release_temps();
+  if (in_lease(d_list)) lease_off_ = lease_mark;
   for (size_t i = 0; i < jobs.size(); ++i) {
     HfGroupJob& job = jobs[perm[i]];
     if (status[i] != kDevOk)
diff --git a/jxl_oxide_b200/csrc/cuda_backend.h b/jxl_oxide_b200/csrc/cuda_backend.h
--- a/jxl_oxide_b200/csrc/cuda_backend.h
+++ b/jxl_oxide_b200/csrc/cuda_backend.h
@@ -13,7 +13,7 @@
 
 namespace jxlb {
 
-struct LfBatchItem {
+struct BatchItem {
   struct Copy {
     void* dst;
     const void* src;
@@ -21,20 +21,34 @@
   };
   Copy up[2];
   int num_up = 0;
+  Copy zero[3];
+  int num_zero = 0;
+  Copy down[2];
+  int num_down = 0;
+  volatile uint32_t* done_flag = nullptr;
+  uint32_t done_seq = 0;
+  bool want_timing = false;
+  float elapsed_ms = 0.0f;
+};
+struct LfBatchItem : BatchItem {
   DevModularBatchRef ref{};
   int num_jobs = 0;
   size_t smem_bytes = 0;
   bool all_staged = false;
-  Copy down[2];
-  int num_down = 0;
-  volatile uint32_t* done_flag = nullptr;
-  bool want_timing = false;
-  float elapsed_ms = 0.0f;
-};
-class LfBatchService {
+};
+struct HfBatchItem : BatchItem {
+  DevHfBatchFrame frame{};
+  uint32_t num_groups = 0;
+  bool sub = false, staged = false;
+  int nthreads = 128;
+  size_t smem_bytes = 0;
+  float block_list_ms = 0.0f;
+  int riders = 0;
+};
+class BatchService {
  public:
-  virtual ~LfBatchService() {}
-  virtual void run(LfBatchItem& item) = 0;
+  virtual ~BatchService() {}
+  virtual void run(BatchItem& item) = 0;
 };
 
 struct StopDecode {};
@@ -85,12 +99,21 @@
   void begin_heavy_stage(size_t bytes_hint) override;
   std::function<void(size_t)> on_heavy_stage;
   std::function<void()> on_need_stream;
+  void begin_coeff_stage(const VarDctState& st) override;
+  std::function<void(size_t)> on_coeff_stage;
+  void set_lease(void* base, size_t bytes) {
+    lease_base_ = static_cast<uint8_t*>(base);
+    lease_cap_ = bytes;
+    lease_off_ = 0;
+  }
+  bool has_lease() const { return lease_base_ != nullptr; }
   void set_arena(void* base, size_t bytes) {
     arena_base_ = static_cast<uint8_t*>(base);
     arena_cap_ = bytes;
     arena_off_ = 0;
   }
   void end_arena();
+  void end_coeff_lease();
   void set_mem_limit(uint64_t bytes) { mem_limit_ = bytes; }
   uint64_t mem_in_use() const { return mem_in_use_; }
   size_t arena_peak() const { return arena_peak_; }
@@ -100,7 +123,8 @@
   void set_stream(cudaStream_t s) { stream_ = s; }
   bool has_stream() const { return stream_ != nullptr; }
   void end_lease();
-  LfBatchService* lf_service = nullptr;
+  BatchService* lf_service = nullptr;
+  BatchService* hf_service = nullptr;
   uint8_t* upload_resident(const uint8_t* data, size_t size);
   void use_resident_once(const uint8_t* dptr) { resident_next_ = dptr; }
   void sync();
@@ -185,6 +209,12 @@
   uint32_t sync_seq_ = 0, item_seq_ = 0;
   uint8_t* arena_base_ = nullptr;
   size_t arena_cap_ = 0, arena_off_ = 0, arena_peak_ = 0, arena_spill_ = 0;
+  uint8_t* lease_base_ = nullptr;
+  size_t lease_cap_ = 0, lease_off_ = 0;
+  bool in_lease(const void* p) const {
+    return lease_base_ && p >= static_cast<const void*>(lease_base_) && p < static_cast<const void*>(lease_base_ + lease_cap_);
+  }
+  std::vector<BatchItem::Copy> pending_zero_;
   bool heavy_announced_ = false;
   uint64_t mem_limit_ = 0, mem_in_use_ = 0;
   std::map<void*, size_t> alloc_sizes_;
diff --git a/jxl_oxide_b200/csrc/host/backend.h b/jxl_oxide_b200/csrc/host/backend.h
--- a/jxl_oxide_b200/csrc/host/backend.h
+++ b/jxl_oxide_b200/csrc/host/backend.h
@@ -121,6 +121,7 @@
   virtual void set_codestream(const uint8_t* data, size_t size) = 0;
   virtual void new_frame() {}
   virtual void begin_heavy_stage(size_t ) {}
+  virtual void begin_coeff_stage(const VarDctState& ) {}
   virtual int alloc_plane(uint32_t w, uint32_t h, bool zero) = 0;
   virtual void free_plane(int id) = 0;
   virtual void download_rect(const View& v, void* dst) = 0;
diff --git a/jxl_oxide_b200/csrc/host/planner.cc b/jxl_oxide_b200/csrc/host/planner.cc
--- a/jxl_oxide_b200/csrc/host/planner.cc
+++ b/jxl_oxide_b200/csrc/host/planner.cc
@@ -671,8 +671,8 @@
 
   be_.phase_mark("hf_global");
   if (vardct) {
-    be_.begin_heavy_stage(size_t(st_.bw) * st_.bh * 64 * 4 * 6 + (size_t(64) << 20));
-    be_.phase_mark("heavy_wait");
+    be_.begin_coeff_stage(st_);
+    be_.phase_mark("lease_wait");
     for (int c = 0; c < 3; ++c) st_.coeff[c] = new_plane(st_.bw * 8, st_.bh * 8, true);
   }
   for (uint32_t p = 0; p < num_passes; ++p) {
@@ -704,6 +704,10 @@
   }
 
   be_.phase_mark("pass_groups");
+  if (vardct) {
+    be_.begin_heavy_stage(size_t(st_.bw) * st_.bh * 64 * 4 * 3 + (size_t(64) << 20));
+    be_.phase_mark("heavy_wait");
+  }
   {
     std::vector<View> coded;
     if (lfg_.has_gmodular)
diff --git a/jxl_oxide_b200/csrc/kernels/entropy.cu b/jxl_oxide_b200/csrc/kernels/entropy.cu
--- a/jxl_oxide_b200/csrc/kernels/entropy.cu
+++ b/jxl_oxide_b200/csrc/kernels/entropy.cu
@@ -210,10 +210,10 @@
 
 
 template <bool SUB>
-__global__ void __launch_bounds__(256) hf_block_list_kernel(DevFrame f, DevHfParams p, uint2* __restrict__ list,
-                                                            uint32_t* __restrict__ counts) {
+__device__ __forceinline__ void hf_block_list_cta(const DevFrame& f, const DevHfParams& p, uint2* __restrict__ list,
+                                                  uint32_t* __restrict__ counts, uint32_t g) {
   __shared__ uint32_t s_warp[8];
-  const uint32_t g = blockIdx.x, tid = threadIdx.x, lane = tid & 31, warp = tid >> 5;
+  const uint32_t tid = threadIdx.x, lane = tid & 31, warp = tid >> 5;
   const HfGroupRect r = hf_group_rect(f, p, g);
   const uint32_t n = r.width * r.height;
   uint2* out = list + size_t(g) * p.group_dim_blocks * p.group_dim_blocks;
@@ -236,14 +236,26 @@
   if (tid == 0) counts[g] = base;
 }
 
+template <bool SUB>
+__global__ void __launch_bounds__(256) hf_block_list_kernel(DevFrame f, DevHfParams p, uint2* __restrict__ list,
+                                                            uint32_t* __restrict__ counts) {
+  hf_block_list_cta<SUB>(f, p, list, counts, blockIdx.x);
+}
+
+template <bool SUB>
+__global__ void __launch_bounds__(256) hf_block_list_batch_kernel(const __grid_constant__ DevHfBatchParams P,
+                                                                  const DevHfBatchCta* __restrict__ ctas) {
+  const DevHfBatchCta c = ctas[blockIdx.x];
+  const DevHfBatchFrame& fr = P.frames[c.frame];
+  hf_block_list_cta<SUB>(fr.f, fr.p, fr.list, fr.counts, c.first);
+}
+
 template <bool SUB, bool STAGED>
-__global__ void __launch_bounds__(128) decode_hf_lanes_kernel(const uint8_t* __restrict__ cs, DevFrame f, DevHfParams p,
-                                                              const uint2* __restrict__ list,
-                                                              const uint32_t* __restrict__ counts,
-                                                              const DevHfJob* __restrict__ jobs,
-                                                              uint64_t* __restrict__ end_bits, int* __restrict__ status,
-                                                              int num_jobs, int first_pass) {
-  extern __shared__ __align__(16) uint8_t smem[];
+__device__ __forceinline__ void hf_lanes_cta(uint8_t* smem, const uint8_t* __restrict__ cs, const DevFrame& f,
+                                             const DevHfParams& p, const uint2* __restrict__ list,
+                                             const uint32_t* __restrict__ counts, const DevHfJob* __restrict__ jobs,
+                                             uint64_t* __restrict__ end_bits, int* __restrict__ status, int job_idx,
+                                             int num_jobs, int first_pass) {
   const uint32_t tid = threadIdx.x, nthreads = blockDim.x;
   const HfLaneSmem L = hf_lane_layout(p, nthreads);
   uint8_t* s_ctx = smem + L.ctxlut;
@@ -298,7 +310,6 @@
     T.cv.ans = reinterpret_cast<const uint64_t*>(s_ans);
   }
   __syncthreads();
-  const int job_idx = blockIdx.x * int(nthreads) + int(tid);
   if (job_idx >= num_jobs) return;
   const DevHfJob job = jobs[job_idx];
   const uint32_t gb = p.group_dim_blocks;
@@ -306,6 +317,34 @@
                               first_pass, end_bits + job_idx, status + job_idx);
 }
 
+template <bool SUB, bool STAGED>
+__global__ void __launch_bounds__(128) decode_hf_lanes_kernel(const uint8_t* __restrict__ cs, DevFrame f, DevHfParams p,
+                                                              const uint2* __restrict__ list,
+                                                              const uint32_t* __restrict__ counts,
+                                                              const DevHfJob* __restrict__ jobs,
+                                                              uint64_t* __restrict__ end_bits, int* __restrict__ status,
+                                                              int num_jobs, int first_pass) {
+  extern __shared__ __align__(16) uint8_t smem[];
+  hf_lanes_cta<SUB, STAGED>(smem, cs, f, p, list, counts, jobs, end_bits, status,
+                            int(blockIdx.x * blockDim.x + threadIdx.x), num_jobs, first_pass);
+}
+
+template <bool SUB, bool STAGED>
+__global__ void __launch_bounds__(128) decode_hf_lanes_batch_kernel(const __grid_constant__ DevHfBatchParams P,
+                                                                    const DevHfBatchCta* __restrict__ ctas) {
+  extern __shared__ __align__(16) uint8_t smem[];
+  const DevHfBatchCta c = ctas[blockIdx.x];
+  const DevHfBatchFrame& fr = P.frames[c.frame];
+  hf_lanes_cta<SUB, STAGED>(smem, fr.cs, fr.f, fr.p, fr.list, fr.counts, fr.jobs, fr.end_bits, fr.status,
+                            int(c.first + threadIdx.x), int(fr.num_jobs), int(fr.first_pass));
+  __threadfence_system();
+  __syncthreads();
+  if (threadIdx.x == 0 && atomicAdd(fr.counter, 1u) == fr.num_ctas - 1) {
+    __threadfence_system();
+    *reinterpret_cast<volatile uint32_t*>(fr.done_flag) = fr.done_seq;
+  }
+}
+
 }
 
 size_t hf_block_list_count(DevFrame f, DevHfParams p) {
@@ -317,6 +356,12 @@
   const uint32_t groups = uint32_t(hf_block_list_count(f, p));
   if (f.subsampled) hf_block_list_kernel<true><<<groups, 256, 0, stream>>>(f, p, list, counts);
   else hf_block_list_kernel<false><<<groups, 256, 0, stream>>>(f, p, list, counts);
+}
+
+HfLanesShape hf_lanes_shape(const DevHfParams& p, int streams_per_cta) {
+  const int nthreads = streams_per_cta <= 64 ? 64 : 128;
+  const HfLaneSmem L = hf_lane_layout(p, uint32_t(nthreads));
+  return HfLanesShape{nthreads, L.total, hf_lane_staged(p, L)};
 }
 
 void launch_decode_hf_lanes(const uint8_t* cs, DevFrame f, DevHfParams p, const uint2* list, const uint32_t* counts,
@@ -331,17 +376,46 @@
     return true;
   }();
   (void)attr_set;
-  const int nthreads = streams_per_cta <= 64 ? 64 : 128;
-  const HfLaneSmem L = hf_lane_layout(p, uint32_t(nthreads));
-  const int ctas = (num_jobs + nthreads - 1) / nthreads;
-#define JXLB_HF_LANES(SUB_, STAGED_)                                                                                 \
-  decode_hf_lanes_kernel<SUB_, STAGED_><<<ctas, nthreads, L.total, stream>>>(cs, f, p, list, counts, jobs, end_bits, \
-                                                                             status, num_jobs, first_pass)
-  if (hf_lane_staged(p, L)) {
+  const HfLanesShape shape = hf_lanes_shape(p, streams_per_cta);
+  const int ctas = (num_jobs + shape.nthreads - 1) / shape.nthreads;
+#define JXLB_HF_LANES(SUB_, STAGED_)                                                                          \
+  decode_hf_lanes_kernel<SUB_, STAGED_><<<ctas, shape.nthreads, shape.smem_bytes, stream>>>(                  \
+      cs, f, p, list, counts, jobs, end_bits, status, num_jobs, first_pass)
+  if (shape.staged) {
     if (f.subsampled) JXLB_HF_LANES(true, true);
     else JXLB_HF_LANES(false, true);
   } else {
     if (f.subsampled) JXLB_HF_LANES(true, false);
+    else JXLB_HF_LANES(false, false);
+  }
+#undef JXLB_HF_LANES
+}
+
+void launch_hf_block_list_batch(const DevHfBatchParams& frames, const DevHfBatchCta* ctas, int num_ctas, bool sub,
+                                cudaStream_t stream) {
+  if (num_ctas <= 0) return;
+  if (sub) hf_block_list_batch_kernel<true><<<num_ctas, 256, 0, stream>>>(frames, ctas);
+  else hf_block_list_batch_kernel<false><<<num_ctas, 256, 0, stream>>>(frames, ctas);
+}
+
+void launch_decode_hf_lanes_batch(const DevHfBatchParams& frames, const DevHfBatchCta* ctas, int num_ctas, bool sub,
+                                  bool staged, int nthreads, size_t smem_bytes, cudaStream_t stream) {
+  if (num_ctas <= 0) return;
+  static const bool attr_set = [] {
+    cudaFuncSetAttribute(decode_hf_lanes_batch_kernel<false, false>, cudaFuncAttributeMaxDynamicSharedMemorySize, 200 * 1024);
+    cudaFuncSetAttribute(decode_hf_lanes_batch_kernel<true, false>, cudaFuncAttributeMaxDynamicSharedMemorySize, 200 * 1024);
+    cudaFuncSetAttribute(decode_hf_lanes_batch_kernel<false, true>, cudaFuncAttributeMaxDynamicSharedMemorySize, 200 * 1024);
+    cudaFuncSetAttribute(decode_hf_lanes_batch_kernel<true, true>, cudaFuncAttributeMaxDynamicSharedMemorySize, 200 * 1024);
+    return true;
+  }();
+  (void)attr_set;
+#define JXLB_HF_LANES(SUB_, STAGED_) \
+  decode_hf_lanes_batch_kernel<SUB_, STAGED_><<<num_ctas, nthreads, smem_bytes, stream>>>(frames, ctas)
+  if (staged) {
+    if (sub) JXLB_HF_LANES(true, true);
+    else JXLB_HF_LANES(false, true);
+  } else {
+    if (sub) JXLB_HF_LANES(true, false);
     else JXLB_HF_LANES(false, false);
   }
 #undef JXLB_HF_LANES
diff --git a/jxl_oxide_b200/csrc/kernels/kernels.h b/jxl_oxide_b200/csrc/kernels/kernels.h
--- a/jxl_oxide_b200/csrc/kernels/kernels.h
+++ b/jxl_oxide_b200/csrc/kernels/kernels.h
@@ -151,6 +151,40 @@
 void launch_decode_hf_lanes(const uint8_t* codestream, DevFrame f, DevHfParams p, const uint2* list, const uint32_t* counts,
                             const DevHfJob* jobs, uint64_t* end_bits, int* status, int num_jobs, int first_pass,
                             int streams_per_cta, cudaStream_t stream);
+struct DevHfBatchFrame {
+  DevFrame f;
+  DevHfParams p;
+  const uint8_t* cs;
+  uint2* list;
+  uint32_t* counts;
+  const DevHfJob* jobs;
+  uint64_t* end_bits;
+  int* status;
+  uint32_t num_jobs, first_pass;
+  uint32_t num_ctas;
+  uint32_t done_seq;
+  uint32_t* counter;
+  uint32_t* done_flag;
+};
+constexpr int kHfBatchMaxFrames = 48;
+struct DevHfBatchParams {
+  DevHfBatchFrame frames[kHfBatchMaxFrames];
+};
+static_assert(sizeof(DevHfBatchParams) <= 32000, "kernel parameter space");
+struct DevHfBatchCta {
+  uint32_t frame;
+  uint32_t first;
+};
+struct HfLanesShape {
+  int nthreads;
+  size_t smem_bytes;
+  bool staged;
+};
+HfLanesShape hf_lanes_shape(const DevHfParams& p, int streams_per_cta);
+void launch_hf_block_list_batch(const DevHfBatchParams& frames, const DevHfBatchCta* ctas, int num_ctas, bool sub,
+                                cudaStream_t stream);
+void launch_decode_hf_lanes_batch(const DevHfBatchParams& frames, const DevHfBatchCta* ctas, int num_ctas, bool sub,
+                                  bool staged, int nthreads, size_t smem_bytes, cudaStream_t stream);
 
 struct DevLfDequantJob {
   DevLfGroupRect rect;
diff --git a/jxl_oxide_b200/csrc/pipeline.cu b/jxl_oxide_b200/csrc/pipeline.cu
--- a/jxl_oxide_b200/csrc/pipeline.cu
+++ b/jxl_oxide_b200/csrc/pipeline.cu
@@ -54,26 +54,156 @@
   cudaStream_t stream = nullptr;
 };
 
-class BatchService : public LfBatchService {
+bool grow_block(int device, void*& base, size_t& bytes, size_t want) {
+  if (bytes >= want) return true;
+  cudaSetDevice(device);
+  if (base) cudaFree(base);
+  base = nullptr;
+  bytes = 0;
+  void* p = nullptr;
+  if (cudaMalloc(&p, want) != cudaSuccess) {
+    cudaGetLastError();
+    return false;
+  }
+  base = p;
+  bytes = want;
+  return true;
+}
+
+class BatchKernels {
  public:
-  BatchService(int device, int num_streams) : device_(device) {
+  virtual ~BatchKernels() {}
+  virtual size_t stage_bytes() const = 0;
+  virtual bool fits(const std::vector<BatchItem*>& items, const BatchItem& next) const = 0;
+  virtual void launch(const std::vector<BatchItem*>& items, uint8_t* h_stage, uint8_t* d_stage, cudaStream_t s,
+                      cudaEvent_t* ev) = 0;
+  virtual void report_times(BatchItem& item, float first_ms, float second_ms) const = 0;
+};
+
+class LfBatchKernels : public BatchKernels {
+ public:
+  size_t stage_bytes() const override { return kMaxRefs * sizeof(DevModularBatchRef); }
+  bool fits(const std::vector<BatchItem*>& items, const BatchItem& next) const override {
+    int refs = static_cast<const LfBatchItem&>(next).num_jobs;
+    for (const BatchItem* it : items) refs += static_cast<const LfBatchItem*>(it)->num_jobs;
+    return refs <= kMaxRefs;
+  }
+  void launch(const std::vector<BatchItem*>& items, uint8_t* h_stage, uint8_t* d_stage, cudaStream_t s, cudaEvent_t* ev) override {
+    DevModularBatchRef* h_refs = reinterpret_cast<DevModularBatchRef*>(h_stage);
+    int total = 0;
+    size_t smem = 0;
+    bool all_staged = true;
+    for (BatchItem* b : items) {
+      const LfBatchItem& it = *static_cast<LfBatchItem*>(b);
+      for (int j = 0; j < it.num_jobs; ++j) {
+        DevModularBatchRef r = it.ref;
+        r.job = uint32_t(j);
+        h_refs[total++] = r;
+      }
+      smem = std::max(smem, it.smem_bytes);
+      all_staged = all_staged && it.all_staged;
+    }
+    cudaMemcpyAsync(d_stage, h_stage, size_t(total) * sizeof(DevModularBatchRef), cudaMemcpyHostToDevice, s);
+    if (ev) cudaEventRecord(ev[0], s), cudaEventRecord(ev[1], s);
+    launch_modular_decode_batch(reinterpret_cast<const DevModularBatchRef*>(d_stage), total, smem, all_staged, s);
+    if (ev) cudaEventRecord(ev[2], s);
+  }
+  void report_times(BatchItem& item, float, float second_ms) const override { item.elapsed_ms = second_ms; }
+
+ private:
+  static constexpr int kMaxRefs = 4096;
+};
+
+class HfBatchKernels : public BatchKernels {
+ public:
+  size_t stage_bytes() const override {
+    return size_t(kMaxCtas) * sizeof(DevHfBatchCta);
+  }
+  bool fits(const std::vector<BatchItem*>& items, const BatchItem& next) const override {
+    if (items.size() + 1 > size_t(kHfBatchMaxFrames)) return false;
+    size_t ctas = ctas_of(next);
+    for (const BatchItem* it : items) ctas += ctas_of(*it);
+    return ctas <= size_t(kMaxCtas);
+  }
+  void launch(const std::vector<BatchItem*>& items, uint8_t* h_stage, uint8_t* d_stage, cudaStream_t s, cudaEvent_t* ev) override {
+    DevHfBatchCta* h_ctas = reinterpret_cast<DevHfBatchCta*>(h_stage);
+    struct Launch {
+      bool sub, staged;
+      int nthreads;
+      size_t smem;
+      uint32_t first, count;
+    };
+    std::vector<Launch> lists, decodes;
+    uint32_t n = 0;
+    for (int sub = 0; sub < 2; ++sub) {
+      Launch L{sub != 0, false, 256, 0, n, 0};
+      for (size_t i = 0; i < items.size(); ++i) {
+        const HfBatchItem& it = *static_cast<const HfBatchItem*>(items[i]);
+        if (it.sub != (sub != 0)) continue;
+        for (uint32_t g = 0; g < it.num_groups; ++g) h_ctas[n++] = DevHfBatchCta{uint32_t(i), g};
+      }
+      L.count = n - L.first;
+      if (L.count) lists.push_back(L);
+    }
+    for (int v = 0; v < 8; ++v) {
+      Launch L{(v & 1) != 0, (v & 2) != 0, (v & 4) ? 128 : 64, 0, n, 0};
+      for (size_t i = 0; i < items.size(); ++i) {
+        const HfBatchItem& it = *static_cast<const HfBatchItem*>(items[i]);
+        if (it.sub != L.sub || it.staged != L.staged || it.nthreads != L.nthreads) continue;
+        for (uint32_t j = 0; j < it.frame.num_jobs; j += uint32_t(it.nthreads)) h_ctas[n++] = DevHfBatchCta{uint32_t(i), j};
+        L.smem = std::max(L.smem, it.smem_bytes);
+      }
+      L.count = n - L.first;
+      if (L.count) decodes.push_back(L);
+    }
+    for (size_t i = 0; i < items.size(); ++i) {
+      HfBatchItem& it = *static_cast<HfBatchItem*>(items[i]);
+      params_.frames[i] = it.frame;
+      it.riders = int(items.size());
+    }
+    cudaMemcpyAsync(d_stage, h_ctas, size_t(n) * sizeof(DevHfBatchCta), cudaMemcpyHostToDevice, s);
+    const DevHfBatchCta* d_ctas = reinterpret_cast<const DevHfBatchCta*>(d_stage);
+    if (ev) cudaEventRecord(ev[0], s);
+    for (const Launch& L : lists) launch_hf_block_list_batch(params_, d_ctas + L.first, int(L.count), L.sub, s);
+    if (ev) cudaEventRecord(ev[1], s);
+    for (const Launch& L : decodes)
+      launch_decode_hf_lanes_batch(params_, d_ctas + L.first, int(L.count), L.sub, L.staged, L.nthreads, L.smem, s);
+    if (ev) cudaEventRecord(ev[2], s);
+  }
+  void report_times(BatchItem& item, float first_ms, float second_ms) const override {
+    static_cast<HfBatchItem&>(item).block_list_ms = first_ms;
+    item.elapsed_ms = second_ms;
+  }
+
+ private:
+  DevHfBatchParams params_{};
+  static constexpr int kMaxCtas = 32768;
+  static size_t ctas_of(const BatchItem& b) {
+    const HfBatchItem& it = static_cast<const HfBatchItem&>(b);
+    return it.num_groups + (it.frame.num_jobs + uint32_t(it.nthreads) - 1) / uint32_t(it.nthreads);
+  }
+};
+
+class PipelineBatchService : public BatchService {
+ public:
+  PipelineBatchService(int device, int num_streams, std::unique_ptr<BatchKernels> kernels)
+      : device_(device), kernels_(std::move(kernels)) {
     cudaSetDevice(device_);
     for (int i = 0; i < num_streams; ++i) {
       Batch b;
       cudaStreamCreateWithFlags(&b.stream, cudaStreamNonBlocking);
-      cudaHostAlloc(reinterpret_cast<void**>(&b.h_refs), kMaxRefs * sizeof(DevModularBatchRef), cudaHostAllocDefault);
-      cudaMalloc(reinterpret_cast<void**>(&b.d_refs), kMaxRefs * sizeof(DevModularBatchRef));
+      cudaHostAlloc(reinterpret_cast<void**>(&b.h_stage), kernels_->stage_bytes(), cudaHostAllocDefault);
+      cudaMalloc(reinterpret_cast<void**>(&b.d_stage), kernels_->stage_bytes());
       void* f = nullptr;
       cudaHostAlloc(&f, 64, cudaHostAllocMapped);
       b.flag = static_cast<volatile uint32_t*>(f);
       *b.flag = 0;
-      cudaEventCreate(&b.e0);
-      cudaEventCreate(&b.e1);
+      for (cudaEvent_t& e : b.ev) cudaEventCreate(&e);
       batches_.push_back(b);
     }
     thread_ = std::thread([this] { loop(); });
   }
-  ~BatchService() override {
+  ~PipelineBatchService() override {
     {
       std::lock_guard<std::mutex> lk(mu_);
       stop_ = true;
@@ -84,14 +214,13 @@
     for (Batch& b : batches_) {
       cudaStreamSynchronize(b.stream);
       cudaStreamDestroy(b.stream);
-      cudaFreeHost(b.h_refs);
-      cudaFree(b.d_refs);
+      cudaFreeHost(b.h_stage);
+      cudaFree(b.d_stage);
       cudaFreeHost(const_cast<uint32_t*>(b.flag));
-      cudaEventDestroy(b.e0);
-      cudaEventDestroy(b.e1);
-    }
-  }
-  void run(LfBatchItem& item) override {
+      for (cudaEvent_t e : b.ev) cudaEventDestroy(e);
+    }
+  }
+  void run(BatchItem& item) override {
     Waiter w;
     w.item = &item;
     {
@@ -101,39 +230,39 @@
     cv_pending_.notify_one();
     std::unique_lock<std::mutex> lk(mu_);
     w.cv.wait(lk, [&] { return w.done; });
-    if (w.error != cudaSuccess) fail(kErrCuda, std::string("CUDA error in the LF batch: ") + cudaGetErrorString(w.error));
-  }
-  uint64_t launches() const { return launches_; }
-  uint64_t items() const { return items_; }
+    if (w.error != cudaSuccess) fail(kErrCuda, std::string("CUDA error in a pipeline batch: ") + cudaGetErrorString(w.error));
+  }
 
  private:
-  static constexpr int kMaxRefs = 4096;
   struct Waiter {
-    LfBatchItem* item = nullptr;
+    BatchItem* item = nullptr;
     bool done = false;
     cudaError_t error = cudaSuccess;
     std::condition_variable cv;
   };
   struct Batch {
     cudaStream_t stream = nullptr;
-    DevModularBatchRef* h_refs = nullptr;
-    DevModularBatchRef* d_refs = nullptr;
+    uint8_t* h_stage = nullptr;
+    uint8_t* d_stage = nullptr;
     volatile uint32_t* flag = nullptr;
     uint32_t seq = 0;
     bool busy = false;
     bool timed = false;
-    cudaEvent_t e0 = nullptr, e1 = nullptr;
+    cudaEvent_t ev[3] = {nullptr, nullptr, nullptr};
     std::vector<Waiter*> riders;
     std::chrono::steady_clock::time_point t0, t_launch;
   };
 
   void finish(Batch& b, cudaError_t err) {
-    float ms = 0.0f;
-    if (b.timed && err == cudaSuccess) cudaEventElapsedTime(&ms, b.e0, b.e1);
+    float first = 0.0f, second = 0.0f;
+    if (b.timed && err == cudaSuccess) {
+      cudaEventElapsedTime(&first, b.ev[0], b.ev[1]);
+      cudaEventElapsedTime(&second, b.ev[1], b.ev[2]);
+    }
     {
       std::lock_guard<std::mutex> lk(mu_);
       for (Waiter* w : b.riders) {
-        w->item->elapsed_ms = ms;
+        kernels_->report_times(*w->item, first, second);
         w->error = err;
         w->done = true;
         w->cv.notify_one();
@@ -146,8 +275,8 @@
     size_t keep = 0;
     for (size_t i = 0; i < b.riders.size(); ++i) {
       Waiter* w = b.riders[i];
-      const LfBatchItem& it = *w->item;
-      if (it.done_flag && *it.done_flag == it.ref.done_seq) {
+      const BatchItem& it = *w->item;
+      if (it.done_flag && *it.done_flag == it.done_seq) {
         std::atomic_thread_fence(std::memory_order_acquire);
         std::lock_guard<std::mutex> lk(mu_);
         w->done = true;
@@ -164,29 +293,20 @@
     auto chk = [&](cudaError_t e) {
       if (err == cudaSuccess && e != cudaSuccess) err = e;
     };
-    int total = 0;
-    size_t smem = 0;
-    bool all_staged = true, timed = false;
+    bool timed = false;
+    std::vector<BatchItem*> items;
     for (Waiter* w : take) {
-      LfBatchItem& it = *w->item;
+      BatchItem& it = *w->item;
       for (int i = 0; i < it.num_up; ++i)
         if (it.up[i].bytes) chk(cudaMemcpyAsync(it.up[i].dst, it.up[i].src, it.up[i].bytes, cudaMemcpyHostToDevice, b.stream));
-      for (int j = 0; j < it.num_jobs; ++j) {
-        DevModularBatchRef r = it.ref;
-        r.job = uint32_t(j);
-        b.h_refs[total++] = r;
-      }
-      smem = std::max(smem, it.smem_bytes);
-      all_staged = all_staged && it.all_staged;
+      for (int i = 0; i < it.num_zero; ++i) chk(cudaMemsetAsync(it.zero[i].dst, 0, it.zero[i].bytes, b.stream));
       timed = timed || it.want_timing;
-    }
-    chk(cudaMemcpyAsync(b.d_refs, b.h_refs, size_t(total) * sizeof(DevModularBatchRef), cudaMemcpyHostToDevice, b.stream));
-    if (timed) chk(cudaEventRecord(b.e0, b.stream));
-    launch_modular_decode_batch(b.d_refs, total, smem, all_staged, b.stream);
+      items.push_back(&it);
+    }
+    kernels_->launch(items, b.h_stage, b.d_stage, b.stream, timed ? b.ev : nullptr);
     chk(cudaGetLastError());
-    if (timed) chk(cudaEventRecord(b.e1, b.stream));
     for (Waiter* w : take) {
-      LfBatchItem& it = *w->item;
+      BatchItem& it = *w->item;
       for (int i = 0; i < it.num_down; ++i)
         if (it.down[i].bytes) chk(cudaMemcpyAsync(it.down[i].dst, it.down[i].src, it.down[i].bytes, cudaMemcpyDeviceToHost, b.stream));
     }
@@ -197,8 +317,6 @@
     b.busy = true;
     b.timed = timed;
     b.t0 = b.t_launch = std::chrono::steady_clock::now();
-    ++launches_;
-    items_ += take.size();
     if (err != cudaSuccess) {
       cudaStreamSynchronize(b.stream);
       finish(b, err);
@@ -240,9 +358,9 @@
         std::unique_lock<std::mutex> lk(mu_);
         if (stop_ && pending_.empty() && !any_busy) return;
         if (free_batch && !pending_.empty()) {
-          int refs = 0;
-          while (!pending_.empty() && refs + pending_.front()->item->num_jobs <= kMaxRefs) {
-            refs += pending_.front()->item->num_jobs;
+          std::vector<BatchItem*> items;
+          while (!pending_.empty() && (items.empty() || kernels_->fits(items, *pending_.front()->item))) {
+            items.push_back(pending_.front()->item);
             take.push_back(pending_.front());
             pending_.pop_front();
           }
@@ -261,13 +379,13 @@
   }
 
   int device_;
+  std::unique_ptr<BatchKernels> kernels_;
   std::vector<Batch> batches_;
   std::thread thread_;
   std::mutex mu_;
   std::condition_variable cv_pending_;
   std::deque<Waiter*> pending_;
   bool stop_ = false;
-  uint64_t launches_ = 0, items_ = 0;
   std::chrono::steady_clock::time_point last_launch_{};
   double ema_batch_ms_ = 0.0;
 };
@@ -308,7 +426,10 @@
   bool stopping = false;
   std::map<int32_t, Resident> resident;
   std::vector<Slab> slabs;
-  std::unique_ptr<BatchService> batcher;
+  std::vector<Slab> leases;
+  std::condition_variable cv_lease;
+  size_t max_lease = 0;
+  std::unique_ptr<PipelineBatchService> batcher, hf_batcher;
   std::vector<HostBuf> hostbufs;
   size_t host_bytes = 0;
   std::condition_variable cv_host;
@@ -317,10 +438,10 @@
   std::vector<int> cpus;
 
   size_t max_hint = 0;
-  int acquire_slab(size_t bytes_hint) {
+  int acquire_slab(size_t bytes_hint, bool with_coeff) {
     std::unique_lock<std::mutex> lk(mu);
     max_hint = std::max(max_hint, bytes_hint);
-    bytes_hint = max_hint;
+    bytes_hint = max_hint + (with_coeff ? max_lease : 0);
     int idx = -1;
     cv_slab.wait(lk, [&] {
       for (size_t i = 0; i < slabs.size(); ++i)
@@ -332,21 +453,38 @@
     });
     Slab& s = slabs[size_t(idx)];
     s.busy = true;
-    if (s.bytes < bytes_hint) {
-      lk.unlock();
-      cudaSetDevice(device);
-      if (s.base) cudaFree(s.base);
-      s.base = nullptr;
-      s.bytes = 0;
-      void* p = nullptr;
-      if (cudaMalloc(&p, bytes_hint) == cudaSuccess) {
-        s.base = p;
-        s.bytes = bytes_hint;
-      } else {
-        cudaGetLastError();
-      }
-    }
+    lk.unlock();
+    grow_block(device, s.base, s.bytes, bytes_hint);
     return idx;
+  }
+  int acquire_lease(size_t bytes) {
+    std::unique_lock<std::mutex> lk(mu);
+    max_lease = std::max(max_lease, bytes);
+    bytes = max_lease;
+    int idx = -1;
+    cv_lease.wait(lk, [&] {
+      for (size_t i = 0; i < leases.size(); ++i)
+        if (!leases[i].busy) {
+          idx = int(i);
+          return true;
+        }
+      return false;
+    });
+    Slab& l = leases[size_t(idx)];
+    l.busy = true;
+    lk.unlock();
+    if (!grow_block(device, l.base, l.bytes, bytes)) {
+      release_lease(idx);
+      return -1;
+    }
+    return idx;
+  }
+  void release_lease(int idx) {
+    {
+      std::lock_guard<std::mutex> lk(mu);
+      leases[size_t(idx)].busy = false;
+    }
+    cv_lease.notify_one();
   }
   void* acquire_host(size_t bytes) {
     std::unique_lock<std::mutex> lk(mu);
@@ -419,30 +557,44 @@
       pthread_setaffinity_np(pthread_self(), sizeof(set), &set);
     }
     jxlb_decoder* dec = decoders[wi];
-    int held = -1;
-    std::chrono::steady_clock::time_point granted;
+    int held = -1, lease = -1;
+    std::chrono::steady_clock::time_point granted, lease_granted;
     auto profiled = [&] { return dec->be->profile || dec->be->host_phases; };
     auto add_ms = [&](const char* name, std::chrono::steady_clock::time_point since, std::chrono::steady_clock::time_point now) {
       auto& acc = dec->be->profile_acc[name];
       acc.first += 1;
       acc.second += std::chrono::duration<double, std::milli>(now - since).count();
     };
-    auto take_slot = [&](size_t hint) {
+    auto take_slot = [&](size_t hint, bool with_coeff) {
       const auto t0 = std::chrono::steady_clock::now();
-      held = acquire_slab(hint);
+      held = acquire_slab(hint, with_coeff);
       granted = std::chrono::steady_clock::now();
       if (profiled()) add_ms("host:slot_wait", t0, granted);
       dec->be->set_arena(slabs[size_t(held)].base, slabs[size_t(held)].bytes);
     };
     dec->be->on_heavy_stage = [&](size_t hint) {
       if (held >= 0) return;
-      take_slot(hint);
+      take_slot(hint, false);
     };
     dec->be->on_need_stream = [&] {
-      if (held < 0) take_slot(0);
+      if (held < 0) take_slot(0, lease < 0);
       dec->be->set_stream(slabs[size_t(held)].stream);
     };
+    dec->be->on_coeff_stage = [&](size_t bytes) {
+      if (held >= 0) {
+        std::lock_guard<std::mutex> lk(mu);
+        max_lease = std::max(max_lease, bytes);
+        return;
+      }
+      if (lease >= 0) return;
+      const auto t0 = std::chrono::steady_clock::now();
+      lease = acquire_lease(bytes);
+      lease_granted = std::chrono::steady_clock::now();
+      if (profiled()) add_ms("host:lease_wait", t0, lease_granted);
+      if (lease >= 0) dec->be->set_lease(leases[size_t(lease)].base, leases[size_t(lease)].bytes);
+    };
     dec->be->lf_service = batcher.get();
+    dec->be->hf_service = hf_batcher.get();
     for (;;) {
       Job job;
       {
@@ -524,6 +676,12 @@
         held = -1;
         if (profiled()) add_ms("host:slot_hold", granted, std::chrono::steady_clock::now());
       }
+      if (lease >= 0) {
+        dec->be->end_coeff_lease();
+        release_lease(lease);
+        lease = -1;
+        if (profiled()) add_ms("host:lease_hold", lease_granted, std::chrono::steady_clock::now());
+      }
       {
         std::lock_guard<std::mutex> lk(mu);
         done.push_back(std::move(d));
@@ -544,11 +702,14 @@
   p->device = device;
   p->heavy_frames = heavy;
   p->slabs.resize(size_t(heavy));
+  p->leases.resize(size_t(2 * heavy));
   if (cudaSetDevice(device) != cudaSuccess) return JXLB_ERR_CUDA;
   cudaDeviceSetLimit(cudaLimitMaxL2FetchGranularity, 32);
   for (Slab& sl : p->slabs)
     if (cudaStreamCreateWithFlags(&sl.stream, cudaStreamNonBlocking) != cudaSuccess) return JXLB_ERR_CUDA;
-  p->batcher.reset(new BatchService(device, cfg && cfg->batch_streams > 0 ? cfg->batch_streams : 6));
+  p->batcher.reset(new PipelineBatchService(device, cfg && cfg->batch_streams > 0 ? cfg->batch_streams : 6,
+                                            std::unique_ptr<BatchKernels>(new LfBatchKernels)));
+  p->hf_batcher.reset(new PipelineBatchService(device, 4, std::unique_ptr<BatchKernels>(new HfBatchKernels)));
   p->hostbufs.resize(6);
   for (int i = 0; i < workers; ++i) {
     int32_t rc = JXLB_OK;
@@ -578,6 +739,9 @@
   for (jxlb_decoder* d : p->decoders) jxlb_decoder_destroy(d);
   cudaSetDevice(p->device);
   p->batcher.reset();
+  p->hf_batcher.reset();
+  for (Slab& l : p->leases)
+    if (l.base) cudaFree(l.base);
   for (Slab& s : p->slabs) {
     if (s.base) cudaFree(s.base);
     if (s.stream) cudaStreamDestroy(s.stream);
```

Result: faster. 8626 (median of 6 runs) (+3.0%).
